# gersteinlab/LESSeq

Hardware: AMD Instinct MI355X
Metric: MRF reads/sec through count+solve (higher is better)
Workload: dtype int32 coordinates / u64 counters (count), f64 (EM); 1 GPU; BASELINE configs[2]: 100M synthetic 100bp reads over 50k mixed events (SE/RI/A5SS/A3SS/MXE/AFE/ALE/T3), 24 chromosomes; events=50000

## Files before the change

### include/lesseq_hip.h

```cpp
#ifndef LESSEQ_HIP_H
#define LESSEQ_HIP_H

#include <stddef.h>
#include <stdint.h>

#ifdef __cplusplus
extern "C" {
#endif

#define LSQ_ABI_VERSION 2

typedef enum {
	LSQ_OK = 0,
	LSQ_E_ARG = -1,
	LSQ_E_IO = -2,
	LSQ_E_FORMAT = -3,
	LSQ_E_PARSE = -4,
	LSQ_E_RANGE = -5,
	LSQ_E_UNSUPPORTED = -6,
	LSQ_E_DEVICE = -7,
	LSQ_E_STATE = -8,
	LSQ_E_INTERNAL = -9,
	LSQ_E_TIMEOUT = -10
} lsq_status;
// ... 88 lines not shown
int lsq_ctx_synchronize_for(lsq_ctx *c, double seconds);

int lsq_events_upload(lsq_ctx *c, lsq_events *e);

int lsq_reads_upload(lsq_ctx *c, int method, const lsq_reads *r);
int lsq_reads_upload_mrf(lsq_ctx *c, int method, const char *read_format, const char *path);
typedef struct lsq_text lsq_text;
int lsq_text_stage(lsq_ctx *c, const char *path, lsq_text **out);
void lsq_text_free(lsq_text *t);
int lsq_reads_upload_text(lsq_ctx *c, int method, const char *read_format, lsq_text *t);
int lsq_text_stage_range(lsq_ctx *c, const char *path, uint64_t byte_begin, uint64_t byte_end, lsq_text **out);
int lsq_text_lines(lsq_ctx *c, lsq_text *t, uint64_t *n_newlines);
int lsq_reads_upload_text_at(lsq_ctx *c, int method, const char *read_format, lsq_text *t, int has_header, uint64_t first_line);
int lsq_mrf_parse_device(lsq_ctx *c, const char *read_format, const char *path, lsq_reads **out);
int lsq_last_mrf_timing(lsq_ctx *c, float *h2d_ms, float *parse_ms);
int lsq_ingest_stage_count(void);
const char *lsq_ingest_stage_name(int stage);
int lsq_last_ingest_stages(const lsq_ctx *c, float *ms, uint64_t *bytes, int capacity);
const char *lsq_last_ingest_stage_name(const lsq_ctx *c, int stage);
int lsq_last_ingest_stage_count(const lsq_ctx *c);
int lsq_last_sam_paths(const lsq_ctx *c, uint32_t *lines_listed, uint32_t *all_slow);
int lsq_last_bam_paths(const lsq_ctx *c, uint64_t *n_blocks, uint64_t *blocks_repaired);
int lsq_bam_check(lsq_ctx *c, const char *path, lsq_bam_report *r);
uint64_t lsq_reads_retained(const lsq_ctx *c, int method);
int lsq_last_library_report(const lsq_ctx *c, int method, uint64_t out[5]);
uint64_t lsq_reads_retained_blocks(const lsq_ctx *c, int method);
uint64_t lsq_reads_pooled(const lsq_ctx *c, int method);
uint64_t lsq_reads_pooled_blocks(const lsq_ctx *c, int method);
int lsq_reads_pool_format(const lsq_ctx *c, int method, int *compact, uint64_t *pool_bytes, uint64_t *pool_reads);

int lsq_count(lsq_ctx *c);
int lsq_count_status(lsq_ctx *c, uint32_t *exceptions, uint32_t *recounted);
int lsq_count_launch_info(lsq_ctx *c, uint32_t *reads_per_look, uint32_t *workgroups_per_cu);
int lsq_host_evaluated(const lsq_ctx *c, uint64_t *n_genes, uint64_t *n_reads);
int lsq_ctx_set_option(lsq_ctx *c, const char *name, double value);

int lsq_solve(lsq_ctx *c);

int64_t lsq_results_num_classes(const lsq_ctx *c);
int lsq_results_class_offsets(const lsq_ctx *c, uint64_t *class_off );
int lsq_results_counts(lsq_ctx *c, uint64_t *class_count, uint64_t *class_bases);
int lsq_results_set_counts(lsq_ctx *c, const uint64_t *class_count, const uint64_t *class_bases);
uint64_t lsq_counts_device_words(const lsq_ctx *c);
int lsq_counts_export_device(lsq_ctx *c, void *d_words);
int lsq_counts_import_device(lsq_ctx *c, const void *d_words);
int lsq_results_solve(lsq_ctx *c, double *theta, double *logll, uint32_t *em_iters, uint8_t *em_flags);
int lsq_solve_finalize(lsq_ctx *c, uint32_t *n_replayed);
int lsq_set_em_guard_band(lsq_ctx *c, double band);

int lsq_fim(lsq_ctx *c);
int64_t lsq_results_fim_size(const lsq_ctx *c);
int lsq_results_fim_offsets(const lsq_ctx *c, uint64_t *fim_off );
int lsq_results_fim(lsq_ctx *c, double *fim, double *var_by_diag, double *var_by_inverse);

int lsq_bootstrap(lsq_ctx *c, uint32_t n_replicates, uint64_t seed);
int lsq_results_bootstrap(lsq_ctx *c, uint32_t *n_ok, double *mean, double *sd, double *q025, double *q500, double *q975);
int lsq_results_bootstrap_theta(lsq_ctx *c, double *theta );
int lsq_bootstrap_replicate(lsq_ctx *c, uint64_t seed, uint32_t b, uint64_t *class_count, double *theta, double *logll, uint32_t *iters, uint8_t *flags);
int lsq_bootstrap_tile(void);
int lsq_bootstrap_resample_host(int n_methods, uint64_t n_events, const uint64_t *class_off, const uint64_t *class_count, uint64_t seed, uint32_t b,
                                uint64_t *out);

int lsq_results_copy_device(lsq_ctx *c, void *d_class_count, void *d_theta, void *d_logll);
void *lsq_ctx_result_stream(lsq_ctx *c);

int lsq_shard_bounds(const lsq_events *e, int world, const double *weights ,
// ... 177 lines not shown
```

### lesseq_amd/api.py

```python
import os
import ctypes as C

import numpy as np

from ._lib import lib, check, check_runtime_once, SynthSpecStruct, BamReportStruct, u64, u32, i32, u16, u8, i64, vp, cs, P, _b

EVENT_TYPES = ("SE", "RI", "A5SS", "A3SS", "MXE", "AFE", "ALE", "T3")


def _take_text(ptr):
    if not ptr:
        return ""
    s = C.string_at(ptr).decode()
    lib.lsq_free(ptr)
    return s


def _ptr(a, ct):
    return a.ctypes.data_as(P(ct))


class Annotation:

    def __init__(self, isoforms_path, g2i_path, begin=0, end=2 ** 62, isoform_format="LH_GENE_TXT", g2i_format="UCSC_GENE2ISOFORM"):
# ... 359 lines not shown
        check(lib.lsq_last_library_report(self.h, method, out))
        return tuple(out)

    def pooled(self, method):
        return lib.lsq_reads_pooled(self.h, method)

    def pooled_blocks(self, method):
        return lib.lsq_reads_pooled_blocks(self.h, method)

    def pool_format(self, method):
        a, n = C.c_int(0), C.c_uint64(0)
        k = (C.c_uint64 * 3)()
        check(lib.lsq_reads_pool_format(self.h, method, C.byref(a), C.byref(n), k))
        return bool(a.value), n.value, tuple(int(x) for x in k)

    def retained_blocks(self, method):
        return lib.lsq_reads_retained_blocks(self.h, method)

    def count(self):
        check(lib.lsq_count(self.h))

    def solve(self):
        check(lib.lsq_solve(self.h))

    def set_option(self, name, value):
        check(lib.lsq_ctx_set_option(self.h, _b(name), float(value)))

    def count_status(self):
        M = max(self.events.n_methods, 1)
        e, r = (u32 * M)(), (u32 * M)()
        check(lib.lsq_count_status(self.h, e, r))
        return list(e)[:self.events.n_methods], list(r)[:self.events.n_methods]

    def counts_device_words(self):
        return int(lib.lsq_counts_device_words(self.h))

    def export_counts_device(self, d_ptr):
        check(lib.lsq_counts_export_device(self.h, vp(d_ptr)))

    def import_counts_device(self, d_ptr):
        check(lib.lsq_counts_import_device(self.h, vp(d_ptr)))

    def launch_info(self):
        a, b = u32(), u32()
        check(lib.lsq_count_launch_info(self.h, C.byref(a), C.byref(b)))
        return int(a.value), int(b.value)

    def set_em_guard_band(self, band):
        check(lib.lsq_set_em_guard_band(self.h, float(band)))

    def solve_finalize(self):
        n = u32()
        check(lib.lsq_solve_finalize(self.h, C.byref(n)))
        return n.value

    EM_LEAN_FORMS = ("none", "four_lane", "four_lane_capped_tail", "head_tail", "four_lane_flat3", "four_lane_flat4")

    def em_launch(self):
        out = (C.c_uint * 8)()
        check(lib.lsq_debug_last_em_launch(self.h, out))
        return {"lean_form": self.EM_LEAN_FORMS[out[0]], "lean_places": int(out[1]), "split": int(out[2]), "general_places": int(out[3]),
                "learnt_placement": bool(out[4]), "quad_cap": int(out[5]), "placement_learnt_after": bool(out[6]), "lane": int(out[7])}

    def synchronize(self):
        check(lib.lsq_ctx_synchronize(self.h))

# ... 176 lines not shown
```

### lesseq_amd/csrc/lsq_count.hip

```cpp
#include "lsq_device.hpp"
#include <hip/hip_ext.h>

namespace {

#ifndef LSQ_COUNT_BLOCK
#define LSQ_COUNT_BLOCK 256
#endif
constexpr int COUNT_BLOCK = LSQ_COUNT_BLOCK;
constexpr unsigned long long BASES_MASK = (1ull << 40) - 1;

#ifdef LSQ_DEV
#define ABL(args, bits) ((((args).ablate) & (bits)) != 0u)
#else
#define ABL(args, bits) false
#endif


struct CountArgs {
	const BucketDesc *buckets;
	const unsigned char *images;
	const TieRec *ties;
	const unsigned char *strand_rank;
	const char *read_names; const unsigned long long *read_name_off;
	const char *gene_names; const unsigned *gene_name_off;
	unsigned n_buckets;
	unsigned ablate;
	unsigned tables_lds_bytes;
	const void *p1; const unsigned char *p1_strand; const unsigned *p1_line;
	const void *p2; const unsigned char *p2_strand; const unsigned *p2_line;
	unsigned compact;
	const unsigned *pn_blk_off; const unsigned *pn_nblk; const int2 *pn_se; const unsigned char *pn_strand; const unsigned *pn_line; const unsigned *pn_bucket;
	const unsigned long long *p1_off, *p2_off, *pn_off, *slot_off;
	const lsq::VisitRec *visits;
	const unsigned *wg_first;
	const unsigned long long *wg_cut;
	const lsq::WgPlan *wg_plan;
	unsigned long long *wg_trace;
	unsigned long long total_slots;
	unsigned long long n_pn;
	unsigned n_workers;
	unsigned long long *cnt, *bases;
	struct ExcEntry *exc;
	unsigned *exc_count;
	unsigned exc_cap;
	unsigned long long *dbg;
	unsigned long long *bar;
};

__device__ inline int2 unpack_one_block(const unsigned a, const int base) {
	const int s = base + (int)(a & lsq::COMPACT_OFF_MASK);
	return make_int2(s, s + (int)(a >> lsq::COMPACT_OFF_BITS));
}
__device__ inline int4 unpack_two_block(const unsigned a, const unsigned b, const int base) {
	const int s1 = base + (int)(a & lsq::COMPACT_OFF_MASK), e1 = s1 + (int)(a >> lsq::COMPACT_OFF_BITS);
	const int s2 = e1 + (int)(b & lsq::COMPACT_OFF_MASK);
	return make_int4(s1, e1, s2, s2 + (int)(b >> lsq::COMPACT_OFF_BITS));
}
__device__ inline int2 pool1_read(const CountArgs &A, const unsigned long long g, const int lo) {
	if (!A.compact) return reinterpret_cast<const int2 *>(A.p1)[g];
	return unpack_one_block(reinterpret_cast<const unsigned *>(A.p1)[g], lo - lsq::COMPACT_BIAS);
}
__device__ inline int4 pool2_read(const CountArgs &A, const unsigned long long g, const int lo) {
	if (!A.compact) return reinterpret_cast<const int4 *>(A.p2)[g];
	const uint2 v = reinterpret_cast<const uint2 *>(A.p2)[g];
	return unpack_two_block(v.x, v.y, lo - lsq::COMPACT_BIAS);
}

struct LdsView {
	const unsigned short *bins;
	const EventRec *ev;
	const int2 *segs;
	const unsigned *iso;
	unsigned long long *hist;
};

__device__ __noinline__ bool tie_orders_read_first(const CountArgs &A, unsigned ev_index, unsigned read_strand, unsigned line) {
	const TieRec *t = A.ties + ev_index;
	const unsigned rs = A.strand_rank[read_strand], gs = A.strand_rank[t->strand_id];
	if (rs != gs) return rs < gs;
// ... 151 lines not shown
			}
		}
		__syncthreads();
	}
}


__device__ inline int nonneg(int x) { return (int)(~(unsigned)x >> 31); }
__device__ inline int inside01(int a, int sx, int sy) { return nonneg((a - sx) | (sy - 1 - a)); }
__device__ inline int gt01(int b, int sy) { return (int)((unsigned)(sy - b) >> 31); }

__device__ inline unsigned run_bits(const int (&sy)[4], unsigned abut, int r0, int r1, int r2, int r3, int b, int &end_run) {
	r1 |= r0 & (int)(abut & 1u) & gt01(b, sy[0]);
	r2 |= r1 & (int)((abut >> 1) & 1u) & gt01(b, sy[1]);
	r3 |= r2 & (int)((abut >> 2) & 1u) & gt01(b, sy[2]);
	end_run = max(max(r0 ? sy[0] : 0, r1 ? sy[1] : 0), max(r2 ? sy[2] : 0, r3 ? sy[3] : 0));
	return (unsigned)(r0 | (r1 << 1) | (r2 << 2) | (r3 << 3));
}

struct FastCtx {
	const uint4 *bins;
	int lo; unsigned shift, n_bins;
	const uint4 *recs;
	unsigned long long *hist;
	unsigned n_events, bucket;
	unsigned long long slot0;
	unsigned pool;
	ExcEntry *exc;
	unsigned *exc_count;
	unsigned exc_cap;
	unsigned ablate;
	unsigned long long *dbg;
	unsigned long long *trace;
};

__device__ inline void emit_exception(const FastCtx &C, unsigned r, unsigned i, unsigned scan) {
	const unsigned slot = atomicAdd(C.exc_count, 1u);
	if (slot < C.exc_cap) {
		ExcEntry e;
		e.slot = C.slot0 + r;
		e.bucket = C.bucket;
		e.ev_pool_scan = i | (C.pool << 29) | (scan << 31);
		C.exc[slot] = e;
	}
}

constexpr unsigned PARK_EVENT_UNKNOWN = 0x7FFFFFFFu;
constexpr unsigned PARK_ONE_EVENT = 0x80000000u;

__device__ inline unsigned wave_sum_u32(unsigned v) {
	v += (unsigned)__builtin_amdgcn_update_dpp(0, (int)v, 0x111, 0xf, 0xf, true);
	v += (unsigned)__builtin_amdgcn_update_dpp(0, (int)v, 0x112, 0xf, 0xf, true);
	v += (unsigned)__builtin_amdgcn_update_dpp(0, (int)v, 0x114, 0xf, 0xf, true);
	v += (unsigned)__builtin_amdgcn_update_dpp(0, (int)v, 0x118, 0xf, 0xf, true);
	v += (unsigned)__builtin_amdgcn_update_dpp(0, (int)v, 0x142, 0xa, 0xf, true);
	v += (unsigned)__builtin_amdgcn_update_dpp(0, (int)v, 0x143, 0xc, 0xf, true);
	return (unsigned)__builtin_amdgcn_readlane((int)v, 63);
}

template <int NB>
__device__ inline bool fast_trip(const FastCtx &C, const int4 v, const int total, const unsigned r, const unsigned i, const bool valid) {
	const int p = v.x, q = (NB == 1) ? v.y : v.w;
	const bool inb = valid && i < C.n_events;
	const unsigned ri = 3u * (inb ? i : 0u);
	const uint4 w0 = C.recs[ri], w1 = C.recs[ri + 1], w2 = C.recs[ri + 2];
	const int gs = (int)w1.x, ge = (int)w0.x;
	const bool started = inb && gs <= p;
	bool covers = started && p <= ge;
	bool exc = covers && p == gs && q == ge;
	covers = covers && !(p == gs && q <= ge);
	if (NB == 2) {
		const bool touching = covers && v.z == v.y;
		exc = exc || touching;
		covers = covers && !touching;
	}
	if (exc && !ABL(C, 128u)) emit_exception(C, r, i, 0u);
	const int sx[4] = {(int)w1.x, (int)w1.z, (int)w2.x, (int)w2.z};
// ... 38 lines not shown
__device__ inline void wave_sync_lds() {
	__builtin_amdgcn_fence(__ATOMIC_ACQ_REL, "wavefront");
	__builtin_amdgcn_wave_barrier();
}

template <int NB>
struct Ring {
	static constexpr unsigned CAP = WAVE_QUEUE_WORDS / NB;
	uint4 *q;
	unsigned head = 0, tail = 0;
	__device__ inline unsigned live() const { return tail - head; }
	__device__ inline void push(bool want, unsigned lane, const uint4 e0, const uint4 e1) {
		const unsigned long long m = __ballot(want);
		if (!m) return;
		const unsigned at = (tail + (unsigned)__popcll(m & ((1ull << lane) - 1ull))) % CAP;
		if (want) {
			if (NB == 1) q[at] = e0;
			else { q[2 * at] = e0; q[2 * at + 1] = e1; }
		}
		tail += (unsigned)__popcll(m);
	}
	__device__ inline void push2(const unsigned bits, const unsigned lane, const uint4 ea, const uint4 eb) {
		static_assert(NB == 1 || NB == 2, "");
		const unsigned long long m0 = __ballot((bits & 1u) != 0u), m1 = __ballot((bits & 2u) != 0u);
		if (!(m0 | m1)) return;
		const unsigned long long lt = (1ull << lane) - 1ull;
		const unsigned at = tail + (unsigned)__popcll(m0 & lt) + (unsigned)__popcll(m1 & lt);
		if (bits & 1u) q[at % CAP] = ea;
		if (bits & 2u) q[(at + (bits & 1u)) % CAP] = eb;
		tail += (unsigned)__popcll(m0) + (unsigned)__popcll(m1);
	}
};

template <int NB, bool PACKED2 = false>
__device__ inline void walk_parked(const FastCtx &C, Ring<(NB == 1 || PACKED2) ? 1 : 2> &R, const bool to_empty, const int base = 0) {
	constexpr int RW = (NB == 1 || PACKED2) ? 1 : 2;
	const unsigned lane = threadIdx.x & 63u;
	wave_sync_lds();
#pragma unroll 1
	while (R.live() >= (to_empty ? 1u : 64u)) {
		const unsigned n = min(R.live(), 64u);
		const bool on = lane < n;
		if (ABL(C, 256u) && lane == 0) { atomicAdd(&C.dbg[2], 1ull); atomicAdd(&C.dbg[3], (unsigned long long)n); }
		if (ABL(C, 4194304u) && lane == 0 && C.trace) { atomicAdd(&C.trace[2], 1ull); atomicAdd(&C.trace[3], (unsigned long long)n); }
		const unsigned at = (R.head + (on ? lane : 0u)) % Ring<RW>::CAP;
		uint4 e0, e1 = make_uint4(0, 0, 0, 0);
		if (RW == 1) e0 = R.q[at];
		else { e0 = R.q[2 * at]; e1 = R.q[2 * at + 1]; }
		R.head += n;
		int4 rd; unsigned i, rel;
		const unsigned ev_word = RW == 1 ? e0.z : e1.x;
		const bool one_event = (ev_word & PARK_ONE_EVENT) != 0;
		if (RW == 1) { e0.z &= ~PARK_ONE_EVENT; } else { e1.x &= ~PARK_ONE_EVENT; }
		if (NB == 1) {
			rd = make_int4((int)e0.x, (int)e0.y, (int)e0.x, (int)e0.y); i = e0.z; rel = e0.w;
			const int brel = rd.x - C.lo;
			const unsigned bin = brel <= 0 ? 0u : min((unsigned)brel >> C.shift, C.n_bins - 1u);
			const unsigned first = reinterpret_cast<const unsigned *>(C.bins)[4u * bin] >> 16;
			if (i == PARK_EVENT_UNKNOWN) { i = first; e0.z = first; }
		}
		else if (PACKED2) {
			rd = unpack_two_block(e0.x, e0.y, base); i = e0.z; rel = e0.w;
			const int brel = rd.x - C.lo;
			const unsigned bin = brel <= 0 ? 0u : min((unsigned)brel >> C.shift, C.n_bins - 1u);
			const unsigned first = reinterpret_cast<const unsigned *>(C.bins)[4u * bin] >> 16;
			if (i == PARK_EVENT_UNKNOWN) { i = first; e0.z = first; }
		}
		else {
			rd = make_int4((int)e0.x, (int)e0.y, (int)e0.z, (int)e0.w); i = e1.x; rel = e1.y;
			const int brel = rd.x - C.lo;
			const unsigned bin = brel <= 0 ? 0u : min((unsigned)brel >> C.shift, C.n_bins - 1u);
			const unsigned first = reinterpret_cast<const unsigned *>(C.bins)[4u * bin] >> 16;
			if (i == PARK_EVENT_UNKNOWN) { i = first; e1.x = first; }
		}
		const int total = NB == 1 ? rd.y - rd.x : (rd.y - rd.x) + (rd.w - rd.z);
		const bool more = fast_trip<NB>(C, rd, total, rel, i, on) && !one_event && !ABL(C, 64u);
		wave_sync_lds();
		if (RW == 1) e0.z = i + 1u; else e1.x = i + 1u;
		R.push(more, lane, e0, e1);
		wave_sync_lds();
	}
}

template <int RPW>
__device__ inline void stream_pool_wide(FastCtx &C, const uint4 *bins, const uint4 *cells, const uint4 *cellx, const unsigned n_cells, const BucketDesc &d,
                                        const CountArgs &A, uint4 *queue, const uint4 *src_generic,
                                        const unsigned long long g0, const unsigned long long g1) {
	constexpr int NB = RPW == 2 ? 1 : 2;
	constexpr int SW = 2;
	static_assert(RPW != 2 || (unsigned)(SW * RPW) <= P1_GROUP_PAD, "a lane's reads of a step lie in one cell group");
	constexpr unsigned TILE = 64u * SW;
	C.pool = RPW == 2 ? 0u : 1u;
	C.slot0 = g0;
	global_words src = (global_words)src_generic;
	const unsigned lane = threadIdx.x & 63u, wave = (unsigned)__builtin_amdgcn_readfirstlane((int)(threadIdx.x >> 6));
// ... 191 lines not shown
					if (n_add2) atomicAdd(&C.hist[L1.jslot], ((unsigned long long)n_add2 << 40) | s_add2);
				} else asm volatile("" ::"v"(n_add), "v"(s_add), "v"(n_add2), "v"(s_add2));
			}
		}
		if (RPW == 1) {
			static_assert(RPW != 1 || N_READS == 2, "two parked entries a step");
#pragma unroll
			for (int q = 0; q < 2; ++q) {
				const bool pq = park[q ? N_READS - 1 : 0];
				const uint4 q0 = pe0[q ? N_READS - 1 : 0], q1 = pe1[q ? N_READS - 1 : 0];
				if (ABL(A, 256u) && pq) atomicAdd(&A.dbg[NB - 1], 1ull);
				R.push(pq, lane, q0, q1);
				if (R.live() >= 64u) {
					if (!ABL(A, 32u)) walk_parked<NB>(C, R, false);
					else R.head = R.tail;
				}
			}
		}
	};
	if (ww0 < ww1) fetch(ww0);
	for (unsigned wt = ww0; wt < ww1; wt += WAVES * TILE) {
		uint4 cur[SW];
#pragma unroll
		for (int k = 0; k < SW; ++k) cur[k] = nxt[k];
		if (wt + WAVES * TILE < ww1) fetch(wt + WAVES * TILE);
		do_step(cur, wt);
	}
	if (R.live() && !ABL(A, 32u)) walk_parked<NB>(C, R, true);
}


template <int NR>
__device__ inline void stream_pool1_compact(FastCtx &C, const uint4 *bins, const uint4 *cells, const uint4 *cellx, const unsigned n_cells, const BucketDesc &d,
                                            const CountArgs &A, uint4 *queue, const void *pool, const unsigned long long g0, const unsigned long long g1) {
	static_assert(NR == 4 || NR == 8, "one or two 16-byte words of four compact records");
	static_assert((unsigned)NR <= P1_GROUP_PAD, "a lane's records of a step lie in one cell group");
	constexpr int CW = NR / 4;
	constexpr unsigned TILE = 64u * NR;
	C.pool = 0u;
	C.slot0 = g0;
	global_words src = (global_words)pool;
	const unsigned lane = threadIdx.x & 63u, wave = (unsigned)__builtin_amdgcn_readfirstlane((int)(threadIdx.x >> 6));
	const unsigned long long R0 = g0 & ~(unsigned long long)(NR - 1);
	const unsigned n = (unsigned)(g1 - R0), first_rel = (unsigned)(g0 - R0), n_rel = (unsigned)(g1 - g0);
	const unsigned last_word = (n - 1u) >> 2;
	const int base = d.lo - lsq::COMPACT_BIAS;
	uint4 nxt[CW];
	auto fetch = [&](const unsigned t) {
#pragma unroll
		for (int cq = 0; cq < CW; ++cq) {
			const unsigned w = min((t >> 2) + lane * (unsigned)CW + (unsigned)cq, last_word);
			const u32x4 v = src[(R0 >> 2) + w];
			nxt[cq] = make_uint4(v.x, v.y, v.z, v.w);
		}
	};
	Ring<1> R;
	R.q = queue;
	const unsigned t_begin = min(wave * TILE, n);
	if (t_begin < n) fetch(t_begin);
	for (unsigned t = t_begin; t < n; t += WAVES * TILE) {
		unsigned rec[NR];
#pragma unroll
		for (int cq = 0; cq < CW; ++cq) { rec[4 * cq] = nxt[cq].x; rec[4 * cq + 1] = nxt[cq].y; rec[4 * cq + 2] = nxt[cq].z; rec[4 * cq + 3] = nxt[cq].w; }
		if (t + WAVES * TILE < n) fetch(t + WAVES * TILE);
		if (ABL(A, 512u)) {
#pragma unroll
			for (int j = 0; j < NR; ++j) asm volatile("" ::"v"(rec[j]));
			continue;
		}
		const int p0 = (int)(rec[0] & lsq::COMPACT_OFF_MASK) + base;
		const int rel0 = p0 - d.lo;
		const unsigned bin = rel0 <= 0 ? 0u : ((unsigned)rel0 >> d.shift);
		const uint4 br = bins[min(bin, d.n_bins - 1u)];
		unsigned ci = (br.x & 0xFFFFu) + (unsigned)(p0 >= (int)br.y) + (unsigned)(p0 >= (int)br.z) + (unsigned)(p0 >= (int)br.w);
		if (__any(p0 >= (int)br.w) && !ABL(A, 65536u)) {
			while (ci + 1u < n_cells && p0 >= (int)cells[ci + 1u].x) ++ci;
		}
		const unsigned cc = min(ci, n_cells - 1u);
		const uint4 cw = cells[cc];
		const uint4 cx = cellx[cc];
		const bool has = ci < n_cells && (int)cw.x <= p0 && p0 < (int)cw.y && !ABL(A, 8u);
		const bool both = has && (cx.z & CELLX_BOTH) != 0;
		const int e1 = has ? (int)cw.z - base : -1, e2 = has ? (int)cw.w - base : -1;
		const bool interior = t + TILE <= n && t >= first_rel;
		unsigned accN = 0, accA = 0, accL = 0;
		auto decide = [&](auto whole_step, auto one_threshold) {
#pragma unroll
			for (int j = 0; j < NR; ++j) {
				const unsigned len = rec[j] >> lsq::COMPACT_OFF_BITS;
				const int e = (int)(rec[j] & lsq::COMPACT_OFF_MASK) + (int)len;
				unsigned p = len | (min(len, 1u) << 24);
				if (!decltype(whole_step)::value) {
					const unsigned idx = t + lane * (unsigned)NR + (unsigned)j;
					p = (idx < n && idx - first_rel < n_rel) ? p : 0u;
				}
				accN += p;
				accA += e <= e1 ? p : 0u;
				if (!decltype(one_threshold)::value) accL += e <= e2 ? p : 0u;
			}
			if (decltype(one_threshold)::value) accL = accA;
		};
		if (__all(e1 == e2) && !ABL(A, 8388608u)) { if (interior) decide(std::true_type{}, std::true_type{}); else decide(std::false_type{}, std::true_type{}); }
		else { if (interior) decide(std::true_type{}, std::false_type{}); else decide(std::false_type{}, std::false_type{}); }
		const unsigned s1 = cx.x & 0xFFFFu, s2 = cx.x >> 16;
		if (!ABL(A, (1u | 16384u))) {
			const unsigned acc2 = both ? accL : accL - accA;
			if (accA && s1 != CELL_NONE) atomicAdd(&C.hist[s1], ((unsigned long long)(accA >> 24) << 40) | (accA & 0xFFFFFFu));
			if (acc2 && s2 != CELL_NONE) atomicAdd(&C.hist[s2], ((unsigned long long)(acc2 >> 24) << 40) | (acc2 & 0xFFFFFFu));
		} else asm volatile("" ::"v"(accA), "v"(accL));
		const bool lane_open = (accN >> 24) != ((both ? accA : accL) >> 24);
		if (ABL(A, 256u)) {
			const bool any_open = __any(lane_open);
			if (lane == 0) { atomicAdd(&A.dbg[12], 1ull); atomicAdd(&A.dbg[11], any_open ? 1ull : 0ull); }
		}
		if (__any(lane_open) && !ABL(A, 17u | 524288u)) {
#pragma unroll
			for (int h = 0; h < NR; h += 2) {
				uint4 en[2];
				unsigned open = 0;
#pragma unroll
				for (int j = h; j < h + 2; ++j) {
					const unsigned len = rec[j] >> lsq::COMPACT_OFF_BITS;
					const int so = (int)(rec[j] & lsq::COMPACT_OFF_MASK), e = so + (int)len;
					const unsigned idx = t + lane * (unsigned)NR + (unsigned)j, rel = idx - first_rel;
					const bool in = idx < n && rel < n_rel;
					const bool gone_near = both && (cx.z & CELLX_NEAR_NO_ABUT) != 0u && e > e1 && 50 * (e - e1) >= (int)len;
					const bool gone_far = both && (cx.z & CELLX_FAR_NO_ABUT) != 0u && e > e2 && 50 * (e - e2) >= (int)len;
					const bool done_near = e <= e1 || gone_near, done_far = e <= e2 || gone_far;
					const bool op = in && len != 0u && !(both ? (done_near && done_far) : e <= e2);
					open |= op ? 1u << (j - h) : 0u;
					const unsigned hint = !has ? PARK_EVENT_UNKNOWN : (!both ? (cx.w | PARK_ONE_EVENT) :
					                      (done_far ? (cx.w | PARK_ONE_EVENT) : (done_near ? ((cx.z & 0xFFFFu) | PARK_ONE_EVENT) : PARK_EVENT_UNKNOWN)));
					en[j - h] = make_uint4((unsigned)(so + base), (unsigned)(so + base) + len, hint, rel);
					if (ABL(A, 256u) && op) { atomicAdd(&A.dbg[5 + (has ? (both ? 2 : 1) : 0)], 1ull); atomicAdd(&A.dbg[0], 1ull); }
				}
				R.push2(open, lane, en[0], en[1]);
				if (R.live() >= 64u) {
					if (!ABL(A, 32u)) walk_parked<1, false>(C, R, false, base);
					else R.head = R.tail;
				}
			}
		}
	}
	if (R.live() && !ABL(A, 32u)) walk_parked<1, false>(C, R, true, base);
}

template <int NR>
__device__ inline void stream_pool2_compact(FastCtx &C, const uint4 *bins, const uint4 *cells, const uint4 *cellx, const unsigned n_cells, const BucketDesc &d,
                                            const CountArgs &A, uint4 *queue, const void *pool, const unsigned long long g0, const unsigned long long g1) {
	static_assert((NR == 2 || NR == 4 || NR == 8) && (unsigned)NR <= P2_GROUP_PAD, "whole 16-byte words of two compact records, inside one junction group");
	constexpr int CW = NR / 2;
	constexpr unsigned TILE = 64u * NR;
	C.pool = 1u;
	C.slot0 = g0;
	global_words src = (global_words)pool;
	const unsigned lane = threadIdx.x & 63u, wave = (unsigned)__builtin_amdgcn_readfirstlane((int)(threadIdx.x >> 6));
	const unsigned long long R0 = g0 & ~(unsigned long long)(NR - 1);
	const unsigned n = (unsigned)(g1 - R0), first_rel = (unsigned)(g0 - R0), n_rel = (unsigned)(g1 - g0);
	const unsigned last_word = (n - 1u) >> 1;
	const int base = d.lo - lsq::COMPACT_BIAS;
	uint4 nxt[CW];
	auto fetch = [&](const unsigned t) {
#pragma unroll
		for (int cq = 0; cq < CW; ++cq) {
			const unsigned w = min((t >> 1) + lane * (unsigned)CW + (unsigned)cq, last_word);
			const u32x4 v = src[(R0 >> 1) + w];
			nxt[cq] = make_uint4(v.x, v.y, v.z, v.w);
		}
	};
	Ring<1> R;
	R.q = queue;
	const unsigned t_begin = min(wave * TILE, n);
	if (t_begin < n) fetch(t_begin);
	for (unsigned t = t_begin; t < n; t += WAVES * TILE) {
		unsigned ra[NR], rb[NR];
#pragma unroll
		for (int cq = 0; cq < CW; ++cq) { ra[2 * cq] = nxt[cq].x; rb[2 * cq] = nxt[cq].y; ra[2 * cq + 1] = nxt[cq].z; rb[2 * cq + 1] = nxt[cq].w; }
		if (t + WAVES * TILE < n) fetch(t + WAVES * TILE);
		if (ABL(A, 512u)) {
#pragma unroll
			for (int j = 0; j < NR; ++j) asm volatile("" ::"v"(ra[j]), "v"(rb[j]));
			continue;
		}
		const bool interior = t + TILE <= n && t >= first_rel;
		const unsigned idx0 = t + lane * (unsigned)NR, rel0 = idx0 - first_rel;
		const bool in0 = interior || (idx0 < n && rel0 < n_rel);
		const int4 rd = unpack_two_block(ra[0], rb[0], base);
		const int rel_p = rd.x - d.lo;
		const unsigned bin = rel_p <= 0 ? 0u : ((unsigned)rel_p >> d.shift);
		const uint4 br = bins[min(bin, d.n_bins - 1u)];
		unsigned c1 = (br.x & 0xFFFFu) + (unsigned)(rd.x >= (int)br.y) + (unsigned)(rd.x >= (int)br.z) + (unsigned)(rd.x >= (int)br.w);
		const unsigned evf = br.x >> 16;
		if (__any(rd.x >= (int)br.w) && !ABL(A, 65536u)) {
			while (c1 + 1u < n_cells && rd.x >= (int)cells[c1 + 1u].x) ++c1;
		}
		const unsigned c1c = min(c1, n_cells - 1u);
		const uint4 cw1 = cells[c1c];
		const uint4 cx1 = cellx[c1c];
		const unsigned i1 = cx1.y;
		const unsigned k1 = (i1 >> 2) & 0x3Fu;
		const bool here = c1 < n_cells && (int)cw1.x <= rd.x && rd.x < (int)cw1.y && !ABL(A, 8u);
		const bool v1 = here && i1 < CELL_INFO_EMPTY;
		const bool start1 = k1 == CELL_K_START;
		const bool inside1 = v1 && !start1 && rd.y <= (int)cw1.z && rd.z != rd.y;
		const bool ends1 = inside1 && rd.y == (int)cw1.z;
		const bool ends1b = v1 && !start1 && (int)cw1.w > (int)cw1.z && rd.y == (int)cw1.w && rd.z != rd.y;
		const unsigned ri = 3u * (v1 ? cx1.w : 0u);
		const uint4 w0r = C.recs[ri], w1r = C.recs[ri + 1u], w2r = C.recs[ri + 2u];
		const unsigned k2 = rd.z == (int)w1r.z ? 1u : (rd.z == (int)w2r.x ? 2u : (rd.z == (int)w2r.z ? 3u : 0u));
		const int end2 = k2 == 1u ? (int)w1r.w : (k2 == 2u ? (int)w2r.y : (int)w2r.w);
		const unsigned abut = (w0r.y >> FAST_ABUT_SHIFT) & 7u;
		const bool abut2 = k2 != 0u && k2 < 3u && ((abut >> k2) & 1u) != 0u;
		const int end2b = !abut2 ? end2 : (k2 == 1u ? (int)w2r.y : (int)w2r.w);
		const unsigned k1e = ends1b ? k1 + 1u : k1;
		const bool junction = (ends1 || ends1b) && k2 > k1e;
		const bool J = junction && rd.w <= end2, Jb = junction && rd.w > end2 && rd.w <= end2b;
		const unsigned len1 = ra[0] >> lsq::COMPACT_OFF_BITS, total = len1 + (rb[0] >> lsq::COMPACT_OFF_BITS);
		const unsigned long long tbl = ((unsigned long long)w0r.w << 32) | w0r.z;
		const unsigned mask1 = (1u << (k1 & 3u)) | (ends1b ? 2u << (k1 & 3u) : 0u), maskA = mask1 | (1u << k2), maskB = maskA | (2u << k2);
		const unsigned clsA = (unsigned)(tbl >> (4u * (maskA & 15u))) & 0xFu, clsB = abut2 ? (unsigned)(tbl >> (4u * (maskB & 15u))) & 0xFu : 0u;
		const unsigned sa = cx1.x & 0xFFFFu;
		const unsigned slotA = clsA != 0u ? (w0r.y & 0xFFFFu) + clsA - 1u : CELL_NONE, slotB = clsB != 0u ? (w0r.y & 0xFFFFu) + clsB - 1u : CELL_NONE;
		const bool any_plain = __any(!junction);
		bool two = false, empty = false, near_free = false, far_free = false, S = false, drop = false, addS = false;
		int e1c = 0, e2c = 0;
// ... 22 lines not shown
		}
		bool park[NR];
		park[0] = in0 && len1 != 0u && !(J || Jb || S || drop || none[0]) && !ABL(A, 17u | 1048576u);
		if (ABL(A, 256u) && park[0]) atomicAdd(&A.dbg[8 + (v1 ? 1 : 0)], 1ull);
		unsigned nA = (in0 && J && slotA != CELL_NONE) ? 1u : 0u, sA = nA ? total : 0u, nB = (in0 && Jb && slotB != CELL_NONE) ? 1u : 0u, sB = nB ? total : 0u;
		const int lim = junction ? end2 - rd.y : -1, limb = junction ? end2b - rd.y : -1;
		bool any_park = park[0];
		const bool any_b = __any(limb > lim) || ABL(A, 8388608u);
#pragma unroll
		for (int j = 1; j < NR; ++j) {
			const unsigned l1 = ra[j] >> lsq::COMPACT_OFF_BITS, l2 = rb[j] >> lsq::COMPACT_OFF_BITS;
			const int reach = (int)(rb[j] & lsq::COMPACT_OFF_MASK) + (int)l2;
			bool in = l1 != 0u;
			if (!interior) { const unsigned idx = idx0 + (unsigned)j; in = in && idx < n && idx - first_rel < n_rel; }
			const bool sameA = in && reach <= lim;
			bool sameB = false;
			const bool cA = sameA && slotA != CELL_NONE;
			nA += cA ? 1u : 0u; sA += cA ? l1 + l2 : 0u;
			if (any_b) {
				sameB = in && reach > lim && reach <= limb;
				const bool cB = sameB && slotB != CELL_NONE;
				nB += cB ? 1u : 0u; sB += cB ? l1 + l2 : 0u;
			}
			park[j] = in && !(sameA || sameB || none[j]) && !ABL(A, 17u | 1048576u | 2097152u);
			if (ABL(A, 256u) && park[j]) atomicAdd(&A.dbg[junction ? 14 : 13], 1ull);
			any_park = any_park || park[j];
		}
		if (!ABL(A, 1u)) {
			if (addS) atomicAdd(&C.hist[sa], (1ull << 40) | len1);
			if (nA) atomicAdd(&C.hist[slotA], ((unsigned long long)nA << 40) | sA);
			if (nB) atomicAdd(&C.hist[slotB], ((unsigned long long)nB << 40) | sB);
		} else asm volatile("" ::"v"(nA), "v"(sA), "v"(nB), "v"(sB));
		if (__any(any_park)) {
			const unsigned hint0 = v1 ? (cx1.w | PARK_ONE_EVENT) : evf;
#pragma unroll
			for (int h = 0; h < NR; h += 2) {
				const uint4 qa = make_uint4(ra[h], rb[h], h == 0 ? hint0 : PARK_EVENT_UNKNOWN, rel0 + (unsigned)h);
				const uint4 qb = make_uint4(ra[h + 1], rb[h + 1], PARK_EVENT_UNKNOWN, rel0 + (unsigned)h + 1u);
				if (ABL(A, 256u)) atomicAdd(&A.dbg[1], (park[h] ? 1ull : 0ull) + (park[h + 1] ? 1ull : 0ull));
				R.push2((park[h] ? 1u : 0u) | (park[h + 1] ? 2u : 0u), lane, qa, qb);
				if (R.live() >= 64u) {
					if (!ABL(A, 32u)) walk_parked<2, true>(C, R, false, base);
					else R.head = R.tail;
				}
			}
		}
	}
	if (R.live() && !ABL(A, 32u)) walk_parked<2, true>(C, R, true, base);
}

__device__ inline void global_add_merged(unsigned long long *cnt, unsigned long long *bases, bool want, const unsigned slot, const unsigned matched) {
	const unsigned lane = threadIdx.x & 63u;
#pragma unroll 1
	for (int round = 0; round < 4; ++round) {
		const unsigned long long m = __ballot(want);
		if (!m) return;
		const unsigned lead = (unsigned)__ffsll((long long)m) - 1u;
		const unsigned s0 = (unsigned)__builtin_amdgcn_readlane((int)slot, lead);
		const bool same = want && slot == s0;
		const unsigned n = (unsigned)__popcll(__ballot(same));
		const unsigned sum = wave_sum_u32(same ? matched : 0u);
		if (lane == lead) { atomicAdd(&cnt[s0], (unsigned long long)n); atomicAdd(&bases[s0], (unsigned long long)sum); }
		want = want && !same;
	}
	if (want) { atomicAdd(&cnt[slot], 1ull); atomicAdd(&bases[slot], (unsigned long long)matched); }
}

__device__ inline void pool_n_worker(const CountArgs &A, const unsigned long long n_pn, const unsigned n_workers) {
	const unsigned long long gsz = (unsigned long long)n_workers * COUNT_BLOCK;
	for (unsigned long long g0 = (unsigned long long)blockIdx.x * COUNT_BLOCK; g0 < n_pn; g0 += gsz) {
		const unsigned long long g = g0 + threadIdx.x;
		bool active = g < n_pn;
		const unsigned b = active ? A.pn_bucket[g] : 0u;
		const BucketDesc *d = A.buckets + b;
		active = active && d->kind == 1;
		const unsigned *bins = reinterpret_cast<const unsigned *>(A.images + d->img_off);
		const uint4 *recs = reinterpret_cast<const uint4 *>(A.images + d->img_off + d->ev_off);
		const int2 *blk = A.pn_se + (active ? A.pn_blk_off[g] : 0u);
		const int nblk = active ? (int)A.pn_nblk[g] : 1;
		int p = 0, q = 0, total = 0;
		unsigned i = 0;
// ... 25 lines not shown
						}
						if (cand) {
							const int nseg = (int)((w0.y >> FAST_NSEG_SHIFT) & 7u);
							Walk w;
							for (int k = 0; k < nblk; ++k) { const int2 bk = blk[k]; if (!w.block(segs, nseg, bk.x, bk.y)) break; }
							const unsigned long long tbl = ((unsigned long long)w0.w << 32) | w0.z;
							const unsigned cls = w.mask < 16u ? (unsigned)(tbl >> (4u * w.mask)) & 0xFu : 0u;
							if (cls != 0 && 50ll * w.matched > 49ll * total) { want = true; slot = d->cls_base + (w0.y & 0xFFFFu) + cls - 1; matched = (unsigned)w.matched; }
						}
						if (p <= ge && !(w0.y & FAST_FLAG_OVERLAPS_NEXT)) active = false;
						++i;
					}
				}
			}
			global_add_merged(A.cnt, A.bases, want, slot, matched);
		}
	}
}

#ifndef LSQ_FAST_WAVES
#define LSQ_FAST_WAVES 6
#endif
template <bool COMPACT, int P1W>
__global__ void __launch_bounds__(COUNT_BLOCK, P1W == 4 ? 5 : LSQ_FAST_WAVES) lsq_count_fast_kernel(CountArgs A) {
	extern __shared__ __align__(16) unsigned char lds[];
	const unsigned tid = threadIdx.x;
	struct Trace {
		unsigned long long *p;
		__device__ Trace(unsigned long long *q) : p(q) { if (p && threadIdx.x == 0) p[4u * blockIdx.x] = wall_clock64(); }
		__device__ ~Trace() { if (p && threadIdx.x == 0) p[4u * blockIdx.x + 1u] = wall_clock64(); }
	} trace(ABL(A, 4194304u) ? A.wg_trace : nullptr);
	if (blockIdx.x < A.n_workers) { pool_n_worker(A, A.n_pn, A.n_workers); return; }
	const unsigned wg = blockIdx.x - A.n_workers, n_wg = gridDim.x - A.n_workers;
	uint4 *wave_queue = reinterpret_cast<uint4 *>(lds + A.tables_lds_bytes) + (tid >> 6) * WAVE_QUEUE_WORDS;
	(void)n_wg;
	typedef const lsq::VisitRec __attribute__((address_space(4))) *const_visit;
	typedef const lsq::WgPlan __attribute__((address_space(4))) *const_plan;
	const_plan plan = (const_plan)(A.wg_plan + wg);
	const unsigned long long s_begin = plan->s_begin, s_end = plan->s_end;
	if (s_begin >= s_end) return;
	if (ABL(A, 4096u)) return;
	const_visit vr = &plan->first;
	unsigned b = vr->b;
	bool first_visit = true;
	while (b < A.n_buckets) {
		const unsigned long long bs = vr->bs;
		if (bs >= s_end) break;
		BucketDesc d;
		d.img_off = vr->d.img_off; d.img_bytes = vr->d.img_bytes; d.n_events = vr->d.n_events; d.n_bins = vr->d.n_bins; d.lo = vr->d.lo; d.shift = vr->d.shift;
		d.ev_off = vr->d.ev_off; d.seg_off = vr->d.seg_off; d.iso_off = vr->d.iso_off; d.hist_off = vr->d.hist_off; d.n_cls = vr->d.n_cls; d.cls_base = vr->d.cls_base;
		d.ev_base = vr->d.ev_base; d.chrom_id = vr->d.chrom_id; d.kind = vr->d.kind; d.hi = vr->d.hi;
		const unsigned long long be = vr->be, p1o = vr->p1o, n1 = vr->p1n, p2o = vr->p2o, n2 = vr->p2n;
		const unsigned next = vr->next;
		unsigned char *buf = lds;
		if (!first_visit) __syncthreads();
		first_visit = false;
		{
			global_words src = (global_words)(A.images + d.img_off);
			uint4 *dst = reinterpret_cast<uint4 *>(buf);
			for (unsigned i = tid; i < d.img_bytes / 16; i += COUNT_BLOCK) { const u32x4 t = src[i]; dst[i] = make_uint4(t.x, t.y, t.z, t.w); }
			unsigned long long *h = reinterpret_cast<unsigned long long *>(buf + d.hist_off);
			for (unsigned i = tid; i < HIST_REPLICAS * (d.n_cls | 1u); i += COUNT_BLOCK) h[i] = 0;
		}
		__syncthreads();
		if (ABL(A, 8192u)) return;
		const uint4 *bins = reinterpret_cast<const uint4 *>(buf);
		const uint4 *cells = reinterpret_cast<const uint4 *>(buf + d.seg_off);
		const unsigned n_cells = d.iso_off & 0xFFFFu;
		const uint4 *cellx = reinterpret_cast<const uint4 *>(buf + d.seg_off + 16u * (d.iso_off >> 16));
		FastCtx C;
		C.bins = bins; C.lo = d.lo; C.shift = d.shift; C.n_bins = d.n_bins;
		C.recs = reinterpret_cast<const uint4 *>(buf + d.ev_off);
		C.hist = reinterpret_cast<unsigned long long *>(buf + d.hist_off) + (tid & (HIST_REPLICAS - 1u)) * (d.n_cls | 1u);
		C.n_events = d.n_events; C.bucket = b;
		C.slot0 = 0; C.pool = 0;
		C.exc = A.exc; C.exc_count = A.exc_count; C.exc_cap = A.exc_cap; C.ablate = A.ablate; C.dbg = A.dbg;
		C.trace = (ABL(A, 4194304u) && A.wg_trace) ? A.wg_trace + 4u * blockIdx.x : nullptr;
		const unsigned long long l0 = (s_begin > bs ? s_begin : bs) - bs;
		const unsigned long long l1 = (s_end < be ? s_end : be) - bs;
		if (l0 < n1 && !ABL(A, 1024u)) {
			if constexpr (COMPACT) stream_pool1_compact<2 * P1W>(C, bins, cells, cellx, n_cells, d, A, wave_queue, A.p1, p1o + l0, p1o + (l1 < n1 ? l1 : n1));
			else stream_pool_wide<2>(C, bins, cells, cellx, n_cells, d, A, wave_queue, reinterpret_cast<const uint4 *>(A.p1), p1o + l0, p1o + (l1 < n1 ? l1 : n1));
		}
		if (l1 > n1 && l0 < n1 + n2 && !ABL(A, 2048u)) {
			const unsigned long long q0 = p2o + ((l0 > n1 ? l0 : n1) - n1), q1 = p2o + ((l1 < n1 + n2 ? l1 : n1 + n2) - n1);
			if constexpr (COMPACT) stream_pool2_compact<(P1W == 4 ? LSQ_P2_COMPACT_WORDS_W5 : LSQ_P2_COMPACT_WORDS)>(C, bins, cells, cellx, n_cells, d, A, wave_queue, A.p2, q0, q1);
			else stream_pool_wide<1>(C, bins, cells, cellx, n_cells, d, A, wave_queue, reinterpret_cast<const uint4 *>(A.p2), q0, q1);
		}
		__syncthreads();
		for (unsigned i = tid; i < d.n_cls; i += COUNT_BLOCK) {
			const unsigned long long *h0 = reinterpret_cast<const unsigned long long *>(buf + d.hist_off) + i;
			unsigned long long v = 0;
#pragma unroll
			for (unsigned r = 0; r < HIST_REPLICAS; ++r) v += h0[r * (d.n_cls | 1u)];
			if (v && !ABL(A, 4u)) {
				atomicAdd(&A.cnt[d.cls_base + i], v >> 40);
				atomicAdd(&A.bases[d.cls_base + i], v & BASES_MASK);
			}
		}
		if (be >= s_end) break;
		b = next;
		vr = (const_visit)(A.visits + b);
	}
}

struct GlobalBucket {
	const BucketDesc *d;
	const unsigned *bins;
	const uint4 *recs;
};

__device__ inline GlobalBucket global_bucket(const CountArgs &A, unsigned b) {
	GlobalBucket G;
	G.d = A.buckets + b;
	G.bins = reinterpret_cast<const unsigned *>(A.images + G.d->img_off);
	G.recs = reinterpret_cast<const uint4 *>(A.images + G.d->img_off + G.d->ev_off);
	return G;
}

__device__ void eval_read_global(const CountArgs &A, const GlobalBucket &G, const int2 *blk, int nblk, unsigned i, bool scan,
// ... 98 lines not shown

namespace lsq {

struct SharePlanCosts { bool weighted = true, snap = true; double two_block = 4.3, walk_look = 9.0, visit = 7000.0, taper = 0.5, hot = 0.0; };
void plan_share_cuts_seg(const unsigned long long *so, const unsigned char *visited_kind, const size_t B, const unsigned long long *x, const unsigned char *kind,
                         const unsigned *looks, const unsigned *bseg, const size_t S, const unsigned long long grid, const SharePlanCosts &pc, unsigned long long *cut) {
	const unsigned long long total_slots = B ? so[B] : 0;
	const bool weighted = pc.weighted && x && kind && looks && bseg && S > 0;
	cut[0] = 0;
	if (!weighted) {
		for (unsigned long long g = 1; g <= grid; ++g) cut[(size_t)g] = total_slots / grid * g + total_slots % grid * g / grid;
		if (pc.snap && grid > 0) {
			const double share = (double)total_slots / (double)grid;
			size_t bb = 0;
			for (unsigned long long g = 1; g < grid; ++g) {
				const unsigned long long t = cut[(size_t)g];
				while (bb + 1 < B && so[bb + 1] <= t) ++bb;
				const unsigned long long lo = so[bb], hi = so[bb + 1];
				unsigned long long u = t;
				if (t - lo <= hi - t && (double)(t - lo) < 0.3 * share) u = lo;
				else if ((double)(hi - t) < 0.3 * share) u = hi;
				cut[(size_t)g] = std::max(u, cut[(size_t)g - 1]);
			}
		}
		cut[(size_t)grid] = total_slots;
		return;
	}
	const double c2 = pc.two_block, cw = pc.walk_look, cv = pc.visit, d_rest = 1e-3;
	const double taper = std::min(1.0, std::max(0.05, pc.taper));
	std::vector<double> dens(S), cum(S + 1, 0.0), jump(S, 0.0), cum_b(B + 1, 0.0);
	for (size_t b = 0; b < B; ++b) if (visited_kind[b] && so[b + 1] > so[b] && bseg[b] < bseg[b + 1]) jump[bseg[b]] = cv;
	for (size_t i = 0; i < S; ++i) {
		const double len = (double)(x[i + 1] - x[i]);
		dens[i] = kind[i] == 2 || len <= 0 ? d_rest : (kind[i] == 0 ? 1.0 : c2) + cw * (double)looks[i] / len + (len >= 8192.0 ? pc.hot : 0.0);
		cum[i + 1] = cum[i] + jump[i] + len * dens[i];
	}
	for (size_t b = 0; b <= B; ++b) cum_b[b] = cum[std::min<size_t>(bseg[b], S)];
	const double total_cost = cum[S];
	const double wsum = (double)grid * (1.0 + taper) / 2.0;
	auto part_before = [&](unsigned long long g) {
		const double k = (double)g, slope = grid > 1 ? (taper - 1.0) / (double)(grid - 1) : 0.0;
		return (k + slope * k * (k - 1.0) / 2.0) / wsum;
	};
	size_t bb = 0, si = 0;
	for (unsigned long long g = 1; g < grid && total_cost > 0; ++g) {
		const double tc = total_cost * part_before(g), share = total_cost * (part_before(g + 1) - part_before(g));
		while (bb + 1 < B && cum_b[bb + 1] <= tc) ++bb;
		while (si + 1 < S && cum[si + 1] <= tc) ++si;
		const double xb = tc - cum_b[bb], yb = cum_b[bb + 1] - tc;
		unsigned long long t;
		if (pc.snap && xb <= yb && xb < 0.3 * share) t = so[bb];
		else if (pc.snap && yb < xb && yb < 0.3 * share) t = so[bb + 1];
		else {
			const double r = tc - cum[si] - jump[si];
			const unsigned long long len = x[si + 1] - x[si];
			t = x[si] + (r <= 0.0 ? 0ull : std::min<unsigned long long>((unsigned long long)(r / dens[si]), len));
		}
		cut[(size_t)g] = std::max(t, cut[(size_t)g - 1]);
	}
	if (!(total_cost > 0)) for (unsigned long long g = 1; g < grid; ++g) cut[(size_t)g] = total_slots * g / grid;
	cut[(size_t)grid] = total_slots;
	for (unsigned long long g = 0; g < grid; ++g)
		if (cut[(size_t)g + 1] - cut[(size_t)g] > (1ull << 21)) {
			for (unsigned long long q = 1; q < grid; ++q) cut[(size_t)q] = total_slots * q / grid;
			break;
		}
}
// ... 10 lines not shown
		const unsigned long long n1 = visited ? std::min(pn1[b], ns) : 0, n2 = visited ? std::min(pn2[b], ns - n1) : 0;
		if (n1) { x.push_back(so[b]); kind.push_back(0); looks.push_back(look1[b]); }
		if (n2) { x.push_back(so[b] + n1); kind.push_back(1); looks.push_back(look2[b]); }
		if (ns - n1 - n2) { x.push_back(so[b] + n1 + n2); kind.push_back(2); looks.push_back(0); }
	}
	bseg[B] = (unsigned)kind.size();
	x.push_back(B ? so[B] : 0);
	plan_share_cuts_seg(so, visited_kind, B, x.data(), kind.data(), looks.data(), bseg.data(), kind.size(), grid, pc, cut);
}

int run_count(lsq_ctx *c) {
	const lsq_events &E = *c->E;
	const size_t n_cls = E.n_cls_total;
	const int M = E.n_methods;
	hipStream_t st_em = nullptr;
	const int prev_lane = c->lane, prev_set = c->set;
	const int lane = prev_lane ^ 1, set = (prev_set + 1) % c->opt_counter_sets;
	hipStream_t st = c->opt_two_count_streams ? c->stream_count2[lane] : c->stream;
	if (c->mark_recorded2[set]) HIP_TRY(hipStreamWaitEvent(st, c->ev_mark2[set], 0));
	HIP_TRY(hipMemsetAsync(c->counters.p + (size_t)prev_set * c->counters_per_set, 0, c->counters_per_set * sizeof(unsigned long long), c->stream_em2[prev_lane]));
	HIP_TRY(hipEventRecord(c->ev_mark2[prev_set], c->stream_em2[prev_lane]));
	c->mark_recorded2[prev_set] = true;
	select_counter_set(c, lane, set);
	st_em = c->stream_em;
	c->fast_launched = 0;
	struct Cleanup { CountArgs A; unsigned long long n_pn; int m; };
	std::vector<Cleanup> cleanups;
	bool counted_signalled = false;
	if (c->time_events) HIP_TRY(hipEventRecord(c->ev0, st));
	const unsigned generic_tables_bytes = (std::max<unsigned>(E.max_lds_bytes, 16) + 15u) & ~15u;
	const unsigned tables_bytes = generic_tables_bytes;
	double max_skew = 0.0;
	for (int m = 0; m < M; ++m) max_skew = std::max(max_skew, c->reads[m].skew);
	const unsigned cap = c->opt_wg_per_cu >= 0 ? (unsigned)c->opt_wg_per_cu : (c->em.small_places >= c->em.opt_flat_min && max_skew < 4.0 ? 5u : 0u);
	const unsigned lds_bytes = std::max(tables_bytes + WAVES * WAVE_QUEUE_WORDS * 16, cap ? 160u * 1024u / (cap + 1u) + 16u : 0u);
	if (lds_bytes > 160 * 1024) return fail(LSQ_E_UNSUPPORTED, "bucket tables + read tile exceed the CU's LDS");
	bool all_compact = true;
	for (int m = 0; m < M; ++m) if (c->reads[m].total_slots && !c->reads[m].compact) all_compact = false;
	const int p1w = !all_compact ? 2 : (c->opt_reads_per_look ? (c->opt_reads_per_look == 8 ? 4 : 2) : (cap != 0 && cap <= 5 ? 4 : 2));
	const void *const fn_wide = (const void *)lsq_count_fast_kernel<false, 2>;
	const void *const fn_compact = p1w == 4 ? (const void *)lsq_count_fast_kernel<true, 4> : (const void *)lsq_count_fast_kernel<true, 2>;
	c->last_reads_per_look = 2u * (unsigned)p1w;
	if (lds_bytes > 64 * 1024) {
		HIP_TRY(hipFuncSetAttribute(fn_wide, hipFuncAttributeMaxDynamicSharedMemorySize, (int)lds_bytes));
		HIP_TRY(hipFuncSetAttribute(fn_compact, hipFuncAttributeMaxDynamicSharedMemorySize, (int)lds_bytes));
		HIP_TRY(hipFuncSetAttribute((const void *)lsq_count_generic_kernel, hipFuncAttributeMaxDynamicSharedMemorySize, (int)lds_bytes));
	}
	unsigned per_cu = std::max(1u, std::min(2048u / COUNT_BLOCK, (160u * 1024u) / lds_bytes));
	{
		if (c->occ_lds_bytes != lds_bytes || c->occ_p1w != p1w) {
			int nb = 0;
			int nb2 = 0;
			HIP_TRY(hipOccupancyMaxActiveBlocksPerMultiprocessor(&nb, fn_wide, (int)COUNT_BLOCK, (size_t)lds_bytes));
			HIP_TRY(hipOccupancyMaxActiveBlocksPerMultiprocessor(&nb2, fn_compact, (int)COUNT_BLOCK, (size_t)lds_bytes));
			c->occ_lds_bytes = lds_bytes; c->occ_p1w = p1w; c->occ_blocks = all_compact ? nb2 : std::min(nb, nb2);
		}
		if (c->occ_blocks >= 1) per_cu = std::min(per_cu, (unsigned)c->occ_blocks);
	}
	c->last_wg_per_cu = per_cu;
	for (int m = 0; m < M; ++m) {
		MethodReads &mr = c->reads[m];
		if (mr.total_slots == 0 || E.buckets.empty()) continue;
		const double mult = c->opt_grid_mult > 0 ? c->opt_grid_mult : (mr.skew >= 32.0 ? 4.0 : (mr.skew >= 4.0 || p1w == 4 ? 3.0 : 2.0));
		unsigned long long grid = (unsigned long long)((double)c->n_cu * per_cu * mult);
		grid = std::max(grid, mr.total_slots / (1ull << 21) + 1);
		grid = std::min<unsigned long long>(grid, std::max<unsigned long long>(mr.total_slots / 64, 1));
#ifdef LSQ_DEV
		if (const char *e = getenv("LSQ_GRID_WGS")) { const long v = atol(e); if (v >= 1) grid = (unsigned long long)v; }
// ... 26 lines not shown
			int rc = mr.wg_first.upload(first.data(), first.size(), st);
			if (!rc) rc = mr.wg_cut.upload(cut.data(), cut.size(), st);
			if (rc) return rc;
			{
				std::vector<WgPlan> plan((size_t)grid);
				for (unsigned long long g = 0; g < grid; ++g) {
					WgPlan &w = plan[(size_t)g];
					w.s_begin = cut[(size_t)g]; w.s_end = cut[(size_t)g + 1];
					w.first = mr.visits_host[std::min<size_t>(first[(size_t)g], B)];
				}
				if ((rc = mr.wg_plan.upload(plan.data(), plan.size(), st))) return rc;
				HIP_TRY(hipStreamSynchronize(st));
			}
			HIP_TRY(hipStreamSynchronize(st));
			mr.wg_grid = grid;
		}
		CountArgs A{};
		A.buckets = c->buckets.p; A.images = c->images.p; A.ties = c->ties.p; A.strand_rank = c->strand_rank.p;
		A.wg_first = mr.wg_first.p; A.wg_cut = mr.wg_cut.p; A.wg_plan = mr.wg_plan.p; A.visits = mr.visits.p;
		A.read_names = mr.named ? mr.names.p : nullptr; A.read_name_off = mr.named ? mr.name_off.p : nullptr;
		A.gene_names = c->gene_names.p; A.gene_name_off = c->gene_name_off.p;
		A.n_buckets = (unsigned)E.buckets.size();
		A.tables_lds_bytes = tables_bytes;
		A.ablate = c->dev_ablate;
		A.compact = mr.compact ? 1u : 0u;
		A.p1 = mr.p1.p; A.p1_strand = mr.p1_strand.p; A.p1_line = mr.p1_line.p;
		A.p2 = mr.p2.p; A.p2_strand = mr.p2_strand.p; A.p2_line = mr.p2_line.p;
		A.pn_blk_off = mr.pn_blk_off.p; A.pn_nblk = mr.pn_nblk.p; A.pn_se = reinterpret_cast<const int2 *>(mr.pn_se.p);
		A.pn_strand = mr.pn_strand.p; A.pn_line = mr.pn_line.p; A.pn_bucket = mr.pn_bucket.p;
		A.p1_off = mr.p1_off.p; A.p2_off = mr.p2_off.p; A.pn_off = mr.pn_off.p; A.slot_off = mr.slot_off.p;
		A.total_slots = mr.total_slots;
		A.cnt = c->cnt.p + (size_t)m * n_cls; A.bases = c->bases.p + (size_t)m * n_cls;
		A.exc = mr.exc.p + (size_t)set * mr.exc_cap; A.exc_count = c->exc_count.p + 2 * m; A.exc_cap = (unsigned)mr.exc_cap;
		A.dbg = c->dbg.p; A.bar = c->dbg.p + 16 + m;
		A.wg_trace = nullptr;
		const unsigned long long n_pn = mr.pn_strand.n;
		A.n_pn = n_pn;
		const unsigned workers_per_cu = 2;
		A.n_workers = (unsigned)std::min<unsigned long long>((n_pn + COUNT_BLOCK - 1) / COUNT_BLOCK, (unsigned long long)c->n_cu * workers_per_cu);
#ifdef LSQ_DEV
		if (c->dev_ablate & 32768u) A.n_workers = 0;
#endif
		if (c->has_fast) {
			if (c->time_events) HIP_TRY(hipEventRecord(c->evf0[m], st));
			const bool last_streaming = m == M - 1 && !c->has_generic && !c->time_events;
			const dim3 fgrid((unsigned)grid + A.n_workers);
#ifdef LSQ_DEV
			if (c->dev_ablate & 4194304u) {
				if (c->wg_trace.n < 4ull * fgrid.x) { int rc = c->wg_trace.alloc(4ull * fgrid.x); if (rc) return rc; }
				HIP_TRY(hipMemsetAsync(c->wg_trace.p, 0, 4ull * fgrid.x * sizeof(unsigned long long), st));
				c->wg_trace_n = fgrid.x; c->wg_trace_workers = A.n_workers;
				A.wg_trace = c->wg_trace.p;
			}
#endif
			void *kargs[] = {(void *)&A};
			HIP_TRY(hipExtLaunchKernel(mr.compact ? fn_compact : fn_wide, fgrid, dim3(COUNT_BLOCK), kargs, lds_bytes, st, nullptr, last_streaming ? c->ev_counted2[lane] : nullptr, 0));
			if (last_streaming) counted_signalled = true;
			if (c->time_events) HIP_TRY(hipEventRecord(c->evf1[m], st));
			c->fast_launched |= 1 << m;
			cleanups.push_back({A, n_pn, m});
		}
		if (c->has_generic) {
			hipLaunchKernelGGL(lsq_count_generic_kernel, dim3((unsigned)grid), dim3(COUNT_BLOCK), generic_tables_bytes, st, A);
			HIP_TRY(hipGetLastError());
		}
	}
	if (c->time_events) HIP_TRY(hipEventRecord(c->ev1, st));
// ... 9 lines not shown
	for (const Cleanup &u : cleanups) {
		const size_t slot = ((size_t)set * LSQ_MAX_METHODS + (size_t)u.m) * sizeof(CountArgs);
		if (memcmp(c->recount_args_host.data() + slot, &u.A, sizeof(CountArgs)) != 0) {
			memcpy(c->recount_args_host.data() + slot, &u.A, sizeof(CountArgs));
			HIP_TRY(hipMemcpyAsync(c->recount_args.p + slot, c->recount_args_host.data() + slot, sizeof(CountArgs), hipMemcpyHostToDevice, st_em));
		}
		const CountArgs *dA = reinterpret_cast<const CountArgs *>(c->recount_args.p + slot);
		hipLaunchKernelGGL(lsq_count_cleanup_kernel, dim3(c->opt_cleanup_grid ? c->opt_cleanup_grid : rgrid), dim3(256), 0, st_em, dA, c->opt_recount ? 1 : 0, u.n_pn,
		                   (const ExcEntry *)u.A.exc, (const unsigned *)u.A.exc_count, u.A.exc_cap);
		HIP_TRY(hipGetLastError());
	}
	return LSQ_OK;
}

}

extern "C" {

int lsq_count_status(lsq_ctx *c, uint32_t *exceptions, uint32_t *recounted) LSQ_API_TRY {
	if (!c) return fail(LSQ_E_ARG, "null context");
	if (!c->counted) return fail(LSQ_E_STATE, "lsq_count must come first");
	HIP_TRY(hipSetDevice(c->device));
	{ int rc = sync_all(c); if (rc) return rc; }
	std::vector<unsigned> h(c->exc_count.n);
	HIP_TRY(hipMemcpy(h.data(), c->exc_count.p, h.size() * sizeof(unsigned), hipMemcpyDeviceToHost));
	note_overflow(c, h);
	for (int m = 0; m < c->E->n_methods; ++m) {
		if (exceptions) exceptions[m] = h[2 * (size_t)m];
		if (recounted) recounted[m] = h[2 * (size_t)m + 1];
	}
	return LSQ_OK;
} LSQ_API_CATCH

int lsq_count_launch_info(lsq_ctx *c, uint32_t *reads_per_look, uint32_t *workgroups_per_cu) LSQ_API_TRY {
	if (!c) return fail(LSQ_E_ARG, "null context");
	if (!c->counted) return fail(LSQ_E_STATE, "lsq_count must come first");
	if (reads_per_look) *reads_per_look = c->last_reads_per_look;
	if (workgroups_per_cu) *workgroups_per_cu = c->last_wg_per_cu;
	return LSQ_OK;
} LSQ_API_CATCH

int lsq_debug_counters(lsq_ctx *c, unsigned long long *out8) LSQ_API_TRY {
	HIP_TRY(hipSetDevice(c->device));
	{ int rc = sync_all(c); if (rc) return rc; }
	HIP_TRY(hipMemcpy(out8, c->dbg.p, 16 * sizeof(unsigned long long), hipMemcpyDeviceToHost));
	std::vector<unsigned> h(c->exc_count.n);
	HIP_TRY(hipMemcpy(h.data(), c->exc_count.p, h.size() * sizeof(unsigned), hipMemcpyDeviceToHost));
	out8[4] = h[0];
	return LSQ_OK;
} LSQ_API_CATCH

int lsq_debug_wg_trace(lsq_ctx *c, unsigned long long *out, unsigned long long cap, unsigned long long *n, unsigned long long *n_workers) LSQ_API_TRY {
	HIP_TRY(hipSetDevice(c->device));
	{ int rc = sync_all(c); if (rc) return rc; }
	const unsigned long long k = std::min<unsigned long long>(cap, c->wg_trace_n);
	if (k) HIP_TRY(hipMemcpy(out, c->wg_trace.p, 4 * k * sizeof(unsigned long long), hipMemcpyDeviceToHost));
	*n = k; *n_workers = c->wg_trace_workers;
	return LSQ_OK;
} LSQ_API_CATCH

int lsq_debug_plan_shares(const unsigned long long *slot_off, const unsigned char *packed, const unsigned long long *n1, const unsigned long long *n2,
                          const unsigned *look1, const unsigned *look2, unsigned long long n_buckets, unsigned long long grid,
                          const double *costs4, int weighted, int snap, unsigned long long *cuts) LSQ_API_TRY {
	if (!slot_off || !packed || !costs4 || !cuts || grid == 0) return fail(LSQ_E_ARG, "null argument");
	lsq::SharePlanCosts pc;
	pc.weighted = weighted != 0; pc.snap = snap != 0;
// ... 34 lines not shown
```

### lesseq_amd/csrc/lsq_device.hip

```cpp
#include "lsq_device.hpp"
#include <chrono>
#include <thread>

namespace lsq {

int upload_strand_ranks(lsq_ctx *c) {
	const auto &names = c->E->strands.names;
	if (names.size() > 256) return fail(LSQ_E_RANGE, "more than 256 distinct strand strings");
	std::vector<int> order(names.size());
	std::iota(order.begin(), order.end(), 0);
	std::sort(order.begin(), order.end(), [&](int a, int b) { return names[a] < names[b]; });
	std::vector<uint8_t> rank(256, 0);
	for (size_t r = 0; r < order.size(); ++r) rank[order[r]] = (uint8_t)r;
	int rc = c->strand_rank.upload(rank.data(), 256, c->stream);
	if (rc) return rc;
	HIP_TRY(hipStreamSynchronize(c->stream));
	return LSQ_OK;
}

static hipError_t wait_for_stream(hipStream_t s) {
	const auto t0 = std::chrono::steady_clock::now();
	for (;;) {
		const hipError_t e = hipStreamQuery(s);
		if (e != hipErrorNotReady) return e;
// ... 1 lines not shown
	}
}

int ensure_lanes(lsq_ctx *c) {
	if (c->lanes_thread.joinable()) c->lanes_thread.join();
	if (c->lanes_status) return fail(c->lanes_status, "%s", c->lanes_error.c_str());
	return LSQ_OK;
}

int sync_all(lsq_ctx *c) {
	{ const int rc = ensure_lanes(c); if (rc) return rc; }
	HIP_TRY(wait_for_stream(c->stream_count2[0]));
	HIP_TRY(wait_for_stream(c->stream_count2[1]));
	HIP_TRY(wait_for_stream(c->stream_em2[0]));
	HIP_TRY(wait_for_stream(c->stream_em2[1]));
	HIP_TRY(wait_for_stream(c->stream));
	return LSQ_OK;
}

void select_counter_set(lsq_ctx *c, int lane, int set) {
	unsigned long long *base = c->counters.p + (size_t)set * c->counters_per_set;
	const size_t per = c->cnt.n;
	c->lane = lane;
	c->set = set;
	c->stream_em = c->stream_em2[lane];
	c->theta.p = c->theta2[lane].p; c->theta.n = c->theta2[lane].n;
	c->logll.p = c->logll2[lane].p; c->logll.n = c->logll2[lane].n;
	c->iters.p = c->iters2[lane].p; c->iters.n = c->iters2[lane].n;
	c->flags.p = c->flags2[lane].p; c->flags.n = c->flags2[lane].n;
	c->cnt.p = base;
	c->bases.p = base + per;
	c->exc_count.p = reinterpret_cast<unsigned *>(base + 2 * per);
	c->dbg.p = base + 2 * per + LSQ_MAX_METHODS;
}

void note_overflow(lsq_ctx *c, const std::vector<unsigned> &h) {
	for (int m = 0; m < c->E->n_methods; ++m) {
		if (!h[2 * (size_t)m + 1] || c->overflow_logged[m]) continue;
		c->overflow_logged[m] = true;
		if (c->opt_recount) continue;
		warn("read file %d: the exception list overflowed (%u pairs for %zu entries); every read of the file was counted again on the device. "
		     "Tables are complete; raise lsq_ctx_set_option \"exception_capacity\" to avoid the second pass", m, h[2 * (size_t)m], c->reads[m].exc_cap);
	}
}

}

extern "C" {

int lsq_ctx_create(int device_id, lsq_ctx **out) { return lsq_ctx_create_with(device_id, 0u, out); }

int lsq_ctx_create_with(int device_id, unsigned flags, lsq_ctx **out) LSQ_API_TRY {
	if (!out) return fail(LSQ_E_ARG, "null argument");
	const bool timing = getenv("LSQ_CLI_TIMING") != nullptr;
	auto t_last = std::chrono::steady_clock::now();
	auto mark = [&](const char *what) {
		if (!timing) return;
		const auto t = std::chrono::steady_clock::now();
		fprintf(stderr, "[timing]     %-32s %.3f s\n", what, std::chrono::duration<double>(t - t_last).count());
		t_last = t;
	};
	int n = 0;
	hipError_t e = hipGetDeviceCount(&n);
	mark("context: runtime start-up");
	if (e != hipSuccess || n <= 0) return fail(LSQ_E_DEVICE, "no HIP device available (%s)", e == hipSuccess ? "device count 0" : hipGetErrorString(e));
	if (device_id < 0 || device_id >= n) return fail(LSQ_E_ARG, "device %d out of range (%d devices)", device_id, n);
// ... 159 lines not shown
		if ((rc = c->gene_name_off.upload(goff.data(), goff.size(), c->stream))) return rc;
	}
	{
		const size_t n_dev = E->dev2out.size();
		std::vector<uint32_t> order(n_dev);
		std::iota(order.begin(), order.end(), 0u);
		std::sort(order.begin(), order.end(), [&](uint32_t a, uint32_t b) { return E->dev2out[a] < E->dev2out[b]; });
		std::vector<uint32_t> pc, pi, pe;
		for (uint32_t dd : order) {
			const int K = E->dev_K[dd];
			for (uint32_t k = 0; k < (1u << K) - 1u; ++k) pc.push_back(E->dev_cls_base[dd] + k);
			for (int j = 0; j < K; ++j) pi.push_back(E->dev_iso_base[dd] + (uint32_t)j);
			pe.push_back(dd);
		}
		if ((rc = c->pack_cls.upload(pc.data(), pc.size(), c->stream))) return rc;
		if ((rc = c->pack_iso.upload(pi.data(), pi.size(), c->stream))) return rc;
		if ((rc = c->pack_ev.upload(pe.data(), pe.size(), c->stream))) return rc;
	}
	mark("events: images, EM order, pack lists");
	const size_t n_iso = E->n_iso_total, M = (size_t)E->n_methods;
	std::vector<double> G(std::max<size_t>(M * n_iso, 1), 0.0);
	for (size_t d = 0; d < E->dev2out.size(); ++d) {
		const Event &ev = E->ev[E->dev2out[d]];
		for (size_t m = 0; m < M; ++m)
			for (int j = 0; j < ev.K; ++j) {
				double nd = (double)ev.ars[m][j];
				G[m * n_iso + E->dev_iso_base[d] + j] = nd <= 0 ? 0.0 : (double)1.0 / nd;
			}
	}
	if ((rc = c->G.upload(G.data(), M * n_iso, c->stream))) return rc;
	const size_t n_cls = E->n_cls_total, n_ev = E->dev2out.size();
	{
		const size_t per = std::max<size_t>(M, 1) * n_cls;
		c->counters_per_set = 2 * per + LSQ_MAX_METHODS + 16 + LSQ_MAX_METHODS;
		if ((rc = c->counters.alloc(LSQ_COUNTER_SETS * c->counters_per_set))) return rc;
		c->cnt.n = per; c->bases.n = per; c->exc_count.n = 2 * LSQ_MAX_METHODS; c->dbg.n = 16;
		for (bool &r : c->mark_recorded2) r = false;
		c->fim_uploaded = false; c->fim_done = false;
		select_counter_set(c, 0, 0);
		HIP_TRY(hipMemsetAsync(c->counters.p, 0, c->counters.n * sizeof(unsigned long long), c->stream));
	}
	for (int l = 0; l < 2; ++l) {
		if ((rc = c->theta2[l].alloc(n_iso)) || (rc = c->logll2[l].alloc(n_ev)) || (rc = c->iters2[l].alloc(n_ev)) || (rc = c->flags2[l].alloc(n_ev))) return rc;
		HIP_TRY(hipMemsetAsync(c->flags2[l].p, 0, std::max<size_t>(n_ev, 1), c->stream));
	}
	select_counter_set(c, 0, 0);
	mark("events: G, counters, EM outputs");
	{
		const size_t nc = E->covered.size();
		std::vector<RouteChrom> chrom(std::max<size_t>(nc, 1));
		std::vector<int2> cov;
		std::vector<int4> clu;
		for (size_t ch = 0; ch < nc; ++ch) {
			RouteChrom &R = chrom[ch];
			memset(&R, 0, sizeof(R));
			R.cov0 = (unsigned)cov.size();
			for (size_t q = 0; q < E->covered[ch].s.size(); ++q) cov.push_back(make_int2((int)E->covered[ch].s[q], (int)E->covered[ch].e[q]));
			R.cov1 = (unsigned)cov.size();
			R.clu0 = (unsigned)clu.size();
			const int first = ch < E->chrom_first_bucket.size() ? E->chrom_first_bucket[ch] : -1;
			if (first >= 0 && ch < E->clu_s.size() && ch < E->cut_lo.size()) {
				const std::vector<int32_t> &cuts = E->cut_lo[ch];
				for (size_t q = 0; q < E->clu_s[ch].size(); ++q) {
					long long s = E->clu_s[ch][q];
					const long long e = E->clu_e[ch][q];
					while (s <= e) {
						const size_t ub = (size_t)(std::upper_bound(cuts.begin(), cuts.end(), (int32_t)s) - cuts.begin());
						const long long next_cut = ub < cuts.size() ? (long long)cuts[ub] : e + 1;
						const long long stop = std::min(e, next_cut - 1);
// ... 24 lines not shown
			}
			std::vector<uint2> loc;
			for (size_t ch = 0; ch < nc; ++ch) {
				RouteChrom &R = chrom[ch];
				R.loc_first = (unsigned)loc.size();
				if (hi[ch] < lo[ch]) continue;
				const long long base = (lo[ch] >> shift) << shift;
				const long long nb = ((hi[ch] - base) >> shift) + 1;
				R.loc_base = (int)base; R.loc_nb = (unsigned)nb;
				unsigned a = R.cov0, u = R.clu0;
				for (long long k = 0; k <= nb; ++k) {
					const long long x = base + (k << shift);
					while (a < R.cov1 && cov[a].x < x) ++a;
					while (u < R.clu1 && clu[u].x < x) ++u;
					loc.push_back(make_uint2(a, u));
				}
			}
			loc.push_back(make_uint2(0, 0)); loc.push_back(make_uint2(0, 0));
			if (cov.empty()) cov.push_back(make_int2(0, 0));
			if (clu.empty()) clu.push_back(make_int4(0, 0, 0, 0));
			c->loc_shift = shift;
			if ((rc = c->loc.upload(loc.data(), loc.size(), c->stream))) return rc;
			if ((rc = c->route_chrom.upload(chrom.data(), chrom.size(), c->stream))) return rc;
			if ((rc = c->cov.upload(cov.data(), cov.size(), c->stream))) return rc;
			if ((rc = c->clu.upload(clu.data(), clu.size(), c->stream))) return rc;
			HIP_TRY(hipStreamSynchronize(c->stream));
		}
		mark("events: loader tables + locator");
		std::vector<unsigned> bb(E->buckets.size() + 1, 0);
		for (size_t b = 0; b < E->buckets.size(); ++b) bb[b + 1] = bb[b] + E->buckets[b].n_bins;
		c->n_fine = bb.back();
		if ((rc = c->bin_base.upload(bb.data(), bb.size(), c->stream))) return rc;
		std::vector<unsigned> cb(E->buckets.size() + 1, 0);
		for (size_t b = 0; b < E->buckets.size(); ++b) cb[b + 1] = cb[b] + (E->buckets[b].kind == 1 ? (E->buckets[b].iso_off & 0xFFFFu) : 0u) + 1u;
		c->n_cell_groups = cb.back();
		if ((rc = c->cell_base.upload(cb.data(), cb.size(), c->stream))) return rc;
		std::vector<unsigned> jb(E->buckets.size() + 1, 0);
		for (size_t b = 0; b <= E->buckets.size(); ++b) jb[b] = E->jg_base[b] + cb[b];
		c->n_junction_groups = jb.back();
		const unsigned long long none = 0;
		if ((rc = c->jg_keys.upload(E->jg_keys.empty() ? &none : (const unsigned long long *)E->jg_keys.data(), std::max<size_t>(E->jg_keys.size(), 1), c->stream))) return rc;
		if ((rc = c->jg_base.upload(E->jg_base.data(), E->jg_base.size(), c->stream))) return rc;
		if ((rc = c->jgroup_base.upload(jb.data(), jb.size(), c->stream))) return rc;
	}
	if ((rc = upload_strand_ranks(c))) return rc;
	HIP_TRY(hipStreamSynchronize(c->stream));
	mark("events: group bases, strand ranks");
	return LSQ_OK;
} LSQ_API_CATCH

int lsq_count(lsq_ctx *c) LSQ_API_TRY {
	if (!c) return fail(LSQ_E_ARG, "null context");
	if (!c->E) return fail(LSQ_E_STATE, "lsq_events_upload must come first");
	HIP_TRY(hipSetDevice(c->device));
	for (int m = 0; m < c->E->n_methods; ++m) if (!c->reads[m].present) return fail(LSQ_E_STATE, "reads of method %d were not uploaded", m);
#ifdef LSQ_DEV
	if (const char *e = getenv("LSQ_ABLATE")) c->dev_ablate = (unsigned)atoi(e); else c->dev_ablate = 0;
	if (const char *e = getenv("LSQ_GRID_MULT")) { const int v = atoi(e); if (v >= 1 && v <= 64) c->opt_grid_mult = v; }
#endif
	int rc = run_count(c);
	if (rc) return rc;
	for (bool &f : c->overflow_logged) f = false;
	if (c->has_host && (rc = host_count(c))) return rc;
	c->counted = true;
	c->solved = false;
	c->counts_external = false;
	return LSQ_OK;
// ... 399 lines not shown
	c->em.small_places = n_small_places; c->em.places = n_places;
	for (EmLane &l : c->em.lane) l.order_valid = false;
	c->em.opt_regroup = false;
	return LSQ_OK;
} LSQ_API_CATCH

int lsq_debug_last_em_launch(lsq_ctx *c, unsigned out[8]) LSQ_API_TRY {
	if (!c || !out) return fail(LSQ_E_ARG, "null argument");
	if (!c->E) return fail(LSQ_E_STATE, "lsq_events_upload must come first");
	HIP_TRY(hipSetDevice(c->device));
	{ int rc = sync_all(c); if (rc) return rc; }
	const EmLaunch &last = c->em.last;
	unsigned split = last.lean;
	if (last.form == EM_FORM_QUAD_FLAT3 || last.form == EM_FORM_QUAD_FLAT4) {
		uint32_t w = 0;
		HIP_TRY(hipMemcpy(&w, c->em.split.p + last.split_word, sizeof w, hipMemcpyDeviceToHost));
		split = std::min<unsigned>(w, last.lean);
	}
	out[0] = last.form; out[1] = last.lean; out[2] = split; out[3] = last.general;
	out[4] = last.learnt ? 1u : 0u; out[5] = last.cap; out[6] = last.regrouped ? 1u : 0u; out[7] = last.lane;
	return LSQ_OK;
} LSQ_API_CATCH

int lsq_ctx_set_option(lsq_ctx *c, const char *name, double value) LSQ_API_TRY {
	if (!c || !name) return fail(LSQ_E_ARG, "null argument");
	const std::string n(name);
	if (n == "grid_multiplier") {
		if (!(value >= 0 && value <= 64)) return fail(LSQ_E_ARG, "grid_multiplier must lie in 0..64 (0 = automatic)");
		c->opt_grid_mult = value;
		for (auto &r : c->reads) r.wg_grid = 0;
	} else if (n == "exception_capacity") {
		if (!(value >= 0 && value <= 4e9)) return fail(LSQ_E_ARG, "exception_capacity must lie in 0..4e9 (0 = automatic)");
		c->opt_exc_cap = (size_t)value;
	} else if (n == "snap_shares") {
		c->opt_snap_shares = value != 0;
		for (auto &r : c->reads) r.wg_grid = 0;
	} else if (n == "share_weighted" || n == "share_cost_two_block" || n == "share_cost_parked" || n == "share_cost_visit" || n == "share_taper" || n == "share_cost_hot") {
		if (!(value >= 0 && value <= 1e6)) return fail(LSQ_E_ARG, "%s must lie in 0..1e6", name);
		if (n == "share_weighted") c->opt_share_weighted = value != 0;
		else if (n == "share_cost_two_block") c->opt_share_cost_p2 = value;
		else if (n == "share_cost_parked") c->opt_share_cost_park = value;
		else if (n == "share_cost_visit") c->opt_share_cost_visit = value;
		else if (n == "share_cost_hot") c->opt_share_cost_hot = value;
		else c->opt_share_taper = value;
		for (auto &r : c->reads) r.wg_grid = 0;
	} else if (n == "sam_skip_flags") {
		if (!(value >= 0 && value <= 65535)) return fail(LSQ_E_ARG, "sam_skip_flags must lie in 0..65535");
		c->opt_sam_skip_flags = (unsigned)value;
	} else if (n == "sam_min_mapq") {
		if (!(value >= 0 && value <= 256)) return fail(LSQ_E_ARG, "sam_min_mapq must lie in 0..256");
		c->opt_sam_min_mapq = (unsigned)value;
	} else if (n == "bam_verify") {
		if (!(value == 0 || value == 1)) return fail(LSQ_E_ARG, "bam_verify must be 0 or 1");
		c->opt_bam_verify = value == 1;
	} else if (n == "compact_pools") {
		c->opt_compact_pools = value != 0;
	} else if (n == "workgroups_per_cu") {
		if (!(value >= -1 && value <= 32)) return fail(LSQ_E_ARG, "workgroups_per_cu must lie in -1..32 (-1 = automatic, 0 = as many as fit)");
		c->opt_wg_per_cu = (int)value;
		c->occ_lds_bytes = 0;
	} else if (n == "reads_per_look") {
		if (!(value == 0 || value == 4 || value == 8)) return fail(LSQ_E_ARG, "reads_per_look must be 0 (automatic), 4 or 8");
		c->opt_reads_per_look = (int)value;
	} else if (n == "count_streams") {
		{ int rc = sync_all(c); if (rc) return rc; }
		c->opt_two_count_streams = value >= 2;
// ... 66 lines not shown
```

### lesseq_amd/csrc/lsq_device.hpp

```cpp
#pragma once
#include <hip/hip_runtime.h>

#include <algorithm>
#include <cmath>
#include <cstring>
#include <memory>
#include <numeric>
#include <string>
#include <thread>
#include <type_traits>
#include <vector>

#include "lsq_internal.hpp"

using namespace lsq;

#define HIP_TRY(expr)                                                                          \
	do {                                                                                       \
		hipError_t _e = (expr);                                                                \
		if (_e != hipSuccess) return fail(LSQ_E_DEVICE, "%s: %s", #expr, hipGetErrorString(_e)); \
	} while (0)


#ifndef LSQ_P1_PAD
// ... 43 lines not shown
template <class T>
struct DevView { T *p = nullptr; size_t n = 0; };

template <int N>
struct PhaseClock {
	hipEvent_t ev[N + 1] = {};
	~PhaseClock() { for (hipEvent_t e : ev) if (e) (void)hipEventDestroy(e); }
	int make() { for (hipEvent_t &e : ev) HIP_TRY(hipEventCreate(&e)); return LSQ_OK; }
	hipError_t mark(int k, hipStream_t st) { return hipEventRecord(ev[k], st); }
	hipError_t ms(int k, float *out) { return hipEventElapsedTime(out, ev[k], ev[k + 1]); }
};

inline unsigned grid_for(unsigned long long items, unsigned per_block) {
	return (unsigned)std::max<unsigned long long>(1, (items + per_block - 1) / per_block);
}
inline unsigned grid_for(int n_cu, unsigned long long items, unsigned per_block, unsigned per_cu) {
	const unsigned long long want = (items + per_block - 1) / per_block, cap = (unsigned long long)n_cu * per_cu;
	return (unsigned)std::max<unsigned long long>(1, std::min(want, cap));
}

struct RouteChrom {
	unsigned loc_first, loc_nb;
	int loc_base;
	unsigned cov0, cov1, clu0, clu1;
	unsigned pad;
};
static_assert(sizeof(RouteChrom) == 32, "RouteChrom is staged in LDS as two 16-byte words");

struct VisitRec {
	BucketDesc d;
	unsigned long long bs, be;
	unsigned long long p1o, p1n, p2o, p2n;
	unsigned b, next;
	unsigned pad[2];
};
static_assert(sizeof(VisitRec) == 128, "VisitRec is read as 32 dwords");
struct WgPlan {
	unsigned long long s_begin, s_end;
	VisitRec first;
};
static_assert(sizeof(WgPlan) == 144, "WgPlan layout");

struct IngestPass {
	const char *name = nullptr;
	hipEvent_t ev[2] = {nullptr, nullptr};
	unsigned long long bytes = 0;
	float ms = 0;
	bool clocked = false;
};

struct MethodReads {
	DevBuf<ExcEntry> exc;
	size_t exc_cap = 0;
	bool present = false;
	uint64_t n_retained = 0, n_retained_blocks = 0, total_slots = 0;
	uint64_t lib_report[5] = {0, 0, 0, 0, 0};
	DevBuf<int32_t> p1, p2, pn_se;
	bool compact = false;
	uint64_t n1_reads = 0, n2_reads = 0;
	DevBuf<uint8_t> p1_strand, p2_strand, pn_strand;
	DevBuf<uint32_t> p1_line, p2_line, pn_line, pn_blk_off, pn_nblk, pn_bucket;
	DevBuf<unsigned long long> p1_off, p2_off, pn_off, pnb_off, slot_off;
	double skew = 1.0;
	bool named = false;
	DevBuf<char> names;
	DevBuf<unsigned long long> name_off;
	DevBuf<unsigned> wg_first;
	DevBuf<unsigned long long> wg_cut;
	DevBuf<WgPlan> wg_plan;
	std::vector<VisitRec> visits_host;
	std::vector<unsigned long long> slot_off_host;
	DevBuf<VisitRec> visits;
	std::vector<unsigned long long> plan_n1, plan_n2;
	std::vector<unsigned long long> plan_seg_x;
	std::vector<unsigned char> plan_seg_kind;
	std::vector<unsigned> plan_seg_looks, plan_seg_first;
	std::vector<unsigned> plan_park1, plan_park2;
	std::vector<unsigned> next_packed_host;
	unsigned long long wg_grid = 0;
};

}

enum EmForm : unsigned { EM_FORM_NONE = 0, EM_FORM_QUAD = 1, EM_FORM_QUAD_CAPPED = 2, EM_FORM_HEAD_TAIL = 3, EM_FORM_QUAD_FLAT3 = 4, EM_FORM_QUAD_FLAT4 = 5 };
enum : unsigned { EM_SPLIT_NONE = 2, EM_SPLIT_KEPT = 3, EM_SPLIT_WORDS = 4 };
struct EmLane {
	lsq::DevBuf<uint32_t> order;
	bool order_valid = false;
	unsigned age = 0;
	lsq::DevBuf<uint32_t> tail_u32;
	lsq::DevBuf<uint8_t> tail_flag;
	lsq::DevBuf<double> tail_f64;
};
struct EmLaunch {
	unsigned form = EM_FORM_NONE, lean = 0, general = 0, cap = 0, lane = 0, split_word = EM_SPLIT_NONE;
// ... 53 lines not shown
	hipEvent_t evt0 = nullptr, evt1 = nullptr;
	hipEvent_t evf0[LSQ_MAX_METHODS] = {}, evf1[LSQ_MAX_METHODS] = {};
	int fast_launched = 0;
	int occ_p1w = 0;
	int opt_reads_per_look = 0;
	unsigned last_reads_per_look = 4, last_wg_per_cu = 0;
	unsigned occ_lds_bytes = 0; int occ_blocks = 0;
	bool time_events = false;
	bool count_timed = false, solve_timed = false;
	lsq_events *E = nullptr;
	DevBuf<BucketDesc> buckets;
	DevBuf<uint8_t> images, strand_rank, dK;
	DevBuf<TieRec> ties;
	DevBuf<uint32_t> cls_base, iso_base, gene_name_off;
	DevBuf<char> gene_names;
	DevBuf<uint32_t> pack_cls, pack_iso, pack_ev;
	EmState em;
	BootState boot;
	DevBuf<double> G, theta2[2], logll2[2];
	DevBuf<uint32_t> iters2[2];
	DevBuf<uint8_t> flags2[2];
	DevView<double> theta, logll;
	DevView<uint32_t> iters;
	DevView<uint8_t> flags;
	DevBuf<uint32_t> fim_start_base, fim_mat_base, fim_starts;
	DevBuf<double> fim, fim_var;
	size_t fim_starts_total = 0, fim_mat_total = 0;
	bool fim_uploaded = false, fim_done = false;
	DevBuf<unsigned long long> counters;
	DevView<unsigned long long> cnt, bases, dbg;
	DevBuf<unsigned long long> wg_trace;
	unsigned long long wg_trace_n = 0, wg_trace_workers = 0;
	DevView<unsigned> exc_count;
	DevBuf<RouteChrom> route_chrom;
	DevBuf<int2> cov;
	DevBuf<int4> clu;
	DevBuf<uint2> loc;
	unsigned loc_shift = 10;
	DevBuf<unsigned> bin_base;
	size_t n_fine = 0;
	DevBuf<unsigned> cell_base;
	size_t n_cell_groups = 0;
	DevBuf<unsigned long long> jg_keys;
	DevBuf<unsigned> jg_base, jgroup_base;
	size_t n_junction_groups = 0;
	unsigned n_chrom_tables = 0;
	double opt_grid_mult = 0;
	size_t opt_exc_cap = 0;
	bool opt_compact_pools = true;
	bool opt_recount = false;
	unsigned opt_cleanup_grid = 0;
	bool overflow_logged[LSQ_MAX_METHODS] = {};
	bool opt_snap_shares = true;
	bool opt_share_weighted = true;
	double opt_share_cost_p2 = 4.3;
	double opt_share_cost_park = 9.0;
	double opt_share_cost_visit = 7000.0;
	double opt_share_cost_hot = 0.5;
	double opt_share_taper = 0;
	unsigned dev_ablate = 0;
	DevBuf<unsigned char> recount_args;
	std::vector<unsigned char> recount_args_host;
	MethodReads reads[LSQ_MAX_METHODS];
	bool counted = false, solved = false;
	bool counts_external = false;
	double em_band = 1E-11;
	bool has_fast = false, has_generic = false, has_host = false;
	uint64_t host_genes = 0, host_reads = 0;
	std::map<size_t, std::vector<unsigned short>> host_seq;
	float count_ms = 0, solve_ms = 0;
	float mrf_h2d_ms = 0, mrf_parse_ms = 0;
	unsigned parse_tiles_handed = 0, parse_lines_listed = 0, parse_all_slow = 0;
	unsigned opt_sam_skip_flags = 0x904u, opt_sam_min_mapq = 0u;
	bool opt_bam_verify = false;
	unsigned sam_lines_listed = 0, sam_all_slow = 0;
	unsigned long long bam_blocks = 0, bam_blocks_repaired = 0;
	unsigned char *pin_buf[2] = {nullptr, nullptr};
	hipEvent_t pin_ev[2] = {nullptr, nullptr};
	IngestPass ing_pass[LSQ_INGEST_PASS_MAX];
	int ing_n = 0, ing_reported = 0;
};

struct lsq_text {
// ... 24 lines not shown
```

### lesseq_amd/csrc/lsq_ingest.hip

```cpp
#include "lsq_ingest.hpp"
#include "lsq_text.hpp"

namespace {

struct IngestRaw {
	unsigned long long n_reads;
	const unsigned long long *blk_off;
	const unsigned *line_no;
	const int *blk_start, *blk_end;
	const unsigned short *blk_chrom;
	const unsigned char *blk_strand;
};

#ifndef LSQ_RAW_WAVES
#define LSQ_RAW_WAVES 8
#endif
template <bool STRANDED, class... Lib>
__global__ void __launch_bounds__(256) __attribute__((amdgpu_waves_per_eu(LSQ_RAW_WAVES))) lsq_route_raw_kernel(RouteTables T, IngestRaw R, RouteOut O, Lib... lib_arg) {
	__shared__ RouteChrom chrom_lds[ROUTE_CHROM_LDS];
	const RouteChrom *chroms = route_stage_chroms(T, chrom_lds);
	const unsigned long long gsz = (unsigned long long)gridDim.x * blockDim.x;
	LocProbe P;
	P.chrom = -1; P.bin = 0;
	if constexpr (!STRANDED) {
		for (unsigned long long i = (unsigned long long)blockIdx.x * blockDim.x + threadIdx.x; i < R.n_reads; i += gsz) {
			const unsigned long long b0 = R.blk_off[i], b1 = R.blk_off[i + 1];
			ReadAcc A;
			ReadBig B;
			A.init();
			for (unsigned long long j = b0; j < b1; ++j) {
				const unsigned c = R.blk_chrom[j];
				if (c >= T.n_chrom) continue;
				const int bs = R.blk_start[j], be = R.blk_end[j];
				if (!route_covered(T, chroms[c], (int)c, bs, be, P)) continue;
// ... 120 lines not shown
	}
}

constexpr unsigned PIECE = 16384;
__global__ void __launch_bounds__(256) lsq_piece_count_kernel(const unsigned *part_cnt, unsigned n_entries, unsigned *piece_cnt) {
	const unsigned e = blockIdx.x * blockDim.x + threadIdx.x;
	if (e < n_entries) piece_cnt[e] = (part_cnt[e] + PIECE - 1u) / PIECE;
}
__global__ void __launch_bounds__(256) lsq_piece_expand_kernel(const unsigned *part_cnt, const unsigned long long *piece_off, unsigned n_entries, uint4 *pieces) {
	const unsigned e = blockIdx.x * blockDim.x + threadIdx.x;
	if (e >= n_entries) return;
	const unsigned n = part_cnt[e];
	const unsigned long long o = piece_off[e];
	const unsigned np = (n + PIECE - 1u) / PIECE;
	for (unsigned q = 0; q < np; ++q) pieces[o + q] = make_uint4(e, q * PIECE, min(PIECE, n - q * PIECE), np == 1u ? 1u : 0u);
}

struct GroupTables {
	const BucketDesc *buckets;
	const unsigned char *images;
	const unsigned *cell_base;
	const unsigned long long *jg_keys; const unsigned *jg_base, *jgroup_base;
	unsigned B;
	unsigned lds_img, lds_keys;
};

struct GroupArgs {
	const uint4 *pieces;
	const unsigned long long *off1, *off2;
	const uint4 *part1, *part2;
	unsigned *fine1, *fine2;
	unsigned *cnt1, *cnt2;
	unsigned *park1, *park2;
};

__global__ void __launch_bounds__(256) lsq_group_classify_kernel(GroupTables T, GroupArgs A) {
	extern __shared__ __align__(16) unsigned char glds[];
	const uint4 pc = A.pieces[blockIdx.x];
	const unsigned pool = pc.x >= T.B ? 1u : 0u, b = pc.x - pool * T.B;
	const BucketDesc d = T.buckets[b];
	const unsigned n_cells = d.kind == 1u ? (d.iso_off & 0xFFFFu) : 0u;
	const unsigned k0 = T.jg_base[b], k1 = T.jg_base[b + 1];
	const unsigned n_groups = pool ? (k1 - k0) + n_cells + 1u : n_cells + 1u;
	const unsigned gbase = pool ? T.jgroup_base[b] : T.cell_base[b];
	unsigned char *img = glds;
	unsigned long long *keys = reinterpret_cast<unsigned long long *>(glds + T.lds_img);
	unsigned *hist = reinterpret_cast<unsigned *>(glds + T.lds_img + T.lds_keys), *park = hist + n_groups;
	if (d.kind == 1u) for (unsigned q = threadIdx.x; q < d.img_bytes / 16u; q += 256u) reinterpret_cast<uint4 *>(img)[q] = reinterpret_cast<const uint4 *>(T.images + d.img_off)[q];
	if (pool) for (unsigned q = threadIdx.x; q < k1 - k0; q += 256u) keys[q] = T.jg_keys[k0 + q];
	for (unsigned q = threadIdx.x; q < 2u * n_groups; q += 256u) hist[q] = 0;
	__syncthreads();
	const uint4 *bins = reinterpret_cast<const uint4 *>(img);
	const lsq::Cell *cells = reinterpret_cast<const lsq::Cell *>(img + d.seg_off);
	const lsq::CellX *cellx = reinterpret_cast<const lsq::CellX *>(img + d.seg_off + 16u * (d.iso_off >> 16));
	const lsq::FastRec *recs = reinterpret_cast<const lsq::FastRec *>(img + d.ev_off);
	const unsigned long long first = (pool ? A.off2[b] : A.off1[b]) + pc.y;
	for (unsigned r = threadIdx.x; r < pc.z; r += 256u) {
		int s0, e0, s1 = 0;
		if (pool) { const uint4 v = A.part2[2ull * (first + r)]; s0 = (int)v.x; e0 = (int)v.y; s1 = (int)v.z; }
		else { const uint4 v = A.part1[first + r]; s0 = (int)v.x; e0 = (int)v.y; }
		unsigned cell = 0, g = pool ? (k1 - k0) : 0u, looks_est = 0;
		if (d.kind == 1u) {
			const int rel = s0 - d.lo;
			const unsigned bin = rel <= 0 ? 0u : min((unsigned)rel >> d.shift, d.n_bins - 1u);
			const uint4 br = bins[bin];
			const int p = s0;
			cell = (br.x & 0xFFFFu) + (unsigned)(p >= (int)br.y) + (unsigned)(p >= (int)br.z) + (unsigned)(p >= (int)br.w);
			if (p >= (int)br.w) while (cell + 1u < n_cells && p >= cells[cell + 1u].lo) ++cell;
			if (!(cell < n_cells && cells[cell].lo <= p && p < cells[cell].hi)) cell = n_cells;
			bool in_junction_group = false;
			if (pool) {
				unsigned jg = k1 - k0;
				if (cell < n_cells && (e0 == cells[cell].e1 || e0 == cells[cell].e2)) {
					const unsigned long long want = lsq::jg_key(cell, e0 == cells[cell].e1 ? 0u : 1u, s1);
					unsigned lo_k = 0, hi_k = k1 - k0;
					while (lo_k < hi_k) { const unsigned mid = (lo_k + hi_k) >> 1; if (keys[mid] < want) lo_k = mid + 1; else hi_k = mid; }
					if (lo_k < k1 - k0 && keys[lo_k] == want) jg = lo_k;
				}
				in_junction_group = jg < k1 - k0;
				g = in_junction_group ? jg : (k1 - k0) + cell;
			} else g = cell;
			bool parks = cell == n_cells, one_event = false;
			if (!parks && !in_junction_group) {
				const lsq::Cell cw = cells[cell];
				const unsigned fl = cellx[cell].flags;
				const int len = e0 - s0;
				const bool both = (fl & lsq::CELLX_BOTH) != 0u;
				const bool near_free = (fl & lsq::CELLX_NEAR_NO_ABUT) != 0u, far_free = (fl & lsq::CELLX_FAR_NO_ABUT) != 0u;
				const bool near_done = e0 <= cw.e1 || (near_free && 50 * (e0 - cw.e1) >= len), far_done = e0 <= cw.e2 || (far_free && 50 * (e0 - cw.e2) >= len);
				if (!pool) { parks = both ? !(near_done && far_done) : e0 > cw.e2; one_event = !both || near_done || far_done; }
				else if (cellx[cell].info == lsq::CELL_INFO_EMPTY) parks = false;
				else parks = both ? (e0 == cw.e1 || e0 == cw.e2 || (e0 > cw.e1 && !near_free) || (e0 > cw.e2 && !far_free)) : e0 > cw.e2;
			}
			if (parks) {
				unsigned looks = 1;
				if (!one_event) {
					looks = 0;
					for (unsigned i = br.x >> 16; i < d.n_events && looks < 64u; ++i) {
						++looks;
						const lsq::FastRec &fr = recs[i];
						if (!(fr.seg[0] <= p && (p > fr.ge || (fr.meta & lsq::FAST_FLAG_OVERLAPS_NEXT) != 0u))) break;
					}
				}
				looks_est = looks;
			}
		}
		(pool ? A.fine2 : A.fine1)[first + r] = gbase + g;
		atomicAdd(&hist[g], 1u);
		if (looks_est) atomicAdd(&park[g], looks_est);
	}
	__syncthreads();
	unsigned *cnt = pool ? A.cnt2 : A.cnt1, *pk = pool ? A.park2 : A.park1;
	for (unsigned q = threadIdx.x; q < n_groups; q += 256u) {
		const unsigned c = hist[q], l = park[q];
		if (pc.w) { if (c) cnt[gbase + q] = c; if (l) pk[gbase + q] = l; }
		else { if (c) atomicAdd(&cnt[gbase + q], c); if (l) atomicAdd(&pk[gbase + q], l); }
// ... 11 lines not shown
}

template <bool COMPACT> __device__ inline void pool_store(void *out, const unsigned long long at, const int2 r, const int base) {
	if (COMPACT) reinterpret_cast<unsigned *>(out)[at] = (unsigned)(r.x - base) | ((unsigned)(r.y - r.x) << lsq::COMPACT_OFF_BITS);
	else reinterpret_cast<int2 *>(out)[at] = r;
}
template <bool COMPACT> __device__ inline void pool_store(void *out, const unsigned long long at, const int4 r, const int base) {
	if (COMPACT) reinterpret_cast<uint2 *>(out)[at] = make_uint2((unsigned)(r.x - base) | ((unsigned)(r.y - r.x) << lsq::COMPACT_OFF_BITS),
	                                                              (unsigned)(r.z - r.y) | ((unsigned)(r.w - r.z) << lsq::COMPACT_OFF_BITS));
	else reinterpret_cast<int4 *>(out)[at] = r;
}

struct PlaceArgs {
	const uint4 *pieces;
	const unsigned long long *part_off1, *part_off2;
	const uint4 *part1, *part2;
	const unsigned *fine1, *fine2;
	const unsigned long long *off1, *off2;
	unsigned *cur1, *cur2;
	const BucketDesc *buckets;
	const unsigned *cell_base, *jg_base, *jgroup_base;
	unsigned B, compact;
	void *p1; unsigned char *p1_strand; unsigned *p1_line;
	void *p2; unsigned char *p2_strand; unsigned *p2_line;
};

__global__ void __launch_bounds__(256) lsq_group_place_kernel(PlaceArgs A) {
	extern __shared__ __align__(16) unsigned char glds[];
	unsigned *cur = reinterpret_cast<unsigned *>(glds);
	const uint4 pc = A.pieces[blockIdx.x];
	const unsigned pool = pc.x >= A.B ? 1u : 0u, b = pc.x - pool * A.B;
	const BucketDesc &d = A.buckets[b];
	const unsigned n_cells = d.kind == 1u ? (d.iso_off & 0xFFFFu) : 0u;
	const unsigned n_groups = pool ? (A.jg_base[b + 1] - A.jg_base[b]) + n_cells + 1u : n_cells + 1u;
	const unsigned gbase = pool ? A.jgroup_base[b] : A.cell_base[b];
	const unsigned long long first = (pool ? A.part_off2[b] : A.part_off1[b]) + pc.y;
	const unsigned *fine = (pool ? A.fine2 : A.fine1) + first;
	unsigned *goff = cur + n_groups;
	const unsigned long long *off = pool ? A.off2 : A.off1;
	const unsigned long long off0 = off[gbase];
	for (unsigned q = threadIdx.x; q < n_groups; q += 256u) { cur[q] = 0; goff[q] = (unsigned)(off[gbase + q] - off0); }
	__syncthreads();
	if (!pc.w) {
		for (unsigned r = threadIdx.x; r < pc.z; r += 256u) atomicAdd(&cur[fine[r] - gbase], 1u);
		__syncthreads();
		unsigned *gcur = pool ? A.cur2 : A.cur1;
		for (unsigned q = threadIdx.x; q < n_groups; q += 256u) { const unsigned c = cur[q]; cur[q] = c ? atomicAdd(&gcur[gbase + q], c) : 0u; }
		__syncthreads();
	}
	const int base = d.lo - lsq::COMPACT_BIAS;
	for (unsigned r0 = threadIdx.x; r0 < pc.z; r0 += 1024u) {
		unsigned g[4]; uint4 v[4], x[4]; bool on[4];
#pragma unroll
		for (int u = 0; u < 4; ++u) {
			const unsigned r = r0 + 256u * (unsigned)u;
			on[u] = r < pc.z;
			g[u] = on[u] ? fine[r] - gbase : 0u;
			if (!pool) { v[u] = on[u] ? A.part1[first + r] : make_uint4(0, 0, 0, 0); x[u] = v[u]; }
			else { v[u] = on[u] ? A.part2[2ull * (first + r)] : make_uint4(0, 0, 0, 0); x[u] = on[u] ? A.part2[2ull * (first + r) + 1] : make_uint4(0, 0, 0, 0); }
		}
#pragma unroll
		for (int u = 0; u < 4; ++u) {
			if (!on[u]) continue;
			const unsigned long long w = off0 + goff[g[u]] + atomicAdd(&cur[g[u]], 1u);
			if (!pool) {
				const int2 rec = make_int2((int)v[u].x, (int)v[u].y);
				if (A.compact) pool_store<true>(A.p1, w, rec, base); else pool_store<false>(A.p1, w, rec, base);
// ... 30 lines not shown
__global__ void __launch_bounds__(256) lsq_ingest_pad_kernel(const BucketDesc *buckets, const unsigned *cell_base, const unsigned *jgroup_base, unsigned n_buckets,
                                                             unsigned n_groups1, unsigned n_groups2, const unsigned *cnt1, const unsigned long long *off1,
                                                             const unsigned *cnt2, const unsigned long long *off2, const unsigned char *images,
                                                             void *p1, void *p2, unsigned compact, unsigned char *p1_strand, unsigned *p1_line,
                                                             unsigned char *p2_strand, unsigned *p2_line) {
	for (unsigned t = blockIdx.x * blockDim.x + threadIdx.x; t < n_groups1 + n_groups2; t += gridDim.x * blockDim.x) {
		const bool one = t < n_groups1;
		const unsigned g = one ? t : t - n_groups1;
		const unsigned n = one ? cnt1[g] : cnt2[g], gp = one ? P1_GROUP_PAD : P2_GROUP_PAD, pad = ((n + gp - 1u) & ~(gp - 1u)) - n;
		if (!pad) continue;
		const unsigned *gbase = one ? cell_base : jgroup_base;
		unsigned lo_b = 0, hi_b = n_buckets;
		while (hi_b - lo_b > 1) { const unsigned mid = (lo_b + hi_b) >> 1; if (gbase[mid] <= g) lo_b = mid; else hi_b = mid; }
		const BucketDesc &d = buckets[lo_b];
		const int base = d.lo - lsq::COMPACT_BIAS;
		if (!one) {
			for (unsigned q = 0; q < pad; ++q) {
				const unsigned long long w = off2[g] + n + q;
				if (compact) reinterpret_cast<uint2 *>(p2)[w] = make_uint2((unsigned)lsq::COMPACT_BIAS, 0u);
				else reinterpret_cast<int4 *>(p2)[w] = make_int4(d.lo, d.lo, d.lo, d.lo);
				p2_strand[w] = 0; p2_line[w] = 0;
			}
			continue;
		}
		const unsigned cell = g - cell_base[lo_b];
		int at = d.lo;
		if (d.kind == 1u && cell < (d.iso_off & 0xFFFFu)) at = reinterpret_cast<const lsq::Cell *>(images + d.img_off + d.seg_off)[cell].lo;
		if (compact && !lsq::compact_block_fits((long long)at - base, 1)) at = base;
		for (unsigned q = 0; q < pad; ++q) {
			const unsigned long long w = off1[g] + n + q;
			if (compact) reinterpret_cast<unsigned *>(p1)[w] = (unsigned)(at - base);
			else reinterpret_cast<int2 *>(p1)[w] = make_int2(at, at);
			p1_strand[w] = 0; p1_line[w] = 0;
		}
	}
}

static const char *const INGEST_STAGE_NAMES[LSQ_INGEST_STAGES] = {
	"newline_count", "route", "partition_count", "partition_scatter", "group_classify", "group_offsets", "group_place"};

void stages_collect(lsq_ctx *c) {
	for (int k = 0; k < c->ing_n; ++k) {
		IngestPass &p = c->ing_pass[k];
		float ms = 0;
		if (p.clocked && p.ev[0] && p.ev[1] && hipEventElapsedTime(&ms, p.ev[0], p.ev[1]) == hipSuccess) p.ms = ms;
	}
	(void)hipGetLastError();
}

}

unsigned lsq::route_lib(const lsq_ctx *c) {
	const lsq_events &E = *c->E;
	return E.stranded() ? route_lib_word(E.library == LSQ_LIBRARY_REVERSE, (unsigned)E.strand_plus, (unsigned)E.strand_minus) : 0u;
}
RouteTables lsq::route_tables(lsq_ctx *c) {
	RouteTables T{};
	T.chrom = c->route_chrom.p; T.cov = c->cov.p; T.clu = c->clu.p; T.loc = c->loc.p; T.loc_shift = c->loc_shift; T.n_chrom = c->n_chrom_tables;
	return T;
}

int lsq::ingest_device(lsq_ctx *c, int method, Front &F) {
	HostStopwatch SW;
	const lsq_events &E = *c->E;
	MethodReads &mr = c->reads[method];
	mr.present = false;
// ... 4 lines not shown
	hipStream_t st = c->stream;
	int rc;
	if ((rc = ensure_lanes(c))) return rc;
	HIP_TRY(hipStreamSynchronize(c->stream_em2[0]));
	HIP_TRY(hipStreamSynchronize(c->stream_em2[1]));
	HIP_TRY(hipStreamSynchronize(c->stream_count2[0]));
	HIP_TRY(hipStreamSynchronize(c->stream_count2[1]));
	const size_t FC = c->n_cell_groups;
	const size_t FJ = c->n_junction_groups;
	const size_t n_cnt = 10 * (size_t)B + 3 * (FC + FJ);
	const size_t n_tot = 8 + ROUTE_LIB_WORD0 + (E.stranded() ? 8 * (size_t)ROUTE_LIB_SLOTS : 0);
	std::vector<unsigned long long> lib_places(E.stranded() ? 8 * (size_t)ROUTE_LIB_SLOTS : 0);
	DevBuf<unsigned> d_key, d_cnt, d_fine1, d_fine2;
	DevBuf<int4> d_rec;
	DevBuf<unsigned long long> d_tot, d_part_off1, d_part_off2, d_piece_off, d_off1, d_off2;
	DevBuf<uint4> d_nb_ent, d_part1, d_part2, d_pieces;
	DevBuf<int2> d_nb_blk;
	ScanScratch SS;
	if ((rc = d_key.alloc(n)) || (rc = d_rec.alloc(n)) || (rc = d_cnt.alloc(n_cnt)) || (rc = d_tot.alloc(n_tot)) || (rc = d_part_off1.alloc(B + 1)) || (rc = d_part_off2.alloc(B + 1)) ||
	    (rc = d_piece_off.alloc(2 * (size_t)B + 1)) || (rc = d_off1.alloc(FC + 1)) || (rc = d_off2.alloc(FJ + 1)) || (rc = SS.reserve(std::max<size_t>(std::max(FC, FJ), 2 * (size_t)B)))) return rc;
	unsigned *part_cnt = d_cnt.p, *part_cur = part_cnt + 2 * (size_t)B, *piece_cnt = part_cur + 2 * (size_t)B;
	unsigned *cntn = piece_cnt + 2 * (size_t)B, *cntnb = cntn + B, *curn = cntnb + B, *curnb = curn + B;
	unsigned *cnt1 = curnb + B, *cnt2 = cnt1 + FC, *cur1 = cnt2 + FJ, *cur2 = cur1 + FC, *park1 = cur2 + FJ, *park2 = park1 + FC;
	if ((rc = mr.p1_off.alloc(B + 1)) || (rc = mr.p2_off.alloc(B + 1)) || (rc = mr.pn_off.alloc(B + 1)) || (rc = mr.pnb_off.alloc(B + 1)) || (rc = mr.slot_off.alloc(B + 1))) return rc;
	const RouteTables T = route_tables(c);
	const size_t part_lds = 8 * (size_t)B;
	const bool part_in_lds = part_lds <= 128 * 1024 && getenv("LSQ_PART_NO_LDS") == nullptr;
	size_t img_max = 16, jg_max = 0, groups_max = 1;
	for (unsigned b = 0; b < B; ++b) {
		const BucketDesc &d = E.buckets[b];
		const size_t n_cells = d.kind == 1u ? (d.iso_off & 0xFFFFu) : 0u, n_jg = E.jg_base[b + 1] - E.jg_base[b];
		if (d.kind == 1u) img_max = std::max<size_t>(img_max, (d.img_bytes + 15u) & ~15u);
		jg_max = std::max(jg_max, n_jg);
		groups_max = std::max(groups_max, n_jg + n_cells + 1);
	}
	const size_t keys_lds = (8 * jg_max + 15) & ~(size_t)15, group_lds = img_max + keys_lds + 8 * groups_max, place_lds = 8 * groups_max;
	if (group_lds > 160 * 1024) return fail(LSQ_E_UNSUPPORTED, "a bucket's tables and group counters exceed the CU's LDS");
	if (part_in_lds && part_lds > 48 * 1024) {
		HIP_TRY(hipFuncSetAttribute((const void *)lsq_part_hist_kernel<true>, hipFuncAttributeMaxDynamicSharedMemorySize, (int)part_lds));
		HIP_TRY(hipFuncSetAttribute((const void *)lsq_part_scatter_kernel<true>, hipFuncAttributeMaxDynamicSharedMemorySize, (int)part_lds));
	}
	if (group_lds > 48 * 1024) HIP_TRY(hipFuncSetAttribute((const void *)lsq_group_classify_kernel, hipFuncAttributeMaxDynamicSharedMemorySize, (int)group_lds));
	if (place_lds > 48 * 1024) HIP_TRY(hipFuncSetAttribute((const void *)lsq_group_place_kernel, hipFuncAttributeMaxDynamicSharedMemorySize, (int)place_lds));
	const unsigned part_grid = (unsigned)std::max<unsigned long long>(1, std::min<unsigned long long>(n / 131072ull, 2ull * (unsigned)c->n_cu));
	SW.mark("ingest: allocations");
	if (!c->ing_n) (void)stage_entry(c, INGEST_STAGE_NAMES[0]);
	(void)stage_entry(c, F.stage);
	for (int s = 2; s < LSQ_INGEST_STAGES; ++s) (void)stage_entry(c, INGEST_STAGE_NAMES[s]);
	c->ing_reported = c->ing_n;

	unsigned compact = c->opt_compact_pools ? 1u : 0u;
	unsigned long long nb_cap = std::max<unsigned long long>(4096, n / 32), nbb_cap = 4 * nb_cap;
	if (const char *e = getenv("LSQ_NB_LIST")) { const long long v = atoll(e); if (v > 0) { nb_cap = (unsigned long long)v; nbb_cap = 2 * nb_cap; } }
	unsigned long long tot[8] = {0, 0, 0, 0, 0, 0, 0, 0}, nb_tot[8] = {0, 0, 0, 0, 0, 0, 0, 0}, sums[5] = {0, 0, 0, 0, 0};
	for (;;) {
		if (d_nb_ent.n < nb_cap) { if ((rc = d_nb_ent.alloc((size_t)nb_cap))) return rc; }
		if (d_nb_blk.n < nbb_cap) { if ((rc = d_nb_blk.alloc((size_t)nbb_cap))) return rc; }
		HIP_TRY(hipMemsetAsync(d_cnt.p, 0, std::max<size_t>(n_cnt, 1) * 4, st));
		HIP_TRY(hipMemsetAsync(d_tot.p, 0, n_tot * 8, st));
		RouteOut O{};
		O.key = d_key.p; O.rec = d_rec.p; O.nb_tot = d_tot.p + 8; O.nb_cap = nb_cap; O.nbb_cap = nbb_cap; O.nb_ent = d_nb_ent.p; O.nb_blk = d_nb_blk.p;
		O.cntn = cntn; O.cntnb = cntnb; O.compact = compact;
		if (n) {
			StageClock k(c, st, F.stage);
			if ((rc = F.launch(T, O, st))) return rc;
			k.end(F.in_bytes + 20ull * n);
		}
// ... 21 lines not shown
		SW.mark("ingest: route + partition counts");
		if (F.settle && (rc = F.settle(st))) { if (rc == LSQ_RETRY) continue; return rc; }
		const bool go_wide = compact && tot[3] * 16 > tot[4] + tot[5] + tot[3];
		const bool list_short = nb_tot[0] > nb_cap || nb_tot[1] > nbb_cap;
		if (go_wide || list_short) {
			if (go_wide) compact = 0;
			if (list_short) { nb_cap = std::max(nb_cap, nb_tot[0]); nbb_cap = std::max(nbb_cap, nb_tot[1]); }
			continue;
		}
		break;
	}
	if (nb_tot[2]) return fail(LSQ_E_RANGE, "a read covers 2^18 or more bases or keeps more than %d separate blocks: outside the device tables' range", INGEST_MAX_BLOCKS);
	if (sums[4] > 0xFFFFFFF0ull) return fail(LSQ_E_RANGE, "too many blocks in multi-block reads");
	const size_t n1p = (size_t)sums[0], n2p = (size_t)sums[1], n_pieces = (size_t)sums[2], nn = (size_t)sums[3], nnb = (size_t)sums[4];
	if (n_pieces > 0x7FFFFFFFull) return fail(LSQ_E_RANGE, "too many partition pieces");
	if ((rc = d_part1.alloc(n1p)) || (rc = d_part2.alloc(2 * n2p)) || (rc = d_fine1.alloc(n1p)) || (rc = d_fine2.alloc(n2p)) || (rc = d_pieces.alloc(n_pieces))) return rc;
	SW.mark("ingest: partition buffers");
	{
		StageClock k(c, st, "partition_scatter");
		PartArgs A{};
		A.key = d_key.p; A.rec = d_rec.p; A.n = n; A.B = B; A.off1 = d_part_off1.p; A.off2 = d_part_off2.p; A.cursor = part_cur;
		A.part1 = d_part1.p; A.part2 = d_part2.p; A.line_no = F.line_no; A.first_line = F.first_line;
		if (n1p + n2p) {
			if (part_in_lds) hipLaunchKernelGGL(lsq_part_scatter_kernel<true>, dim3(part_grid), dim3(PART_WG), part_lds, st, A);
			else hipLaunchKernelGGL(lsq_part_scatter_kernel<false>, dim3(part_grid), dim3(PART_WG), 0, st, A);
		}
		hipLaunchKernelGGL(lsq_piece_expand_kernel, dim3(2 * B / 256 + 1), dim3(256), 0, st, (const unsigned *)part_cnt, (const unsigned long long *)d_piece_off.p, 2 * B, d_pieces.p);
		HIP_TRY(hipGetLastError());
		k.end(8ull * n + 16ull * (n1p + n2p) + 16ull * n1p + 32ull * n2p);
	}
	GroupArgs GA{};
	GA.pieces = d_pieces.p; GA.off1 = d_part_off1.p; GA.off2 = d_part_off2.p; GA.part1 = d_part1.p; GA.part2 = d_part2.p;
	GA.fine1 = d_fine1.p; GA.fine2 = d_fine2.p; GA.cnt1 = cnt1; GA.cnt2 = cnt2; GA.park1 = park1; GA.park2 = park2;
	if (n_pieces) {
		StageClock k(c, st, "group_classify");
		GroupTables GT{};
		GT.buckets = c->buckets.p; GT.images = c->images.p; GT.cell_base = c->cell_base.p; GT.jg_keys = c->jg_keys.p; GT.jg_base = c->jg_base.p; GT.jgroup_base = c->jgroup_base.p;
		GT.B = B; GT.lds_img = (unsigned)img_max; GT.lds_keys = (unsigned)keys_lds;
		hipLaunchKernelGGL(lsq_group_classify_kernel, dim3((unsigned)n_pieces), dim3(256), group_lds, st, GT, GA);
		HIP_TRY(hipGetLastError());
		k.end(16ull * n1p + 32ull * n2p + 4ull * (n1p + n2p));
	}
	unsigned long long psum[2] = {0, 0};
	{
		StageClock k(c, st, "group_offsets");
		if ((rc = device_scan<P1_GROUP_PAD>(SS, cnt1, FC, d_off1.p, st)) || (rc = device_scan<P2_GROUP_PAD>(SS, cnt2, FJ, d_off2.p, st))) return rc;
		hipLaunchKernelGGL(lsq_ingest_offsets_kernel, dim3(B / 256 + 1), dim3(256), 0, st, c->cell_base.p, c->jgroup_base.p, B, d_off1.p, d_off2.p, mr.pn_off.p,
		                   mr.p1_off.p, mr.p2_off.p, mr.slot_off.p);
		HIP_TRY(hipGetLastError());
		k.end(12ull * (FC + FJ));
	}
	SW.mark("ingest: partition + group launches");
	HIP_TRY(hipMemcpyAsync(&psum[0], mr.p1_off.p + B, 8, hipMemcpyDeviceToHost, st));
	HIP_TRY(hipMemcpyAsync(&psum[1], mr.p2_off.p + B, 8, hipMemcpyDeviceToHost, st));
	HIP_TRY(hipStreamSynchronize(st));
	SW.mark("ingest: partition + groups");
	const size_t n1 = (size_t)psum[0], n2 = (size_t)psum[1];
	mr.compact = compact != 0;
	mr.n1_reads = tot[4]; mr.n2_reads = tot[5];
	if ((rc = mr.p1.alloc(mr.compact ? ((n1 + 3) & ~(size_t)3) : 2 * n1)) || (rc = mr.p1_strand.alloc(n1)) || (rc = mr.p1_line.alloc(n1))) return rc;
	if ((rc = mr.p2.alloc(mr.compact ? 2 * ((n2 + 1) & ~(size_t)1) : 4 * n2)) || (rc = mr.p2_strand.alloc(n2)) || (rc = mr.p2_line.alloc(n2))) return rc;
	if ((rc = mr.pn_se.alloc(2 * nnb)) || (rc = mr.pn_blk_off.alloc(nn)) || (rc = mr.pn_nblk.alloc(nn)) || (rc = mr.pn_strand.alloc(nn)) ||
	    (rc = mr.pn_line.alloc(nn)) || (rc = mr.pn_bucket.alloc(nn))) return rc;
	{
		StageClock k(c, st, "group_place");
		if (n_pieces) {
// ... 9 lines not shown
			hipLaunchKernelGGL(lsq_ingest_pad_kernel, dim3(pgrid), dim3(256), 0, st, c->buckets.p, c->cell_base.p, c->jgroup_base.p, B, (unsigned)FC, (unsigned)FJ,
			                   (const unsigned *)cnt1, (const unsigned long long *)d_off1.p, (const unsigned *)cnt2, (const unsigned long long *)d_off2.p, c->images.p,
			                   (void *)mr.p1.p, (void *)mr.p2.p, compact, mr.p1_strand.p, mr.p1_line.p, mr.p2_strand.p, mr.p2_line.p);
		}
		if (nn) {
			NbOut N{};
			N.ent = d_nb_ent.p; N.blk = d_nb_blk.p; N.n_ent = nb_tot[0]; N.pn_off = mr.pn_off.p; N.pnb_off = mr.pnb_off.p; N.curn = curn; N.curnb = curnb;
			N.pn_blk_off = mr.pn_blk_off.p; N.pn_nblk = mr.pn_nblk.p; N.pn_line = mr.pn_line.p; N.pn_bucket = mr.pn_bucket.p; N.pn_strand = mr.pn_strand.p;
			N.pn_se = reinterpret_cast<int2 *>(mr.pn_se.p); N.line_no = F.line_no; N.first_line = F.first_line;
			const unsigned ngrid = (unsigned)std::min<unsigned long long>((nb_tot[0] + 255) / 256, (unsigned long long)c->n_cu * 16);
			hipLaunchKernelGGL(lsq_ingest_nblock_kernel, dim3(ngrid), dim3(256), 0, st, N);
		}
		HIP_TRY(hipGetLastError());
		k.end(16ull * n1p + 32ull * n2p + 4ull * (n1p + n2p) + (mr.compact ? 4ull : 8ull) * (n1 + 2 * n2) + 5ull * (n1 + n2));
	}
	{
		size_t want = std::max<size_t>(65536, (n1 + n2) / 4);
		if (c->opt_exc_cap) want = c->opt_exc_cap;
		if (mr.exc_cap != want) {
			if ((rc = mr.exc.alloc(LSQ_COUNTER_SETS * want))) return rc;
			mr.exc_cap = want;
		}
	}
	if ((rc = upload_strand_ranks(c))) return rc;
	mr.n_retained = tot[0];
	for (int q = 0; q < 5; ++q) {
		mr.lib_report[q] = 0;
		for (size_t k = 0; k < lib_places.size(); k += 8) mr.lib_report[q] += lib_places[k + q];
	}
	mr.n_retained_blocks = tot[1] + nb_tot[1];
	mr.total_slots = n1 + n2 + nn;
	mr.wg_grid = 0;
	{
		std::vector<unsigned long long> so(B + 1, 0), o1(B + 1, 0), o2(B + 1, 0), f1(FC + 1, 0), f2(FJ + 1, 0);
		std::vector<unsigned> park(FC + FJ + 1, 0);
		HIP_TRY(hipMemcpyAsync(so.data(), mr.slot_off.p, (B + 1) * sizeof(unsigned long long), hipMemcpyDeviceToHost, st));
		HIP_TRY(hipMemcpyAsync(o1.data(), mr.p1_off.p, (B + 1) * sizeof(unsigned long long), hipMemcpyDeviceToHost, st));
		HIP_TRY(hipMemcpyAsync(o2.data(), mr.p2_off.p, (B + 1) * sizeof(unsigned long long), hipMemcpyDeviceToHost, st));
		HIP_TRY(hipMemcpyAsync(f1.data(), d_off1.p, (FC + 1) * sizeof(unsigned long long), hipMemcpyDeviceToHost, st));
		HIP_TRY(hipMemcpyAsync(f2.data(), d_off2.p, (FJ + 1) * sizeof(unsigned long long), hipMemcpyDeviceToHost, st));
		if (FC + FJ) HIP_TRY(hipMemcpyAsync(park.data(), park1, (FC + FJ) * sizeof(unsigned), hipMemcpyDeviceToHost, st));
		HIP_TRY(hipStreamSynchronize(st));
		SW.mark("ingest: place + read-back");
		stages_collect(c);
		unsigned long long mx = 0;
		for (unsigned b = 0; b < B; ++b) mx = std::max(mx, so[b + 1] - so[b]);
		mr.slot_off_host = so;
		mr.skew = (B && mr.total_slots) ? (double)mx * (double)B / (double)mr.total_slots : 1.0;
		{
			mr.plan_n1.resize(B); mr.plan_n2.resize(B); mr.plan_park1.assign(B, 0); mr.plan_park2.assign(B, 0);
			mr.plan_seg_x.clear(); mr.plan_seg_kind.clear(); mr.plan_seg_looks.clear(); mr.plan_seg_first.assign(B + 1, 0);
			size_t g1 = 0, g2 = 0;
			for (unsigned b = 0; b < B; ++b) {
				const unsigned n_cg = (E.buckets[b].kind == 1 ? (E.buckets[b].iso_off & 0xFFFFu) : 0u) + 1u, n_jg = (E.jg_base[b + 1] - E.jg_base[b]) + n_cg;
				const unsigned long long n1 = o1[b + 1] - o1[b], n2 = o2[b + 1] - o2[b], ns = so[b + 1] - so[b];
				mr.plan_n1[b] = n1; mr.plan_n2[b] = n2;
				mr.plan_seg_first[b] = (unsigned)mr.plan_seg_kind.size();
				const bool visited = E.buckets[b].kind == 1u && ns != 0;
				if (visited) {
					for (unsigned q = 0; q < n_cg && g1 + q < FC; ++q) {
						const unsigned long long a = f1[g1 + q], e = f1[g1 + q + 1];
						mr.plan_park1[b] += park[g1 + q];
						if (e > a) { mr.plan_seg_x.push_back(so[b] + (a - o1[b])); mr.plan_seg_kind.push_back(0); mr.plan_seg_looks.push_back(park[g1 + q]); }
					}
					for (unsigned q = 0; q < n_jg && g2 + q < FJ; ++q) {
						const unsigned long long a = f2[g2 + q], e = f2[g2 + q + 1];
						mr.plan_park2[b] += park[FC + g2 + q];
						if (e > a) { mr.plan_seg_x.push_back(so[b] + n1 + (a - o2[b])); mr.plan_seg_kind.push_back(1); mr.plan_seg_looks.push_back(park[FC + g2 + q]); }
					}
					if (ns > n1 + n2) { mr.plan_seg_x.push_back(so[b] + n1 + n2); mr.plan_seg_kind.push_back(2); mr.plan_seg_looks.push_back(0); }
				} else if (ns) { mr.plan_seg_x.push_back(so[b]); mr.plan_seg_kind.push_back(2); mr.plan_seg_looks.push_back(0); }
				g1 += n_cg; g2 += n_jg;
			}
			mr.plan_seg_first[B] = (unsigned)mr.plan_seg_kind.size();
			mr.plan_seg_x.push_back(B ? so[B] : 0);
		}
		std::vector<VisitRec> vis(B + 1);
		mr.next_packed_host.assign(B + 1, B);
		memset(vis.data(), 0, vis.size() * sizeof(VisitRec));
		unsigned next = B;
		for (unsigned b = B; b-- > 0;) {
			VisitRec &v = vis[b];
			v.d = E.buckets[b];
			v.bs = so[b]; v.be = so[b + 1];
			v.p1o = o1[b]; v.p1n = o1[b + 1] - o1[b]; v.p2o = o2[b]; v.p2n = o2[b + 1] - o2[b];
			v.b = b; v.next = next;
			if (E.buckets[b].kind == 1u && so[b + 1] > so[b]) next = b;
			mr.next_packed_host[b] = next;
		}
		vis[B].b = B; vis[B].next = B; vis[B].bs = vis[B].be = mr.total_slots;
		if ((rc = mr.visits.upload(vis.data(), vis.size(), st))) return rc;
		mr.visits_host = vis;
		HIP_TRY(hipStreamSynchronize(st));
	}
	mr.present = true;
	c->counted = c->solved = false;
	SW.mark("ingest: plan, visit records");
	return LSQ_OK;
}

namespace {

void front_of_raw(lsq_ctx *c, const IngestRaw &Rw, unsigned long long n_blocks, Front &F) {
	F.n = Rw.n_reads; F.line_no = Rw.line_no; F.first_line = 0;
	F.in_bytes = 12ull * Rw.n_reads + 11ull * n_blocks;
	F.launch = [c, Rw](const RouteTables &T, const RouteOut &O, hipStream_t st) -> int {
		const unsigned igrid = (unsigned)std::min<unsigned long long>((Rw.n_reads + 255) / 256 + 1, (unsigned long long)c->n_cu * 16);
		if (c->E->stranded()) hipLaunchKernelGGL((lsq_route_raw_kernel<true, unsigned>), dim3(igrid), dim3(256), 0, st, T, Rw, O, route_lib(c));
		else hipLaunchKernelGGL(lsq_route_raw_kernel<false>, dim3(igrid), dim3(256), 0, st, T, Rw, O);
		HIP_TRY(hipGetLastError());
		return LSQ_OK;
	};
}

}

extern "C" {

// ... 52 lines not shown
const char *lsq_last_ingest_stage_name(const lsq_ctx *c, int stage) {
	if (stage < 0 || stage >= lsq_last_ingest_stage_count(c)) return nullptr;
	return c && c->ing_reported ? c->ing_pass[stage].name : lsq_ingest_stage_name(stage);
}
int lsq_last_ingest_stages(const lsq_ctx *c, float *ms, uint64_t *bytes, int capacity) LSQ_API_TRY {
	if (!c) return fail(LSQ_E_ARG, "null context");
	for (int k = 0; k < lsq_last_ingest_stage_count(c) && k < capacity; ++k) {
		if (ms) ms[k] = c->ing_reported ? c->ing_pass[k].ms : 0.0f;
		if (bytes) bytes[k] = c->ing_reported ? c->ing_pass[k].bytes : 0;
	}
	return LSQ_OK;
} LSQ_API_CATCH

uint64_t lsq_reads_retained(const lsq_ctx *c, int method) { return (c && method >= 0 && method < LSQ_MAX_METHODS) ? c->reads[method].n_retained : 0; }
uint64_t lsq_reads_pooled(const lsq_ctx *c, int method) {
	if (!c || method < 0 || method >= LSQ_MAX_METHODS) return 0;
	const MethodReads &mr = c->reads[method];
	return mr.n1_reads + mr.n2_reads + mr.pn_line.n;
}
uint64_t lsq_reads_pooled_blocks(const lsq_ctx *c, int method) {
	if (!c || method < 0 || method >= LSQ_MAX_METHODS) return 0;
	const MethodReads &mr = c->reads[method];
	return mr.n1_reads + 2 * mr.n2_reads + mr.pn_se.n / 2;
}
int lsq_last_library_report(const lsq_ctx *c, int method, uint64_t out[5]) LSQ_API_TRY {
	if (!c || !out || method < 0 || method >= LSQ_MAX_METHODS) return fail(LSQ_E_ARG, "bad context or method");
	if (!c->E || !c->E->stranded()) return fail(LSQ_E_STATE, "the events of this context are unstranded: there is no library report");
	if (!c->reads[method].present) return fail(LSQ_E_STATE, "no reads uploaded for method %d", method);
	for (int q = 0; q < 5; ++q) out[q] = c->reads[method].lib_report[q];
	return LSQ_OK;
} LSQ_API_CATCH
uint64_t lsq_reads_retained_blocks(const lsq_ctx *c, int method) { return (c && method >= 0 && method < LSQ_MAX_METHODS) ? c->reads[method].n_retained_blocks : 0; }

int lsq_reads_pool_format(const lsq_ctx *c, int method, int *compact, uint64_t *pool_bytes, uint64_t *pool_reads) LSQ_API_TRY {
	if (!c || method < 0 || method >= LSQ_MAX_METHODS) return fail(LSQ_E_ARG, "bad context or method");
	const MethodReads &mr = c->reads[method];
	if (!mr.present) return fail(LSQ_E_STATE, "no reads uploaded for method %d", method);
	if (compact) *compact = mr.compact ? 1 : 0;
	if (pool_bytes) *pool_bytes = 4ull * (mr.p1.n + mr.p2.n + mr.pn_se.n);
	if (pool_reads) { pool_reads[0] = mr.n1_reads; pool_reads[1] = mr.n2_reads; pool_reads[2] = mr.pn_line.n; }
	return LSQ_OK;
} LSQ_API_CATCH

}
```

### lesseq_amd/csrc/lsq_replay.hip

```cpp
#include "lsq_device.hpp"
#include <atomic>


namespace {

struct HostRead {
	int start, end;
	unsigned line;
	unsigned matched;
	unsigned short cls;
	unsigned char strand;
};

struct HostWalk {
	long long pos = 0; int it = 0; bool found = false; uint64_t mask = 0; long long matched = 0;
	bool block(const lsq::Event &e, long long a, long long b) {
		while (it < e.N) {
			const long long sx = e.seg_s[(size_t)it], sy = e.seg_e[(size_t)it];
			if (!(sx < b)) break;
			pos = std::max(pos, sx);
			if (a >= pos && a < sy) {
				if (found && a > pos) break;
				found = true;
				mask |= 1ull << it;
				pos = std::min(sy, b);
				matched += pos - a;
				if (b < sy) { a = b; break; }
				a = (b == sy) ? b : sy;
			} else if (pos > sx && pos < sy) {
				break;
			}
			++it;
		}
// ... 402 lines not shown
	if (n_replayed) *n_replayed = n;
	return rc;
} LSQ_API_CATCH

int lsq_host_evaluated(const lsq_ctx *c, uint64_t *n_genes, uint64_t *n_reads) LSQ_API_TRY {
	if (!c) return fail(LSQ_E_ARG, "null context");
	if (!c->counted) return fail(LSQ_E_STATE, "lsq_count must come first");
	if (n_genes) *n_genes = c->has_host ? c->host_genes : 0;
	if (n_reads) *n_reads = c->has_host ? c->host_reads : 0;
	return LSQ_OK;
} LSQ_API_CATCH

int lsq_debug_check_pool_layout(lsq_ctx *c, int method, unsigned long long *out) LSQ_API_TRY {
	if (!c || !c->E || !out || method < 0 || method >= c->E->n_methods) return fail(LSQ_E_ARG, "bad argument");
	HIP_TRY(hipSetDevice(c->device));
	{ int rc = lsq::sync_all(c); if (rc) return rc; }
	const lsq_events &E = *c->E;
	const lsq::MethodReads &mr = c->reads[method];
	if (!mr.present) return fail(LSQ_E_STATE, "no reads uploaded for method %d", method);
	for (int q = 0; q < 6; ++q) out[q] = 0;
	for (size_t b = 0; b < E.buckets.size(); ++b) {
		const lsq::BucketDesc &d = E.buckets[b];
		BucketReads R;
		{ int rc = fetch_bucket(mr, b, d.lo, R); if (rc) return rc; }
		const lsq::Cell *cells = d.kind == 1 ? reinterpret_cast<const lsq::Cell *>(E.images.data() + d.img_off + d.seg_off) : nullptr;
		const unsigned n_cells = d.kind == 1 ? (d.iso_off & 0xFFFFu) : 0u;
		auto cell_of = [&](int p) -> long {
			for (unsigned q = 0; q < n_cells; ++q) if (cells[q].lo <= p && p < cells[q].hi) return (long)q;
			return -1;
		};
		const size_t n1 = R.p1_line.size(), n2 = R.p2_line.size();
		if ((n1 % P1_GROUP_PAD) || (n2 % P2_GROUP_PAD)) return fail(LSQ_E_STATE, "bucket %zu: pool slices of %zu and %zu records are not whole groups of %u / %u", b, n1, n2, P1_GROUP_PAD, P2_GROUP_PAD);
		out[0] += n1; out[3] += n2;
		for (size_t q = 0; q < n1; q += P1_GROUP_PAD) {
			long first = -2;
			bool mixed = false;
			for (size_t k = q; k < q + P1_GROUP_PAD; ++k) {
				const int s = R.p1[2 * k], e = R.p1[2 * k + 1];
				if (s == e) { ++out[1]; continue; }
				const long cl = cell_of(s);
				if (first == -2) first = cl; else if (cl != first) mixed = true;
			}
			if (mixed) ++out[2];
		}
		const uint64_t *k0 = E.jg_keys.data() + E.jg_base[b], *k1 = E.jg_keys.data() + E.jg_base[b + 1];
		auto group_of = [&](const int32_t *r) -> long {
			const long cl = cell_of(r[0]);
			if (cl < 0 || (r[1] != cells[cl].e1 && r[1] != cells[cl].e2)) return -1;
			const uint64_t want = lsq::jg_key((uint32_t)cl, r[1] == cells[cl].e1 ? 0u : 1u, r[2]);
			const uint64_t *it = std::lower_bound(k0, k1, want);
			return (it != k1 && *it == want) ? (long)(it - k0) : -1;
		};
		for (size_t q = 0; q < n2; q += P2_GROUP_PAD) {
			const int32_t *ra = &R.p2[4 * q];
			const bool ea = ra[0] == ra[1];
			const long ga = ea ? -1 : group_of(ra);
			bool bad = false;
			out[4] += ea ? 1u : 0u;
			for (size_t k = q + 1; k < q + P2_GROUP_PAD; ++k) {
				const int32_t *rb = &R.p2[4 * k];
				const bool eb = rb[0] == rb[1];
				out[4] += eb ? 1u : 0u;
				if (ea) bad = bad || !eb;
				else if (ga >= 0 && !eb && group_of(rb) != ga) bad = true;
				else if (ga < 0 && !eb && (group_of(rb) >= 0 || cell_of(rb[0]) != cell_of(ra[0]))) bad = true;
			}
			if (bad) ++out[5];
		}
	}
	if (out[0] - out[1] != mr.n1_reads || out[3] - out[4] != mr.n2_reads)
		return fail(LSQ_E_STATE, "the pools hold %llu + %llu reads, the ingest counted %llu + %llu", out[0] - out[1], out[3] - out[4],
		            (unsigned long long)mr.n1_reads, (unsigned long long)mr.n2_reads);
	return LSQ_OK;
} LSQ_API_CATCH

}
```

Before: 837.4 billion reads/s.

## Route hard reads to precomputed look records instead of in-kernel parking rings

```diff
diff --git a/include/lesseq_hip.h b/include/lesseq_hip.h
--- a/include/lesseq_hip.h
+++ b/include/lesseq_hip.h
@@ -144,6 +144,8 @@
 int lsq_count(lsq_ctx *c);
 int lsq_count_status(lsq_ctx *c, uint32_t *exceptions, uint32_t *recounted);
 int lsq_count_launch_info(lsq_ctx *c, uint32_t *reads_per_look, uint32_t *workgroups_per_cu);
+int lsq_count_guard_entries(lsq_ctx *c, uint32_t *guards);
+int lsq_reads_hard_looks(const lsq_ctx *c, int method, uint64_t out[6]);
 int lsq_host_evaluated(const lsq_ctx *c, uint64_t *n_genes, uint64_t *n_reads);
 int lsq_ctx_set_option(lsq_ctx *c, const char *name, double value);
 
diff --git a/lesseq_amd/api.py b/lesseq_amd/api.py
--- a/lesseq_amd/api.py
+++ b/lesseq_amd/api.py
@@ -415,6 +415,21 @@
         check(lib.lsq_count_status(self.h, e, r))
         return list(e)[:self.events.n_methods], list(r)[:self.events.n_methods]
 
+    def guard_entries(self):
+        M = max(self.events.n_methods, 1)
+        g = (u32 * M)()
+        lib.lsq_count_guard_entries.argtypes = [vp, P(u32)]
+        lib.lsq_count_guard_entries.restype = C.c_int
+        check(lib.lsq_count_guard_entries(self.h, g))
+        return list(g)[:self.events.n_methods]
+
+    def hard_looks(self, method):
+        out = (u64 * 6)()
+        lib.lsq_reads_hard_looks.argtypes = [vp, C.c_int, P(u64)]
+        lib.lsq_reads_hard_looks.restype = C.c_int
+        check(lib.lsq_reads_hard_looks(self.h, method, out))
+        return tuple(int(x) for x in out)
+
     def counts_device_words(self):
         return int(lib.lsq_counts_device_words(self.h))
 
diff --git a/lesseq_amd/csrc/lsq_count.hip b/lesseq_amd/csrc/lsq_count.hip
--- a/lesseq_amd/csrc/lsq_count.hip
+++ b/lesseq_amd/csrc/lsq_count.hip
@@ -1,4 +1,5 @@
 #include "lsq_device.hpp"
+#include "lsq_settle.hpp"
 #include <hip/hip_ext.h>
 
 namespace {
@@ -45,6 +46,8 @@
 	unsigned exc_cap;
 	unsigned long long *dbg;
 	unsigned long long *bar;
+	unsigned long long *guard;
+	const lsq::LookRec *looks;
 };
 
 __device__ inline int2 unpack_one_block(const unsigned a, const int base) {
@@ -262,6 +265,7 @@
 	unsigned ablate;
 	unsigned long long *dbg;
 	unsigned long long *trace;
+	unsigned long long *guard;
 };
 
 __device__ inline void emit_exception(const FastCtx &C, unsigned r, unsigned i, unsigned scan) {
@@ -273,6 +277,13 @@
 		e.ev_pool_scan = i | (C.pool << 29) | (scan << 31);
 		C.exc[slot] = e;
 	}
+}
+
+__device__ inline void emit_guard(const FastCtx &C, const unsigned r, const int p) {
+	const int brel = p - C.lo;
+	const unsigned bin = brel <= 0 ? 0u : min((unsigned)brel >> C.shift, C.n_bins - 1u);
+	emit_exception(C, r, reinterpret_cast<const unsigned *>(C.bins)[4u * bin] >> 16, 1u);
+	atomicAdd(C.guard, 1ull);
 }
 
 constexpr unsigned PARK_EVENT_UNKNOWN = 0x7FFFFFFFu;
@@ -377,9 +388,9 @@
 	}
 };
 
-template <int NB, bool PACKED2 = false>
-__device__ inline void walk_parked(const FastCtx &C, Ring<(NB == 1 || PACKED2) ? 1 : 2> &R, const bool to_empty, const int base = 0) {
-	constexpr int RW = (NB == 1 || PACKED2) ? 1 : 2;
+template <int NB>
+__device__ inline void walk_parked(const FastCtx &C, Ring<NB> &R, const bool to_empty) {
+	constexpr int RW = NB;
 	const unsigned lane = threadIdx.x & 63u;
 	wave_sync_lds();
 #pragma unroll 1
@@ -399,13 +410,6 @@
 		if (RW == 1) { e0.z &= ~PARK_ONE_EVENT; } else { e1.x &= ~PARK_ONE_EVENT; }
 		if (NB == 1) {
 			rd = make_int4((int)e0.x, (int)e0.y, (int)e0.x, (int)e0.y); i = e0.z; rel = e0.w;
-			const int brel = rd.x - C.lo;
-			const unsigned bin = brel <= 0 ? 0u : min((unsigned)brel >> C.shift, C.n_bins - 1u);
-			const unsigned first = reinterpret_cast<const unsigned *>(C.bins)[4u * bin] >> 16;
-			if (i == PARK_EVENT_UNKNOWN) { i = first; e0.z = first; }
-		}
-		else if (PACKED2) {
-			rd = unpack_two_block(e0.x, e0.y, base); i = e0.z; rel = e0.w;
 			const int brel = rd.x - C.lo;
 			const unsigned bin = brel <= 0 ? 0u : min((unsigned)brel >> C.shift, C.n_bins - 1u);
 			const unsigned first = reinterpret_cast<const unsigned *>(C.bins)[4u * bin] >> 16;
@@ -663,7 +667,7 @@
 
 template <int NR>
 __device__ inline void stream_pool1_compact(FastCtx &C, const uint4 *bins, const uint4 *cells, const uint4 *cellx, const unsigned n_cells, const BucketDesc &d,
-                                            const CountArgs &A, uint4 *queue, const void *pool, const unsigned long long g0, const unsigned long long g1) {
+                                            const CountArgs &A, const void *pool, const unsigned long long g0, const unsigned long long g1) {
 	static_assert(NR == 4 || NR == 8, "one or two 16-byte words of four compact records");
 	static_assert((unsigned)NR <= P1_GROUP_PAD, "a lane's records of a step lie in one cell group");
 	constexpr int CW = NR / 4;
@@ -685,8 +689,6 @@
 			nxt[cq] = make_uint4(v.x, v.y, v.z, v.w);
 		}
 	};
-	Ring<1> R;
-	R.q = queue;
 	const unsigned t_begin = min(wave * TILE, n);
 	if (t_begin < n) fetch(t_begin);
 	for (unsigned t = t_begin; t < n; t += WAVES * TILE) {
@@ -735,7 +737,7 @@
 		else { if (interior) decide(std::true_type{}, std::false_type{}); else decide(std::false_type{}, std::false_type{}); }
 		const unsigned s1 = cx.x & 0xFFFFu, s2 = cx.x >> 16;
 		if (!ABL(A, (1u | 16384u))) {
-			const unsigned acc2 = both ? accL : accL - accA;
+			const unsigned acc2 = both ? accA : accL - accA;
 			if (accA && s1 != CELL_NONE) atomicAdd(&C.hist[s1], ((unsigned long long)(accA >> 24) << 40) | (accA & 0xFFFFFFu));
 			if (acc2 && s2 != CELL_NONE) atomicAdd(&C.hist[s2], ((unsigned long long)(acc2 >> 24) << 40) | (acc2 & 0xFFFFFFu));
 		} else asm volatile("" ::"v"(accA), "v"(accL));
@@ -745,40 +747,23 @@
 			if (lane == 0) { atomicAdd(&A.dbg[12], 1ull); atomicAdd(&A.dbg[11], any_open ? 1ull : 0ull); }
 		}
 		if (__any(lane_open) && !ABL(A, 17u | 524288u)) {
-#pragma unroll
-			for (int h = 0; h < NR; h += 2) {
-				uint4 en[2];
-				unsigned open = 0;
-#pragma unroll
-				for (int j = h; j < h + 2; ++j) {
+			if (lane_open) {
+#pragma unroll
+				for (int j = 0; j < NR; ++j) {
 					const unsigned len = rec[j] >> lsq::COMPACT_OFF_BITS;
 					const int so = (int)(rec[j] & lsq::COMPACT_OFF_MASK), e = so + (int)len;
 					const unsigned idx = t + lane * (unsigned)NR + (unsigned)j, rel = idx - first_rel;
 					const bool in = idx < n && rel < n_rel;
-					const bool gone_near = both && (cx.z & CELLX_NEAR_NO_ABUT) != 0u && e > e1 && 50 * (e - e1) >= (int)len;
-					const bool gone_far = both && (cx.z & CELLX_FAR_NO_ABUT) != 0u && e > e2 && 50 * (e - e2) >= (int)len;
-					const bool done_near = e <= e1 || gone_near, done_far = e <= e2 || gone_far;
-					const bool op = in && len != 0u && !(both ? (done_near && done_far) : e <= e2);
-					open |= op ? 1u << (j - h) : 0u;
-					const unsigned hint = !has ? PARK_EVENT_UNKNOWN : (!both ? (cx.w | PARK_ONE_EVENT) :
-					                      (done_far ? (cx.w | PARK_ONE_EVENT) : (done_near ? ((cx.z & 0xFFFFu) | PARK_ONE_EVENT) : PARK_EVENT_UNKNOWN)));
-					en[j - h] = make_uint4((unsigned)(so + base), (unsigned)(so + base) + len, hint, rel);
-					if (ABL(A, 256u) && op) { atomicAdd(&A.dbg[5 + (has ? (both ? 2 : 1) : 0)], 1ull); atomicAdd(&A.dbg[0], 1ull); }
-				}
-				R.push2(open, lane, en[0], en[1]);
-				if (R.live() >= 64u) {
-					if (!ABL(A, 32u)) walk_parked<1, false>(C, R, false, base);
-					else R.head = R.tail;
+					if (in && len != 0u && !(e <= (both ? e1 : e2))) emit_guard(C, rel, so + base);
 				}
 			}
 		}
 	}
-	if (R.live() && !ABL(A, 32u)) walk_parked<1, false>(C, R, true, base);
 }
 
 template <int NR>
 __device__ inline void stream_pool2_compact(FastCtx &C, const uint4 *bins, const uint4 *cells, const uint4 *cellx, const unsigned n_cells, const BucketDesc &d,
-                                            const CountArgs &A, uint4 *queue, const void *pool, const unsigned long long g0, const unsigned long long g1) {
+                                            const CountArgs &A, const void *pool, const unsigned long long g0, const unsigned long long g1) {
 	static_assert((NR == 2 || NR == 4 || NR == 8) && (unsigned)NR <= P2_GROUP_PAD, "whole 16-byte words of two compact records, inside one junction group");
 	constexpr int CW = NR / 2;
 	constexpr unsigned TILE = 64u * NR;
@@ -799,8 +784,6 @@
 			nxt[cq] = make_uint4(v.x, v.y, v.z, v.w);
 		}
 	};
-	Ring<1> R;
-	R.q = queue;
 	const unsigned t_begin = min(wave * TILE, n);
 	if (t_begin < n) fetch(t_begin);
 	for (unsigned t = t_begin; t < n; t += WAVES * TILE) {
@@ -821,7 +804,6 @@
 		const unsigned bin = rel_p <= 0 ? 0u : ((unsigned)rel_p >> d.shift);
 		const uint4 br = bins[min(bin, d.n_bins - 1u)];
 		unsigned c1 = (br.x & 0xFFFFu) + (unsigned)(rd.x >= (int)br.y) + (unsigned)(rd.x >= (int)br.z) + (unsigned)(rd.x >= (int)br.w);
-		const unsigned evf = br.x >> 16;
 		if (__any(rd.x >= (int)br.w) && !ABL(A, 65536u)) {
 			while (c1 + 1u < n_cells && rd.x >= (int)cells[c1 + 1u].x) ++c1;
 		}
@@ -910,21 +892,45 @@
 			if (nB) atomicAdd(&C.hist[slotB], ((unsigned long long)nB << 40) | sB);
 		} else asm volatile("" ::"v"(nA), "v"(sA), "v"(nB), "v"(sB));
 		if (__any(any_park)) {
-			const unsigned hint0 = v1 ? (cx1.w | PARK_ONE_EVENT) : evf;
-#pragma unroll
-			for (int h = 0; h < NR; h += 2) {
-				const uint4 qa = make_uint4(ra[h], rb[h], h == 0 ? hint0 : PARK_EVENT_UNKNOWN, rel0 + (unsigned)h);
-				const uint4 qb = make_uint4(ra[h + 1], rb[h + 1], PARK_EVENT_UNKNOWN, rel0 + (unsigned)h + 1u);
-				if (ABL(A, 256u)) atomicAdd(&A.dbg[1], (park[h] ? 1ull : 0ull) + (park[h + 1] ? 1ull : 0ull));
-				R.push2((park[h] ? 1u : 0u) | (park[h + 1] ? 2u : 0u), lane, qa, qb);
-				if (R.live() >= 64u) {
-					if (!ABL(A, 32u)) walk_parked<2, true>(C, R, false, base);
-					else R.head = R.tail;
-				}
+			if (any_park) {
+#pragma unroll
+				for (int j = 0; j < NR; ++j)
+					if (park[j]) emit_guard(C, rel0 + (unsigned)j, (int)(ra[j] & lsq::COMPACT_OFF_MASK) + base);
 			}
 		}
 	}
-	if (R.live() && !ABL(A, 32u)) walk_parked<2, true>(C, R, true, base);
+}
+
+__device__ inline u32x4 looks_first(const lsq::LookRec *looks, const unsigned long long i0, const unsigned long long i1) {
+	global_words src = (global_words)looks;
+	const unsigned lane = threadIdx.x & 63u, wave = (unsigned)__builtin_amdgcn_readfirstlane((int)(threadIdx.x >> 6));
+	const unsigned n = (unsigned)(i1 - i0);
+	u32x4 v = {0u, 0u, 0u, 0u};
+	if (wave * 64u < n) v = src[i0 + min(wave * 64u + lane, n - 1u)];
+	return v;
+}
+template <int NB>
+__device__ inline void stream_looks(FastCtx &C, const CountArgs &A, const int base, const lsq::LookRec *looks, const unsigned long long pool_first,
+                                    const unsigned long long i0, const unsigned long long i1, const u32x4 first) {
+	C.pool = NB == 1 ? 0u : 1u;
+	C.slot0 = pool_first;
+	global_words src = (global_words)looks;
+	const unsigned lane = threadIdx.x & 63u, wave = (unsigned)__builtin_amdgcn_readfirstlane((int)(threadIdx.x >> 6));
+	const unsigned n = (unsigned)(i1 - i0);
+	const unsigned t_begin = min(wave * 64u, n);
+	u32x4 nxt = first;
+	for (unsigned t = t_begin; t < n; t += WAVES * 64u) {
+		const u32x4 cur = nxt;
+		if (t + WAVES * 64u < n) nxt = src[i0 + min(t + WAVES * 64u + lane, n - 1u)];
+		const bool on = t + lane < n;
+		if (ABL(C, 256u) && lane == 0) { atomicAdd(&C.dbg[2], 1ull); atomicAdd(&C.dbg[3], (unsigned long long)min(64u, n - t)); }
+		if (ABL(A, 512u)) { asm volatile("" ::"v"(cur.x), "v"(cur.y), "v"(cur.z), "v"(cur.w)); continue; }
+		int4 rd;
+		if (NB == 1) { const int2 r1 = unpack_one_block(cur.x, base); rd = make_int4(r1.x, r1.y, r1.x, r1.y); }
+		else rd = unpack_two_block(cur.x, cur.y, base);
+		const int total = NB == 1 ? rd.y - rd.x : (rd.y - rd.x) + (rd.w - rd.z);
+		(void)fast_trip<NB>(C, rd, total, cur.w, cur.z, on);
+	}
 }
 
 __device__ inline void global_add_merged(unsigned long long *cnt, unsigned long long *bases, bool want, const unsigned slot, const unsigned matched) {
@@ -1016,7 +1022,7 @@
 	} trace(ABL(A, 4194304u) ? A.wg_trace : nullptr);
 	if (blockIdx.x < A.n_workers) { pool_n_worker(A, A.n_pn, A.n_workers); return; }
 	const unsigned wg = blockIdx.x - A.n_workers, n_wg = gridDim.x - A.n_workers;
-	uint4 *wave_queue = reinterpret_cast<uint4 *>(lds + A.tables_lds_bytes) + (tid >> 6) * WAVE_QUEUE_WORDS;
+	uint4 *wave_queue = COMPACT ? nullptr : reinterpret_cast<uint4 *>(lds + A.tables_lds_bytes) + (tid >> 6) * WAVE_QUEUE_WORDS;
 	(void)n_wg;
 	typedef const lsq::VisitRec __attribute__((address_space(4))) *const_visit;
 	typedef const lsq::WgPlan __attribute__((address_space(4))) *const_plan;
@@ -1034,9 +1040,17 @@
 		d.img_off = vr->d.img_off; d.img_bytes = vr->d.img_bytes; d.n_events = vr->d.n_events; d.n_bins = vr->d.n_bins; d.lo = vr->d.lo; d.shift = vr->d.shift;
 		d.ev_off = vr->d.ev_off; d.seg_off = vr->d.seg_off; d.iso_off = vr->d.iso_off; d.hist_off = vr->d.hist_off; d.n_cls = vr->d.n_cls; d.cls_base = vr->d.cls_base;
 		d.ev_base = vr->d.ev_base; d.chrom_id = vr->d.chrom_id; d.kind = vr->d.kind; d.hi = vr->d.hi;
-		const unsigned long long be = vr->be, p1o = vr->p1o, n1 = vr->p1n, p2o = vr->p2o, n2 = vr->p2n;
-		const unsigned next = vr->next;
+		const unsigned long long be = vr->be, p1o = vr->p1o, n1 = vr->p1n, p2o = vr->p2o, n2 = vr->p2n, lko = vr->lko;
+		const unsigned next = vr->next, lk1 = vr->lk1n, lk2 = vr->lk2n;
 		unsigned char *buf = lds;
+		const unsigned long long l0 = (s_begin > bs ? s_begin : bs) - bs;
+		const unsigned long long l1 = (s_end < be ? s_end : be) - bs;
+		const unsigned long long n12 = n1 + n2, a1 = n12 + lk1, a2 = a1 + lk2;
+		const bool has_lk1 = COMPACT && l1 > n12 && l0 < a1, has_lk2 = COMPACT && l1 > a1 && l0 < a2;
+		const unsigned long long k1a = (l0 > n12 ? l0 : n12) - n12, k1b = (l1 < a1 ? l1 : a1) - n12, k2a = (l0 > a1 ? l0 : a1) - n12, k2b = (l1 < a2 ? l1 : a2) - n12;
+		u32x4 lkf1 = {0u, 0u, 0u, 0u}, lkf2 = {0u, 0u, 0u, 0u};
+		if (has_lk1) lkf1 = looks_first(A.looks + lko, k1a, k1b);
+		if (has_lk2) lkf2 = looks_first(A.looks + lko, k2a, k2b);
 		if (!first_visit) __syncthreads();
 		first_visit = false;
 		{
@@ -1060,16 +1074,19 @@
 		C.slot0 = 0; C.pool = 0;
 		C.exc = A.exc; C.exc_count = A.exc_count; C.exc_cap = A.exc_cap; C.ablate = A.ablate; C.dbg = A.dbg;
 		C.trace = (ABL(A, 4194304u) && A.wg_trace) ? A.wg_trace + 4u * blockIdx.x : nullptr;
-		const unsigned long long l0 = (s_begin > bs ? s_begin : bs) - bs;
-		const unsigned long long l1 = (s_end < be ? s_end : be) - bs;
+		C.guard = A.guard;
 		if (l0 < n1 && !ABL(A, 1024u)) {
-			if constexpr (COMPACT) stream_pool1_compact<2 * P1W>(C, bins, cells, cellx, n_cells, d, A, wave_queue, A.p1, p1o + l0, p1o + (l1 < n1 ? l1 : n1));
+			if constexpr (COMPACT) stream_pool1_compact<2 * P1W>(C, bins, cells, cellx, n_cells, d, A, A.p1, p1o + l0, p1o + (l1 < n1 ? l1 : n1));
 			else stream_pool_wide<2>(C, bins, cells, cellx, n_cells, d, A, wave_queue, reinterpret_cast<const uint4 *>(A.p1), p1o + l0, p1o + (l1 < n1 ? l1 : n1));
 		}
 		if (l1 > n1 && l0 < n1 + n2 && !ABL(A, 2048u)) {
 			const unsigned long long q0 = p2o + ((l0 > n1 ? l0 : n1) - n1), q1 = p2o + ((l1 < n1 + n2 ? l1 : n1 + n2) - n1);
-			if constexpr (COMPACT) stream_pool2_compact<(P1W == 4 ? LSQ_P2_COMPACT_WORDS_W5 : LSQ_P2_COMPACT_WORDS)>(C, bins, cells, cellx, n_cells, d, A, wave_queue, A.p2, q0, q1);
+			if constexpr (COMPACT) stream_pool2_compact<(P1W == 4 ? LSQ_P2_COMPACT_WORDS_W5 : LSQ_P2_COMPACT_WORDS)>(C, bins, cells, cellx, n_cells, d, A, A.p2, q0, q1);
 			else stream_pool_wide<1>(C, bins, cells, cellx, n_cells, d, A, wave_queue, reinterpret_cast<const uint4 *>(A.p2), q0, q1);
+		}
+		if constexpr (COMPACT) {
+			if (has_lk1 && !ABL(A, 32u)) stream_looks<1>(C, A, d.lo - lsq::COMPACT_BIAS, A.looks + lko, p1o, k1a, k1b, lkf1);
+			if (has_lk2 && !ABL(A, 32u)) stream_looks<2>(C, A, d.lo - lsq::COMPACT_BIAS, A.looks + lko, p2o, k2a, k2b, lkf2);
 		}
 		__syncthreads();
 		for (unsigned i = tid; i < d.n_cls; i += COUNT_BLOCK) {
@@ -1234,7 +1251,7 @@
 	for (size_t b = 0; b < B; ++b) if (visited_kind[b] && so[b + 1] > so[b] && bseg[b] < bseg[b + 1]) jump[bseg[b]] = cv;
 	for (size_t i = 0; i < S; ++i) {
 		const double len = (double)(x[i + 1] - x[i]);
-		dens[i] = kind[i] == 2 || len <= 0 ? d_rest : (kind[i] == 0 ? 1.0 : c2) + cw * (double)looks[i] / len + (len >= 8192.0 ? pc.hot : 0.0);
+		dens[i] = kind[i] == 2 || len <= 0 ? d_rest : (kind[i] == 3 ? cw : (kind[i] == 0 ? 1.0 : c2) + cw * (double)looks[i] / len + (len >= 8192.0 ? pc.hot : 0.0));
 		cum[i + 1] = cum[i] + jump[i] + len * dens[i];
 	}
 	for (size_t b = 0; b <= B; ++b) cum_b[b] = cum[std::min<size_t>(bseg[b], S)];
@@ -1311,8 +1328,10 @@
 	const unsigned tables_bytes = generic_tables_bytes;
 	double max_skew = 0.0;
 	for (int m = 0; m < M; ++m) max_skew = std::max(max_skew, c->reads[m].skew);
-	const unsigned cap = c->opt_wg_per_cu >= 0 ? (unsigned)c->opt_wg_per_cu : (c->em.small_places >= c->em.opt_flat_min && max_skew < 4.0 ? 5u : 0u);
-	const unsigned lds_bytes = std::max(tables_bytes + WAVES * WAVE_QUEUE_WORDS * 16, cap ? 160u * 1024u / (cap + 1u) + 16u : 0u);
+	const unsigned cap = c->opt_wg_per_cu >= 0 ? (unsigned)c->opt_wg_per_cu : (c->em.small_places >= c->em.opt_flat_min && max_skew < 4.0 ? 5u : (unsigned)LSQ_FAST_WAVES);
+	bool any_wide = false;
+	for (int m = 0; m < M; ++m) if (c->reads[m].total_slots && !c->reads[m].compact) any_wide = true;
+	const unsigned lds_bytes = std::max(tables_bytes + (any_wide ? WAVES * WAVE_QUEUE_WORDS * 16 : 0u), cap ? 160u * 1024u / (cap + 1u) + 16u : 0u);
 	if (lds_bytes > 160 * 1024) return fail(LSQ_E_UNSUPPORTED, "bucket tables + read tile exceed the CU's LDS");
 	bool all_compact = true;
 	for (int m = 0; m < M; ++m) if (c->reads[m].total_slots && !c->reads[m].compact) all_compact = false;
@@ -1405,7 +1424,8 @@
 		A.total_slots = mr.total_slots;
 		A.cnt = c->cnt.p + (size_t)m * n_cls; A.bases = c->bases.p + (size_t)m * n_cls;
 		A.exc = mr.exc.p + (size_t)set * mr.exc_cap; A.exc_count = c->exc_count.p + 2 * m; A.exc_cap = (unsigned)mr.exc_cap;
-		A.dbg = c->dbg.p; A.bar = c->dbg.p + 16 + m;
+		A.dbg = c->dbg.p; A.bar = c->dbg.p + 16 + m; A.guard = c->guard_count.p + m;
+		A.looks = reinterpret_cast<const lsq::LookRec *>(mr.looks.p);
 		A.wg_trace = nullptr;
 		const unsigned long long n_pn = mr.pn_strand.n;
 		A.n_pn = n_pn;
@@ -1481,6 +1501,17 @@
 	return LSQ_OK;
 } LSQ_API_CATCH
 
+int lsq_count_guard_entries(lsq_ctx *c, uint32_t *guards) LSQ_API_TRY {
+	if (!c || !guards) return fail(LSQ_E_ARG, "null argument");
+	if (!c->counted) return fail(LSQ_E_STATE, "lsq_count must come first");
+	HIP_TRY(hipSetDevice(c->device));
+	{ int rc = sync_all(c); if (rc) return rc; }
+	std::vector<unsigned long long> h(c->guard_count.n);
+	HIP_TRY(hipMemcpy(h.data(), c->guard_count.p, h.size() * sizeof(unsigned long long), hipMemcpyDeviceToHost));
+	for (int m = 0; m < c->E->n_methods; ++m) guards[m] = (uint32_t)std::min<unsigned long long>(h[(size_t)m], 0xFFFFFFFFull);
+	return LSQ_OK;
+} LSQ_API_CATCH
+
 int lsq_count_launch_info(lsq_ctx *c, uint32_t *reads_per_look, uint32_t *workgroups_per_cu) LSQ_API_TRY {
 	if (!c) return fail(LSQ_E_ARG, "null context");
 	if (!c->counted) return fail(LSQ_E_STATE, "lsq_count must come first");
diff --git a/lesseq_amd/csrc/lsq_device.hip b/lesseq_amd/csrc/lsq_device.hip
--- a/lesseq_amd/csrc/lsq_device.hip
+++ b/lesseq_amd/csrc/lsq_device.hip
@@ -57,6 +57,7 @@
 	c->bases.p = base + per;
 	c->exc_count.p = reinterpret_cast<unsigned *>(base + 2 * per);
 	c->dbg.p = base + 2 * per + LSQ_MAX_METHODS;
+	c->guard_count.p = c->dbg.p + 16 + LSQ_MAX_METHODS;
 }
 
 void note_overflow(lsq_ctx *c, const std::vector<unsigned> &h) {
@@ -282,9 +283,9 @@
 	const size_t n_cls = E->n_cls_total, n_ev = E->dev2out.size();
 	{
 		const size_t per = std::max<size_t>(M, 1) * n_cls;
-		c->counters_per_set = 2 * per + LSQ_MAX_METHODS + 16 + LSQ_MAX_METHODS;
+		c->counters_per_set = 2 * per + LSQ_MAX_METHODS + 16 + 2 * LSQ_MAX_METHODS;
 		if ((rc = c->counters.alloc(LSQ_COUNTER_SETS * c->counters_per_set))) return rc;
-		c->cnt.n = per; c->bases.n = per; c->exc_count.n = 2 * LSQ_MAX_METHODS; c->dbg.n = 16;
+		c->cnt.n = per; c->bases.n = per; c->exc_count.n = 2 * LSQ_MAX_METHODS; c->dbg.n = 16; c->guard_count.n = LSQ_MAX_METHODS;
 		for (bool &r : c->mark_recorded2) r = false;
 		c->fim_uploaded = false; c->fim_done = false;
 		select_counter_set(c, 0, 0);
@@ -375,7 +376,7 @@
 		c->n_fine = bb.back();
 		if ((rc = c->bin_base.upload(bb.data(), bb.size(), c->stream))) return rc;
 		std::vector<unsigned> cb(E->buckets.size() + 1, 0);
-		for (size_t b = 0; b < E->buckets.size(); ++b) cb[b + 1] = cb[b] + (E->buckets[b].kind == 1 ? (E->buckets[b].iso_off & 0xFFFFu) : 0u) + 1u;
+		for (size_t b = 0; b < E->buckets.size(); ++b) cb[b + 1] = cb[b] + (E->buckets[b].kind == 1 ? (E->buckets[b].iso_off & 0xFFFFu) : 0u) + 2u;
 		c->n_cell_groups = cb.back();
 		if ((rc = c->cell_base.upload(cb.data(), cb.size(), c->stream))) return rc;
 		std::vector<unsigned> jb(E->buckets.size() + 1, 0);
@@ -841,6 +842,8 @@
 	} else if (n == "exception_capacity") {
 		if (!(value >= 0 && value <= 4e9)) return fail(LSQ_E_ARG, "exception_capacity must lie in 0..4e9 (0 = automatic)");
 		c->opt_exc_cap = (size_t)value;
+	} else if (n == "hard_looks") {
+		c->opt_hard_looks = value != 0;
 	} else if (n == "snap_shares") {
 		c->opt_snap_shares = value != 0;
 		for (auto &r : c->reads) r.wg_grid = 0;
diff --git a/lesseq_amd/csrc/lsq_device.hpp b/lesseq_amd/csrc/lsq_device.hpp
--- a/lesseq_amd/csrc/lsq_device.hpp
+++ b/lesseq_amd/csrc/lsq_device.hpp
@@ -99,14 +99,16 @@
 	unsigned long long bs, be;
 	unsigned long long p1o, p1n, p2o, p2n;
 	unsigned b, next;
-	unsigned pad[2];
-};
-static_assert(sizeof(VisitRec) == 128, "VisitRec is read as 32 dwords");
+	unsigned lk1n, lk2n;
+	unsigned long long lko;
+	unsigned long long pad;
+};
+static_assert(sizeof(VisitRec) == 144, "VisitRec is read as 36 dwords");
 struct WgPlan {
 	unsigned long long s_begin, s_end;
 	VisitRec first;
 };
-static_assert(sizeof(WgPlan) == 144, "WgPlan layout");
+static_assert(sizeof(WgPlan) == 160, "WgPlan layout");
 
 struct IngestPass {
 	const char *name = nullptr;
@@ -128,6 +130,10 @@
 	DevBuf<uint8_t> p1_strand, p2_strand, pn_strand;
 	DevBuf<uint32_t> p1_line, p2_line, pn_line, pn_blk_off, pn_nblk, pn_bucket;
 	DevBuf<unsigned long long> p1_off, p2_off, pn_off, pnb_off, slot_off;
+	DevBuf<uint4> looks;
+	bool hard_routed = false;
+	uint64_t n_hard1 = 0, n_hard2 = 0, n_looks1 = 0, n_looks2 = 0;
+	float looks_ms = 0;
 	double skew = 1.0;
 	bool named = false;
 	DevBuf<char> names;
@@ -247,6 +253,7 @@
 	DevBuf<unsigned long long> wg_trace;
 	unsigned long long wg_trace_n = 0, wg_trace_workers = 0;
 	DevView<unsigned> exc_count;
+	DevView<unsigned long long> guard_count;
 	DevBuf<RouteChrom> route_chrom;
 	DevBuf<int2> cov;
 	DevBuf<int4> clu;
@@ -264,6 +271,7 @@
 	size_t opt_exc_cap = 0;
 	bool opt_compact_pools = true;
 	bool opt_recount = false;
+	bool opt_hard_looks = true;
 	unsigned opt_cleanup_grid = 0;
 	bool overflow_logged[LSQ_MAX_METHODS] = {};
 	bool opt_snap_shares = true;
diff --git a/lesseq_amd/csrc/lsq_ingest.hip b/lesseq_amd/csrc/lsq_ingest.hip
--- a/lesseq_amd/csrc/lsq_ingest.hip
+++ b/lesseq_amd/csrc/lsq_ingest.hip
@@ -1,5 +1,6 @@
 #include "lsq_ingest.hpp"
 #include "lsq_text.hpp"
+#include "lsq_settle.hpp"
 
 namespace {
 
@@ -186,6 +187,7 @@
 	unsigned *fine1, *fine2;
 	unsigned *cnt1, *cnt2;
 	unsigned *park1, *park2;
+	unsigned route_hard;
 };
 
 __global__ void __launch_bounds__(256) lsq_group_classify_kernel(GroupTables T, GroupArgs A) {
@@ -195,7 +197,7 @@
 	const BucketDesc d = T.buckets[b];
 	const unsigned n_cells = d.kind == 1u ? (d.iso_off & 0xFFFFu) : 0u;
 	const unsigned k0 = T.jg_base[b], k1 = T.jg_base[b + 1];
-	const unsigned n_groups = pool ? (k1 - k0) + n_cells + 1u : n_cells + 1u;
+	const unsigned n_groups = pool ? (k1 - k0) + n_cells + 2u : n_cells + 2u;
 	const unsigned gbase = pool ? T.jgroup_base[b] : T.cell_base[b];
 	unsigned char *img = glds;
 	unsigned long long *keys = reinterpret_cast<unsigned long long *>(glds + T.lds_img);
@@ -210,8 +212,8 @@
 	const lsq::FastRec *recs = reinterpret_cast<const lsq::FastRec *>(img + d.ev_off);
 	const unsigned long long first = (pool ? A.off2[b] : A.off1[b]) + pc.y;
 	for (unsigned r = threadIdx.x; r < pc.z; r += 256u) {
-		int s0, e0, s1 = 0;
-		if (pool) { const uint4 v = A.part2[2ull * (first + r)]; s0 = (int)v.x; e0 = (int)v.y; s1 = (int)v.z; }
+		int s0, e0, s1 = 0, e1 = 0;
+		if (pool) { const uint4 v = A.part2[2ull * (first + r)]; s0 = (int)v.x; e0 = (int)v.y; s1 = (int)v.z; e1 = (int)v.w; }
 		else { const uint4 v = A.part1[first + r]; s0 = (int)v.x; e0 = (int)v.y; }
 		unsigned cell = 0, g = pool ? (k1 - k0) : 0u, looks_est = 0;
 		if (d.kind == 1u) {
@@ -234,8 +236,19 @@
 				in_junction_group = jg < k1 - k0;
 				g = in_junction_group ? jg : (k1 - k0) + cell;
 			} else g = cell;
-			bool parks = cell == n_cells, one_event = false;
-			if (!parks && !in_junction_group) {
+			if (A.route_hard) {
+				const bool in_cell = cell < n_cells;
+				const lsq::Cell cw = cells[in_cell ? cell : 0u];
+				const lsq::CellX cx = cellx[in_cell ? cell : 0u];
+				const bool settles = pool ? lsq::settles_in_loop2(s0, e0, s1, e1, in_cell, in_junction_group, cw, cx, recs[in_cell && cx.info < lsq::CELL_INFO_EMPTY ? cx.ev : 0u])
+				                          : lsq::settles_in_loop1(s0, e0, in_cell, cw, cx);
+				if (!settles) {
+					const unsigned looks = lsq::for_each_look(recs, d.n_events, br.x >> 16, p, e0, pool != 0u, in_cell, cw, cx, [](unsigned) {});
+					if (looks <= lsq::HARD_LOOK_LIMIT) { g = n_groups - 1u; atomicAdd(&park[g], looks); }
+				}
+			}
+			bool parks = !A.route_hard && cell == n_cells, one_event = false;
+			if (!A.route_hard && !parks && !in_junction_group) {
 				const lsq::Cell cw = cells[cell];
 				const unsigned fl = cellx[cell].flags;
 				const int len = e0 - s0;
@@ -313,7 +326,7 @@
 	const unsigned pool = pc.x >= A.B ? 1u : 0u, b = pc.x - pool * A.B;
 	const BucketDesc &d = A.buckets[b];
 	const unsigned n_cells = d.kind == 1u ? (d.iso_off & 0xFFFFu) : 0u;
-	const unsigned n_groups = pool ? (A.jg_base[b + 1] - A.jg_base[b]) + n_cells + 1u : n_cells + 1u;
+	const unsigned n_groups = pool ? (A.jg_base[b + 1] - A.jg_base[b]) + n_cells + 2u : n_cells + 2u;
 	const unsigned gbase = pool ? A.jgroup_base[b] : A.cell_base[b];
 	const unsigned long long first = (pool ? A.part_off2[b] : A.part_off1[b]) + pc.y;
 	const unsigned *fine = (pool ? A.fine2 : A.fine1) + first;
@@ -410,6 +423,58 @@
 			if (compact) reinterpret_cast<unsigned *>(p1)[w] = (unsigned)(at - base);
 			else reinterpret_cast<int2 *>(p1)[w] = make_int2(at, at);
 			p1_strand[w] = 0; p1_line[w] = 0;
+		}
+	}
+}
+
+struct LookArgs {
+	const BucketDesc *buckets;
+	const unsigned char *images;
+	const unsigned *cell_base, *jgroup_base;
+	const unsigned *cnt1, *cnt2;
+	const unsigned long long *off1, *off2;
+	const unsigned long long *p1_off, *p2_off;
+	const unsigned *p1; const uint2 *p2;
+	const unsigned long long *look_off;
+	unsigned *cursor;
+	lsq::LookRec *looks;
+};
+__global__ void __launch_bounds__(256) lsq_ingest_looks_kernel(LookArgs A) {
+	const unsigned b = blockIdx.x;
+	const BucketDesc d = A.buckets[b];
+	if (d.kind != 1u) return;
+	const unsigned char *img = A.images + d.img_off;
+	const unsigned *bins = reinterpret_cast<const unsigned *>(img);
+	const lsq::Cell *cells = reinterpret_cast<const lsq::Cell *>(img + d.seg_off);
+	const lsq::CellX *cellx = reinterpret_cast<const lsq::CellX *>(img + d.seg_off + 16u * (d.iso_off >> 16));
+	const lsq::FastRec *recs = reinterpret_cast<const lsq::FastRec *>(img + d.ev_off);
+	const unsigned n_cells = d.iso_off & 0xFFFFu;
+	const int base = d.lo - lsq::COMPACT_BIAS;
+	for (unsigned pool = 0; pool < 2u; ++pool) {
+		const unsigned g = (pool ? A.jgroup_base[b + 1] : A.cell_base[b + 1]) - 1u;
+		const unsigned n = pool ? A.cnt2[g] : A.cnt1[g];
+		const unsigned long long first = pool ? A.off2[g] : A.off1[g];
+		const unsigned slot0 = (unsigned)(first - (pool ? A.p2_off[b] : A.p1_off[b]));
+		const unsigned long long out0 = A.look_off[2u * b + pool], out1 = A.look_off[2u * b + pool + 1u];
+		for (unsigned r = threadIdx.x; r < n; r += 256u) {
+			unsigned wa, wb = 0u;
+			if (pool) { const uint2 v = A.p2[first + r]; wa = v.x; wb = v.y; } else wa = A.p1[first + r];
+			const int p = base + (int)(wa & lsq::COMPACT_OFF_MASK);
+			const int rel = p - d.lo;
+			const unsigned bin = rel <= 0 ? 0u : min((unsigned)rel >> d.shift, d.n_bins - 1u);
+			const unsigned *br = bins + 4u * bin;
+			const unsigned cell = lsq::cell_of_position(br, cells, n_cells, p);
+			const bool in_cell = cell < n_cells;
+			const lsq::Cell cw = cells[in_cell ? cell : 0u];
+			const lsq::CellX cx = cellx[in_cell ? cell : 0u];
+			const int e = p + (int)(wa >> lsq::COMPACT_OFF_BITS);
+			const unsigned looks = lsq::for_each_look(recs, d.n_events, br[0] >> 16, p, e, pool != 0u, in_cell, cw, cx, [](unsigned) {});
+			if (!looks) continue;
+			unsigned long long at = out0 + atomicAdd(&A.cursor[2u * b + pool], looks);
+			lsq::for_each_look(recs, d.n_events, br[0] >> 16, p, e, pool != 0u, in_cell, cw, cx, [&](unsigned ev) {
+				if (at < out1) { lsq::LookRec L; L.a = wa; L.b = wb; L.ev = ev; L.slot = slot0 + r; A.looks[at] = L; }
+				++at;
+			});
 		}
 	}
 }
@@ -480,7 +545,7 @@
 		const size_t n_cells = d.kind == 1u ? (d.iso_off & 0xFFFFu) : 0u, n_jg = E.jg_base[b + 1] - E.jg_base[b];
 		if (d.kind == 1u) img_max = std::max<size_t>(img_max, (d.img_bytes + 15u) & ~15u);
 		jg_max = std::max(jg_max, n_jg);
-		groups_max = std::max(groups_max, n_jg + n_cells + 1);
+		groups_max = std::max(groups_max, n_jg + n_cells + 2);
 	}
 	const size_t keys_lds = (8 * jg_max + 15) & ~(size_t)15, group_lds = img_max + keys_lds + 8 * groups_max, place_lds = 8 * groups_max;
 	if (group_lds > 160 * 1024) return fail(LSQ_E_UNSUPPORTED, "a bucket's tables and group counters exceed the CU's LDS");
@@ -568,6 +633,7 @@
 	GroupArgs GA{};
 	GA.pieces = d_pieces.p; GA.off1 = d_part_off1.p; GA.off2 = d_part_off2.p; GA.part1 = d_part1.p; GA.part2 = d_part2.p;
 	GA.fine1 = d_fine1.p; GA.fine2 = d_fine2.p; GA.cnt1 = cnt1; GA.cnt2 = cnt2; GA.park1 = park1; GA.park2 = park2;
+	GA.route_hard = (compact && c->opt_hard_looks) ? 1u : 0u;
 	if (n_pieces) {
 		StageClock k(c, st, "group_classify");
 		GroupTables GT{};
@@ -643,9 +709,10 @@
 	mr.total_slots = n1 + n2 + nn;
 	mr.wg_grid = 0;
 	{
-		std::vector<unsigned long long> so(B + 1, 0), o1(B + 1, 0), o2(B + 1, 0), f1(FC + 1, 0), f2(FJ + 1, 0);
-		std::vector<unsigned> park(FC + FJ + 1, 0);
-		HIP_TRY(hipMemcpyAsync(so.data(), mr.slot_off.p, (B + 1) * sizeof(unsigned long long), hipMemcpyDeviceToHost, st));
+		std::vector<unsigned long long> so(B + 1, 0), o1(B + 1, 0), o2(B + 1, 0), on(B + 1, 0), f1(FC + 1, 0), f2(FJ + 1, 0);
+		std::vector<unsigned> park(FC + FJ + 1, 0), gcnt(FC + FJ + 1, 0);
+		HIP_TRY(hipMemcpyAsync(on.data(), mr.pn_off.p, (B + 1) * sizeof(unsigned long long), hipMemcpyDeviceToHost, st));
+		if (FC + FJ) HIP_TRY(hipMemcpyAsync(gcnt.data(), cnt1, (FC + FJ) * sizeof(unsigned), hipMemcpyDeviceToHost, st));
 		HIP_TRY(hipMemcpyAsync(o1.data(), mr.p1_off.p, (B + 1) * sizeof(unsigned long long), hipMemcpyDeviceToHost, st));
 		HIP_TRY(hipMemcpyAsync(o2.data(), mr.p2_off.p, (B + 1) * sizeof(unsigned long long), hipMemcpyDeviceToHost, st));
 		HIP_TRY(hipMemcpyAsync(f1.data(), d_off1.p, (FC + 1) * sizeof(unsigned long long), hipMemcpyDeviceToHost, st));
@@ -654,6 +721,51 @@
 		HIP_TRY(hipStreamSynchronize(st));
 		SW.mark("ingest: place + read-back");
 		stages_collect(c);
+		const bool hard = GA.route_hard != 0u;
+		std::vector<unsigned long long> lko(2 * (size_t)B + 1, 0), e1n(B, 0), e2n(B, 0);
+		mr.hard_routed = hard; mr.n_hard1 = mr.n_hard2 = 0;
+		{
+			size_t g1 = 0, g2 = 0;
+			for (unsigned b = 0; b < B; ++b) {
+				const unsigned n_cg = (E.buckets[b].kind == 1 ? (E.buckets[b].iso_off & 0xFFFFu) : 0u) + 2u, n_jg = (E.jg_base[b + 1] - E.jg_base[b]) + n_cg;
+				const size_t h1 = g1 + n_cg - 1, h2 = g2 + n_jg - 1;
+				e1n[b] = f1[h1] - o1[b]; e2n[b] = f2[h2] - o2[b];
+				const unsigned long long l1 = hard ? park[h1] : 0u, l2 = hard ? park[FC + h2] : 0u;
+				mr.n_hard1 += gcnt[h1]; mr.n_hard2 += gcnt[FC + h2];
+				lko[2 * (size_t)b + 1] = lko[2 * (size_t)b] + l1; lko[2 * (size_t)b + 2] = lko[2 * (size_t)b + 1] + l2;
+				so[b + 1] = so[b] + e1n[b] + e2n[b] + l1 + l2 + (on[b + 1] - on[b]);
+				g1 += n_cg; g2 += n_jg;
+			}
+		}
+		const unsigned long long n_looks = lko[2 * (size_t)B];
+		if (n_looks > 0xFFFFFFF0ull) return fail(LSQ_E_RANGE, "more than 2^32 look records in one read file");
+		mr.n_looks1 = mr.n_looks2 = 0; mr.looks_ms = 0;
+		for (unsigned b = 0; b < B; ++b) { mr.n_looks1 += lko[2 * (size_t)b + 1] - lko[2 * (size_t)b]; mr.n_looks2 += lko[2 * (size_t)b + 2] - lko[2 * (size_t)b + 1]; }
+		if ((rc = mr.looks.alloc((size_t)n_looks))) return rc;
+		if ((rc = mr.slot_off.upload(so.data(), so.size(), st))) return rc;
+		mr.total_slots = B ? so[B] : 0;
+		if (n_looks) {
+			hipEvent_t t0 = nullptr, t1 = nullptr;
+			HIP_TRY(hipEventCreate(&t0)); HIP_TRY(hipEventCreate(&t1));
+			HIP_TRY(hipEventRecord(t0, st));
+			DevBuf<unsigned long long> d_lko;
+			DevBuf<unsigned> d_cursor;
+			if ((rc = d_lko.upload(lko.data(), lko.size(), st)) || (rc = d_cursor.alloc(2 * (size_t)B))) return rc;
+			HIP_TRY(hipMemsetAsync(d_cursor.p, 0, 2 * (size_t)B * sizeof(unsigned), st));
+			HIP_TRY(hipMemsetAsync(mr.looks.p, 0, (size_t)n_looks * sizeof(uint4), st));
+			LookArgs LA{};
+			LA.buckets = c->buckets.p; LA.images = c->images.p; LA.cell_base = c->cell_base.p; LA.jgroup_base = c->jgroup_base.p;
+			LA.cnt1 = cnt1; LA.cnt2 = cnt2; LA.off1 = d_off1.p; LA.off2 = d_off2.p; LA.p1_off = mr.p1_off.p; LA.p2_off = mr.p2_off.p;
+			LA.p1 = reinterpret_cast<const unsigned *>(mr.p1.p); LA.p2 = reinterpret_cast<const uint2 *>(mr.p2.p);
+			LA.look_off = d_lko.p; LA.cursor = d_cursor.p; LA.looks = reinterpret_cast<lsq::LookRec *>(mr.looks.p);
+			hipLaunchKernelGGL(lsq_ingest_looks_kernel, dim3(B), dim3(256), 0, st, LA);
+			HIP_TRY(hipGetLastError());
+			HIP_TRY(hipEventRecord(t1, st));
+			HIP_TRY(hipStreamSynchronize(st));
+			mr.looks_ms = 0;
+			(void)hipEventElapsedTime(&mr.looks_ms, t0, t1);
+			(void)hipEventDestroy(t0); (void)hipEventDestroy(t1);
+		}
 		unsigned long long mx = 0;
 		for (unsigned b = 0; b < B; ++b) mx = std::max(mx, so[b + 1] - so[b]);
 		mr.slot_off_host = so;
@@ -663,23 +775,26 @@
 			mr.plan_seg_x.clear(); mr.plan_seg_kind.clear(); mr.plan_seg_looks.clear(); mr.plan_seg_first.assign(B + 1, 0);
 			size_t g1 = 0, g2 = 0;
 			for (unsigned b = 0; b < B; ++b) {
-				const unsigned n_cg = (E.buckets[b].kind == 1 ? (E.buckets[b].iso_off & 0xFFFFu) : 0u) + 1u, n_jg = (E.jg_base[b + 1] - E.jg_base[b]) + n_cg;
-				const unsigned long long n1 = o1[b + 1] - o1[b], n2 = o2[b + 1] - o2[b], ns = so[b + 1] - so[b];
+				const unsigned n_cg = (E.buckets[b].kind == 1 ? (E.buckets[b].iso_off & 0xFFFFu) : 0u) + 2u, n_jg = (E.jg_base[b + 1] - E.jg_base[b]) + n_cg;
+				const unsigned long long n1 = e1n[b], n2 = e2n[b], ns = so[b + 1] - so[b];
+				const unsigned long long l1 = lko[2 * (size_t)b + 1] - lko[2 * (size_t)b], l2 = lko[2 * (size_t)b + 2] - lko[2 * (size_t)b + 1];
 				mr.plan_n1[b] = n1; mr.plan_n2[b] = n2;
 				mr.plan_seg_first[b] = (unsigned)mr.plan_seg_kind.size();
 				const bool visited = E.buckets[b].kind == 1u && ns != 0;
 				if (visited) {
-					for (unsigned q = 0; q < n_cg && g1 + q < FC; ++q) {
+					for (unsigned q = 0; q + 1 < n_cg && g1 + q < FC; ++q) {
 						const unsigned long long a = f1[g1 + q], e = f1[g1 + q + 1];
 						mr.plan_park1[b] += park[g1 + q];
 						if (e > a) { mr.plan_seg_x.push_back(so[b] + (a - o1[b])); mr.plan_seg_kind.push_back(0); mr.plan_seg_looks.push_back(park[g1 + q]); }
 					}
-					for (unsigned q = 0; q < n_jg && g2 + q < FJ; ++q) {
+					for (unsigned q = 0; q + 1 < n_jg && g2 + q < FJ; ++q) {
 						const unsigned long long a = f2[g2 + q], e = f2[g2 + q + 1];
 						mr.plan_park2[b] += park[FC + g2 + q];
 						if (e > a) { mr.plan_seg_x.push_back(so[b] + n1 + (a - o2[b])); mr.plan_seg_kind.push_back(1); mr.plan_seg_looks.push_back(park[FC + g2 + q]); }
 					}
-					if (ns > n1 + n2) { mr.plan_seg_x.push_back(so[b] + n1 + n2); mr.plan_seg_kind.push_back(2); mr.plan_seg_looks.push_back(0); }
+					mr.plan_park1[b] += (unsigned)l1; mr.plan_park2[b] += (unsigned)l2;
+					if (l1 + l2) { mr.plan_seg_x.push_back(so[b] + n1 + n2); mr.plan_seg_kind.push_back(3); mr.plan_seg_looks.push_back(0); }
+					if (ns > n1 + n2 + l1 + l2) { mr.plan_seg_x.push_back(so[b] + n1 + n2 + l1 + l2); mr.plan_seg_kind.push_back(2); mr.plan_seg_looks.push_back(0); }
 				} else if (ns) { mr.plan_seg_x.push_back(so[b]); mr.plan_seg_kind.push_back(2); mr.plan_seg_looks.push_back(0); }
 				g1 += n_cg; g2 += n_jg;
 			}
@@ -694,7 +809,8 @@
 			VisitRec &v = vis[b];
 			v.d = E.buckets[b];
 			v.bs = so[b]; v.be = so[b + 1];
-			v.p1o = o1[b]; v.p1n = o1[b + 1] - o1[b]; v.p2o = o2[b]; v.p2n = o2[b + 1] - o2[b];
+			v.p1o = o1[b]; v.p1n = e1n[b]; v.p2o = o2[b]; v.p2n = e2n[b];
+			v.lko = lko[2 * (size_t)b]; v.lk1n = (unsigned)(lko[2 * (size_t)b + 1] - lko[2 * (size_t)b]); v.lk2n = (unsigned)(lko[2 * (size_t)b + 2] - lko[2 * (size_t)b + 1]);
 			v.b = b; v.next = next;
 			if (E.buckets[b].kind == 1u && so[b + 1] > so[b]) next = b;
 			mr.next_packed_host[b] = next;
@@ -813,6 +929,16 @@
 } LSQ_API_CATCH
 uint64_t lsq_reads_retained_blocks(const lsq_ctx *c, int method) { return (c && method >= 0 && method < LSQ_MAX_METHODS) ? c->reads[method].n_retained_blocks : 0; }
 
+int lsq_reads_hard_looks(const lsq_ctx *c, int method, uint64_t out[6]) LSQ_API_TRY {
+	if (!c || !out || method < 0 || method >= LSQ_MAX_METHODS) return fail(LSQ_E_ARG, "bad context or method");
+	const MethodReads &mr = c->reads[method];
+	if (!mr.present) return fail(LSQ_E_STATE, "no reads uploaded for method %d", method);
+	out[0] = mr.n_hard1; out[1] = mr.n_hard2; out[2] = mr.n_looks1; out[3] = mr.n_looks2;
+	out[4] = (mr.n_looks1 + mr.n_looks2) * sizeof(lsq::LookRec);
+	out[5] = (uint64_t)(mr.looks_ms * 1000.0f);
+	return LSQ_OK;
+} LSQ_API_CATCH
+
 int lsq_reads_pool_format(const lsq_ctx *c, int method, int *compact, uint64_t *pool_bytes, uint64_t *pool_reads) LSQ_API_TRY {
 	if (!c || method < 0 || method >= LSQ_MAX_METHODS) return fail(LSQ_E_ARG, "bad context or method");
 	const MethodReads &mr = c->reads[method];
diff --git a/lesseq_amd/csrc/lsq_replay.hip b/lesseq_amd/csrc/lsq_replay.hip
--- a/lesseq_amd/csrc/lsq_replay.hip
+++ b/lesseq_amd/csrc/lsq_replay.hip
@@ -1,4 +1,6 @@
 #include "lsq_device.hpp"
+#include "lsq_settle.hpp"
+#include <array>
 #include <atomic>
 
 
@@ -467,7 +469,11 @@
 		const size_t n1 = R.p1_line.size(), n2 = R.p2_line.size();
 		if ((n1 % P1_GROUP_PAD) || (n2 % P2_GROUP_PAD)) return fail(LSQ_E_STATE, "bucket %zu: pool slices of %zu and %zu records are not whole groups of %u / %u", b, n1, n2, P1_GROUP_PAD, P2_GROUP_PAD);
 		out[0] += n1; out[3] += n2;
-		for (size_t q = 0; q < n1; q += P1_GROUP_PAD) {
+		const size_t h1 = std::min<size_t>(n1, (size_t)mr.visits_host[b].p1n), h2 = std::min<size_t>(n2, (size_t)mr.visits_host[b].p2n);
+		if ((h1 % P1_GROUP_PAD) || (h2 % P2_GROUP_PAD)) return fail(LSQ_E_STATE, "bucket %zu: the hard groups start at records %zu and %zu, inside a group", b, h1, h2);
+		for (size_t k = h1; k < n1; ++k) out[1] += R.p1[2 * k] == R.p1[2 * k + 1];
+		for (size_t k = h2; k < n2; ++k) out[4] += R.p2[4 * k] == R.p2[4 * k + 1];
+		for (size_t q = 0; q < h1; q += P1_GROUP_PAD) {
 			long first = -2;
 			bool mixed = false;
 			for (size_t k = q; k < q + P1_GROUP_PAD; ++k) {
@@ -486,7 +492,7 @@
 			const uint64_t *it = std::lower_bound(k0, k1, want);
 			return (it != k1 && *it == want) ? (long)(it - k0) : -1;
 		};
-		for (size_t q = 0; q < n2; q += P2_GROUP_PAD) {
+		for (size_t q = 0; q < h2; q += P2_GROUP_PAD) {
 			const int32_t *ra = &R.p2[4 * q];
 			const bool ea = ra[0] == ra[1];
 			const long ga = ea ? -1 : group_of(ra);
@@ -502,6 +508,56 @@
 			}
 			if (bad) ++out[5];
 		}
+		if (!mr.compact || d.kind != 1) {
+			if (h1 != n1 || h2 != n2 || mr.visits_host[b].lk1n || mr.visits_host[b].lk2n) return fail(LSQ_E_STATE, "bucket %zu: hard reads or look records outside compact pools of a packed bucket", b);
+			continue;
+		}
+		const lsq::CellX *cellx = reinterpret_cast<const lsq::CellX *>(E.images.data() + d.img_off + d.seg_off + 16u * (d.iso_off >> 16));
+		const lsq::FastRec *recs = reinterpret_cast<const lsq::FastRec *>(E.images.data() + d.img_off + d.ev_off);
+		const uint32_t *bins = reinterpret_cast<const uint32_t *>(E.images.data() + d.img_off);
+		const int32_t base = d.lo - lsq::COMPACT_BIAS;
+		typedef std::array<uint32_t, 4> Look;
+		std::vector<Look> want[2], have[2];
+		const lsq::Cell no_cell{0, 0, 0, 0};
+		const lsq::CellX no_cellx{0, 0, 0, 0};
+		for (int pool = 0; pool < 2; ++pool) {
+			const size_t n = pool ? n2 : n1, h = pool ? h2 : h1;
+			for (size_t k = 0; k < n; ++k) {
+				const int32_t *r = pool ? &R.p2[4 * k] : &R.p1[2 * k];
+				if (r[0] == r[1]) continue;
+				const long cl = cell_of(r[0]);
+				const bool in_cell = cl >= 0;
+				const lsq::Cell &cw = in_cell ? cells[cl] : no_cell;
+				const lsq::CellX &cx = in_cell ? cellx[cl] : no_cellx;
+				const bool settles = pool ? lsq::settles_in_loop2(r[0], r[1], r[2], r[3], in_cell, group_of(r) >= 0, cw, cx, recs[in_cell && cx.info < lsq::CELL_INFO_EMPTY ? cx.ev : 0u])
+				                          : lsq::settles_in_loop1(r[0], r[1], in_cell, cw, cx);
+				const int rel = r[0] - d.lo;
+				const uint32_t bin = rel <= 0 ? 0u : std::min<uint32_t>((uint32_t)rel >> d.shift, d.n_bins - 1u);
+				const uint32_t wa = (uint32_t)(r[0] - base) | ((uint32_t)(r[1] - r[0]) << lsq::COMPACT_OFF_BITS);
+				const uint32_t wb = pool ? (uint32_t)(r[2] - r[1]) | ((uint32_t)(r[3] - r[2]) << lsq::COMPACT_OFF_BITS) : 0u;
+				std::vector<uint32_t> evs;
+				const unsigned looks = lsq::for_each_look(recs, d.n_events, bins[4u * bin] >> 16, r[0], r[1], pool != 0, in_cell, cw, cx, [&](uint32_t ev) { evs.push_back(ev); });
+				if (k < h) {
+					if (mr.hard_routed && !settles && looks <= lsq::HARD_LOOK_LIMIT)
+						return fail(LSQ_E_STATE, "bucket %zu, %s pool, record %zu: the streaming loop does not settle it, and it lies outside the hard group", b, pool ? "two-block" : "one-block", k);
+				} else {
+					if (settles) return fail(LSQ_E_STATE, "bucket %zu, %s pool, record %zu: a read of the hard group that the streaming loop settles", b, pool ? "two-block" : "one-block", k);
+					if (looks > lsq::HARD_LOOK_LIMIT) return fail(LSQ_E_STATE, "bucket %zu, %s pool, record %zu: a read of the hard group past the look limit", b, pool ? "two-block" : "one-block", k);
+					for (uint32_t ev : evs) want[pool].push_back(Look{wa, wb, ev, (uint32_t)k});
+				}
+			}
+		}
+		{
+			const lsq::VisitRec &v = mr.visits_host[b];
+			std::vector<lsq::LookRec> lk((size_t)v.lk1n + v.lk2n);
+			if (!lk.empty()) HIP_TRY(hipMemcpy(lk.data(), reinterpret_cast<const lsq::LookRec *>(mr.looks.p) + v.lko, lk.size() * sizeof(lsq::LookRec), hipMemcpyDeviceToHost));
+			for (size_t q = 0; q < lk.size(); ++q) have[q < v.lk1n ? 0 : 1].push_back(Look{lk[q].a, lk[q].b, lk[q].ev, lk[q].slot});
+			for (int pool = 0; pool < 2; ++pool) {
+				std::sort(want[pool].begin(), want[pool].end()); std::sort(have[pool].begin(), have[pool].end());
+				if (want[pool] != have[pool])
+					return fail(LSQ_E_STATE, "bucket %zu: the %s look records (%zu) are not the (read, event) pairs of its hard reads (%zu)", b, pool ? "two-block" : "one-block", have[pool].size(), want[pool].size());
+			}
+		}
 	}
 	if (out[0] - out[1] != mr.n1_reads || out[3] - out[4] != mr.n2_reads)
 		return fail(LSQ_E_STATE, "the pools hold %llu + %llu reads, the ingest counted %llu + %llu", out[0] - out[1], out[3] - out[4],
diff --git a/lesseq_amd/csrc/lsq_settle.hpp b/lesseq_amd/csrc/lsq_settle.hpp
--- /dev/null
+++ b/lesseq_amd/csrc/lsq_settle.hpp
@@ -0,0 +1,85 @@
+#pragma once
+#include "lsq_internal.hpp"
+
+#if defined(__HIPCC__)
+#define LSQ_HD __host__ __device__
+#else
+#define LSQ_HD
+#endif
+
+namespace lsq {
+
+constexpr unsigned HARD_LOOK_LIMIT = 64;
+
+struct LookRec {
+	uint32_t a, b;
+	uint32_t ev;
+	uint32_t slot;
+};
+static_assert(sizeof(LookRec) == 16, "LookRec is one 16-byte load");
+
+LSQ_HD inline bool settles_in_loop1(const int s, const int e, const bool in_cell, const Cell &cw, const CellX &cx) {
+	(void)s;
+	if (!in_cell) return false;
+	return e <= ((cx.flags & CELLX_BOTH) != 0u ? cw.e1 : cw.e2);
+}
+
+LSQ_HD inline bool settles_in_loop2(const int s0, const int e0, const int s1, const int e1, const bool in_cell, const bool in_junction_group,
+                                    const Cell &cw, const CellX &cx, const FastRec &owner) {
+	if (!in_cell) return false;
+	const uint32_t info = cx.info, k1 = (info >> 2) & 0x3Fu;
+	const bool v1 = info < CELL_INFO_EMPTY, start1 = k1 == CELL_K_START;
+	if (in_junction_group) {
+		if (!v1 || start1 || s1 == e0) return false;
+		const bool ends1 = e0 == cw.e1, ends1b = cw.e2 > cw.e1 && e0 == cw.e2;
+		if (!ends1 && !ends1b) return false;
+		const uint32_t k2 = s1 == owner.seg[2] ? 1u : (s1 == owner.seg[4] ? 2u : (s1 == owner.seg[6] ? 3u : 0u));
+		const int end2 = k2 == 1u ? owner.seg[3] : (k2 == 2u ? owner.seg[5] : owner.seg[7]);
+		const uint32_t abut = (owner.meta >> FAST_ABUT_SHIFT) & 7u;
+		const bool abut2 = k2 != 0u && k2 < 3u && ((abut >> k2) & 1u) != 0u;
+		const int end2b = !abut2 ? end2 : (k2 == 1u ? owner.seg[5] : owner.seg[7]);
+		const uint32_t k1e = ends1b ? k1 + 1u : k1;
+		return k2 > k1e && e1 <= end2b;
+	}
+	if (info == CELL_INFO_EMPTY) return true;
+	const int l1 = e0 - s0, l2 = e1 - s1;
+	const bool weak = s1 != e0 && 50 * l1 <= 49 * (l1 + l2);
+	const bool near_free = (cx.flags & CELLX_NEAR_NO_ABUT) != 0u, far_free = (cx.flags & CELLX_FAR_NO_ABUT) != 0u;
+	const bool one_ok = e0 <= cw.e2;
+	const bool two_ok = e0 != cw.e1 && e0 != cw.e2 && (e0 < cw.e1 || near_free) && (e0 < cw.e2 || far_free);
+	return weak && ((cx.flags & CELLX_BOTH) != 0u ? two_ok : (v1 && !start1 && one_ok));
+}
+
+template <class F>
+LSQ_HD inline unsigned for_each_look(const FastRec *recs, const uint32_t n_events, const uint32_t first_event, const int p, const int e, const bool two_block,
+                                     const bool in_cell, const Cell &cw, const CellX &cx, F &&f) {
+	if (in_cell && cx.info < CELL_INFO_EMPTY) { f(cx.ev); return 1u; }
+	if (in_cell && cx.info == CELL_INFO_EMPTY) return 0u;
+	if (in_cell) {
+		const int len = e - p;
+		const bool gone_near = !two_block && (cx.flags & CELLX_NEAR_NO_ABUT) != 0u && e > cw.e1 && 50 * (e - cw.e1) >= len;
+		const bool gone_far = !two_block && (cx.flags & CELLX_FAR_NO_ABUT) != 0u && e > cw.e2 && 50 * (e - cw.e2) >= len;
+		unsigned looks = 0;
+		if (!gone_near) { f(cx.ev); ++looks; }
+		if (!gone_far) { f(cx.flags & 0xFFFFu); ++looks; }
+		return looks;
+	}
+	unsigned looks = 0;
+	for (uint32_t i = first_event; i < n_events; ++i) {
+		if (looks == HARD_LOOK_LIMIT) return HARD_LOOK_LIMIT + 1u;
+		++looks;
+		f(i);
+		const FastRec &fr = recs[i];
+		if (!(fr.seg[0] <= p && (p > fr.ge || (fr.meta & FAST_FLAG_OVERLAPS_NEXT) != 0u))) break;
+	}
+	return looks;
+}
+
+LSQ_HD inline uint32_t cell_of_position(const uint32_t *bin_record, const Cell *cells, const uint32_t n_cells, const int p) {
+	uint32_t cell = (bin_record[0] & 0xFFFFu) + (uint32_t)(p >= (int)bin_record[1]) + (uint32_t)(p >= (int)bin_record[2]) + (uint32_t)(p >= (int)bin_record[3]);
+	if (p >= (int)bin_record[3]) while (cell + 1u < n_cells && p >= cells[cell + 1u].lo) ++cell;
+	if (!(cell < n_cells && cells[cell].lo <= p && p < cells[cell].hi)) cell = n_cells;
+	return cell;
+}
+
+}
```

New measurement: 833.6 billion reads/s. Within noise of the previous version (-0.5%).
